# RWAlgorithms/ConjugateGradientOptim.jl

Measured on AMD Instinct MI355X. Metric: CG iterations/sec at n=1e8 (outer iterations of minimizeobjective, PR-CG), higher is better.
Workload: dtype f64

## Files before the change

conjugategradientoptim.jl_amd/_lib.py:

```python
from __future__ import annotations

import ctypes as C
import os
import subprocess

_PKG = os.path.dirname(os.path.abspath(__file__))
LIB_PATH = os.environ.get("CGO_LIB_PATH") or os.path.join(_PKG, "lib", "libcgo_hip.so")
CSRC = os.path.join(_PKG, "csrc")

dp = C.POINTER(C.c_double)
i64p = C.POINTER(C.c_int64)


class BetaConfig(C.Structure):
    _fields_ = [("kind", C.c_int32), ("lbfgs_m", C.c_int32), ("mu", C.c_double)]


class CGConfigC(C.Structure):
    _fields_ = [("eps", C.c_double), ("beta", BetaConfig), ("max_iters", C.c_int64),
                ("verbose", C.c_int32), ("trace_enabled", C.c_int32)]


class LSConfigC(C.Structure):
    _fields_ = [("kind", C.c_int32), ("cond_kind", C.c_int32), ("c1", C.c_double),
# ... 89 lines not shown
    _fields_ = [("kind", C.c_int32), ("k", C.c_int32), ("a", C.c_double * 7), ("a_acc", C.c_double), ("beta", C.c_double),
                ("co_set", C.c_int32), ("co_count", C.c_int32), ("co_gamma", C.c_double), ("co_cy", C.c_double * 10),
                ("co_cs", C.c_double * 10)]


class BatchPassOutC(C.Structure):
    _fields_ = [("ts", (C.c_double * 7) * 7), ("gu", C.c_double), ("uu", C.c_double), ("width", C.c_int64), ("stored", C.c_int64)]


class BatchProbeC(C.Structure):
    _fields_ = [("tier", C.c_int32), ("obj_kind", C.c_int32), ("m", C.c_int32), ("n_params", C.c_int32), ("model", C.c_void_p),
                ("n", C.c_int64), ("batch", C.c_int64), ("x", dp), ("u", dp), ("params", dp * 4), ("scalars", dp),
                ("skip", C.POINTER(C.c_uint8)), ("S", dp), ("Y", dp), ("qn", C.c_void_p), ("npass", C.c_int32),
                ("reserved", C.c_int32), ("pass_", BatchPassC * 32), ("rows", dp), ("out", C.POINTER(BatchPassOutC)),
                ("x_out", dp), ("u_out", dp), ("g_out", dp), ("S_out", dp), ("Y_out", dp), ("qn_out", C.c_void_p),
                ("reason", C.POINTER(C.c_int32)), ("done", i64p), ("passes", i64p), ("points", C.c_int32),
                ("reserved2", C.c_int32), ("ld", C.c_int64), ("symbol", C.c_char * 128)]


ALLGATHER_FN = C.CFUNCTYPE(C.c_int, C.c_void_p, dp, dp, C.c_int32)
FDF_FN = C.CFUNCTYPE(C.c_double, C.c_void_p, dp, dp, C.c_int64)

_vp = C.c_void_p
_pp = C.POINTER(C.c_void_p)
SIGNATURES = {
    "cgo_version": (C.c_int, []),
    "cgo_build_id": (C.c_char_p, []),
    "cgo_last_error": (C.c_char_p, []),
    "cgo_status_name": (C.c_char_p, [C.c_int32]),
    "cgo_device_count": (C.c_int, [C.POINTER(C.c_int32)]),
    "cgo_check_cg_config": (C.c_int, [C.POINTER(CGConfigC)]),
    "cgo_check_ls_config": (C.c_int, [C.POINTER(LSConfigC)]),
    "cgo_ctx_create": (C.c_int, [C.c_int32, _pp]),
    "cgo_solver_policy_init": (None, [C.POINTER(SolverPolicyC)]),
    "cgo_ctx_set_default_policy": (C.c_int, [_vp, C.POINTER(SolverPolicyC)]),
    "cgo_solver_get_policy": (C.c_int, [_vp, C.POINTER(SolverPolicyC)]),
    "cgo_solver_create_ex": (C.c_int, [_vp, _vp, C.POINTER(CGConfigC), C.POINTER(LSConfigC), C.POINTER(SolverPolicyC), _pp]),
    "cgo_solver_create_sys_ex": (C.c_int, [_vp, _vp, C.POINTER(CGConfigC), C.POINTER(LSSConfigC), C.POINTER(SolverPolicyC), _pp]),
    "cgo_ctx_destroy": (C.c_int, [_vp]),
    "cgo_comm_unique_id": (C.c_int, [_vp]),
    "cgo_ctx_set_comm_rccl": (C.c_int, [_vp, C.c_int32, C.c_int32, _vp]),
    "cgo_ctx_set_comm_callback": (C.c_int, [_vp, C.c_int32, C.c_int32, ALLGATHER_FN, _vp]),
    "cgo_ctx_set_comm_shm": (C.c_int, [_vp, C.c_int32, C.c_int32, C.c_char_p, C.c_int32]),
    "cgo_shm_unlink": (C.c_int, [C.c_char_p]),
    "cgo_ctx_comm_info": (C.c_int, [_vp, C.POINTER(C.c_int32), C.POINTER(C.c_int32), C.POINTER(C.c_int32), C.POINTER(C.c_int32)]),
    "cgo_ctx_exchange_stats": (C.c_int, [_vp, i64p, dp, dp, C.c_int32]),
    "cgo_ctx_comm_connect_devices": (C.c_int, [_vp, C.POINTER(C.c_int32)]),
    "cgo_rccl_available": (C.c_int, []),
    "cgo_objective_create": (C.c_int, [_vp, C.c_int32, C.c_int64, C.c_int64, C.c_int64, _pp]),
    "cgo_objective_create_from_source": (C.c_int, [_vp, C.c_char_p, C.c_int32, C.c_int64, C.c_int64, C.c_int64, _pp]),
    "cgo_objective_create_callback": (C.c_int, [_vp, FDF_FN, _vp, C.c_int64, C.c_int64, C.c_int64, _pp]),
    "cgo_objective_destroy": (C.c_int, [_vp]),
    "cgo_objective_create_from_source_ex": (C.c_int, [_vp, C.c_char_p, C.c_int32, C.c_int64, C.c_int64, C.c_int64, _pp]),
    "cgo_objective_num_params": (C.c_int, [_vp, C.POINTER(C.c_int32)]),
    "cgo_objective_set_param_host": (C.c_int, [_vp, C.c_int32, dp]),
    "cgo_objective_set_param_device": (C.c_int, [_vp, C.c_int32, _vp]),
    "cgo_objective_fill_param": (C.c_int, [_vp, C.c_int32, C.c_int32, C.c_uint64, C.c_double, C.c_double]),
    "cgo_objective_set_scalar": (C.c_int, [_vp, C.c_int32, C.c_double]),
    "cgo_objective_set_cost_class": (C.c_int, [_vp, C.c_int32]),
    "cgo_objective_eval_host": (C.c_int, [_vp, dp, dp, dp]),
    "cgo_solver_create": (C.c_int, [_vp, _vp, C.POINTER(CGConfigC), C.POINTER(LSConfigC), _pp]),
    "cgo_solver_destroy": (C.c_int, [_vp]),
    "cgo_solver_set_x0_host": (C.c_int, [_vp, dp]),
    "cgo_solver_set_x0_fill": (C.c_int, [_vp, C.c_int32, C.c_uint64, C.c_double, C.c_double]),
    "cgo_solver_set_x0_device": (C.c_int, [_vp, _vp]),
    "cgo_solver_results_device": (C.c_int, [_vp, _vp, _vp]),
    "cgo_solver_start": (C.c_int, [_vp]),
    "cgo_solver_iterate": (C.c_int, [_vp, C.c_int64, C.POINTER(C.c_int32)]),
    "cgo_solver_results": (C.c_int, [_vp, C.POINTER(ResultsC)]),
    "cgo_solver_trial_log": (C.c_int, [_vp, C.c_int64, dp, dp, dp, i64p]),
    "cgo_solver_profile_enable": (C.c_int, [_vp, C.c_int32]),
    "cgo_solver_profile_reset": (C.c_int, [_vp]),
    "cgo_solver_profile_get": (C.c_int, [_vp, C.c_int32, i64p, dp, dp]),
    "cgo_kernel_kind_name": (C.c_char_p, [C.c_int32]),
    "cgo_solver_kernel_family": (C.c_char_p, [_vp]),
    "cgo_solver_controller_launches": (C.c_int64, [_vp]),
    "cgo_solver_resident_stats": (C.c_int, [_vp, i64p, i64p, i64p]),
    "cgo_solver_lbfgs_stats": (C.c_int, [_vp, i64p, i64p, i64p]),
    "cgo_num_kernel_kinds": (C.c_int, []),
    "cgo_solver_set_lazy_direction": (C.c_int, [_vp, C.c_int32]),
    "cgo_solver_probe_set_beta_prev": (C.c_int, [_vp, C.c_double]),
    "cgo_solver_set_replay_depth": (C.c_int, [_vp, C.c_int32]),
    "cgo_solver_set_lean_sums": (C.c_int, [_vp, C.c_int32]),
    "cgo_solver_probe_set_replay": (C.c_int, [_vp, C.c_int32, dp, dp]),
    "cgo_solver_kernel_symbol": (C.c_int, [_vp, C.c_int32, C.c_char_p, C.c_int32]),
    "cgo_evalwolfeconditions": (C.c_int, [C.POINTER(LSConfigC), C.c_double, C.c_double, C.c_double, C.c_double,
                                          C.c_double, C.c_double, C.POINTER(C.c_int32), C.POINTER(C.c_int32)]),
    "cgo_evalbacktrackcondition": (C.c_int, [C.POINTER(LSConfigC), C.c_double, C.c_double, C.c_double, C.c_double,
                                             C.POINTER(C.c_int32)]),
    "cgo_check_lss_config": (C.c_int, [C.POINTER(LSSConfigC)]),
    "cgo_lss_default_max_iters": (C.c_int64, [C.c_double]),
    "cgo_solver_create_sys": (C.c_int, [_vp, _vp, C.POINTER(CGConfigC), C.POINTER(LSSConfigC), _pp]),
    "cgo_solvesystem": (C.c_int, [_vp, _vp, dp, C.POINTER(CGConfigC), C.POINTER(LSSConfigC), C.POINTER(ResultsC)]),
    "cgo_minimize": (C.c_int, [_vp, _vp, dp, C.POINTER(CGConfigC), C.POINTER(LSConfigC), C.POINTER(ResultsC)]),
    "cgo_minimize_rerun": (C.c_int, [_vp, _vp, dp, C.POINTER(CGConfigC), C.POINTER(LSConfigC),
                                     C.POINTER(CGConfigC), C.POINTER(LSConfigC), C.c_int32,
                                     C.POINTER(ResultsC), C.POINTER(C.c_int32)]),
    "cgo_minimize_batch": (C.c_int, [_vp, C.c_int32, C.c_int64, C.c_int64, dp, dp, C.POINTER(CGConfigC), C.POINTER(LSConfigC),
                                     C.c_int64, C.POINTER(BatchResultsC)]),
    "cgo_batch_max_n": (C.c_int64, [_vp, C.c_int32]),
    "cgo_minimize_batch_obj": (C.c_int, [_vp, _vp, C.c_int64, dp, C.POINTER(dp), C.c_int32, C.POINTER(CGConfigC), C.POINTER(LSConfigC),
                                         C.c_int64, C.POINTER(BatchResultsC)]),
    "cgo_batch_max_n_obj": (C.c_int64, [_vp]),
    "cgo_batch_open": (C.c_int, [_vp, _vp, C.c_int64, C.POINTER(dp), C.c_int32, C.POINTER(_vp)]),
    "cgo_batch_solve": (C.c_int, [_vp, dp, dp, C.POINTER(C.c_uint8), C.POINTER(CGConfigC), C.POINTER(LSConfigC), C.c_int64,
                                  C.POINTER(BatchResultsC)]),
    "cgo_batch_close": (C.c_int, [_vp]),
    "cgo_batch_policy_init": (None, [C.POINTER(BatchPolicyC)]),
    "cgo_minimize_batch_ex": (C.c_int, [_vp, C.c_int32, C.c_int64, C.c_int64, dp, dp, C.POINTER(CGConfigC), C.POINTER(LSConfigC),
                                        C.c_int64, C.POINTER(BatchPolicyC), C.POINTER(BatchResultsC), C.POINTER(C.c_int32)]),
    "cgo_minimize_batch_obj_ex": (C.c_int, [_vp, _vp, C.c_int64, dp, C.POINTER(dp), C.c_int32, C.POINTER(CGConfigC), C.POINTER(LSConfigC),
                                            C.c_int64, C.POINTER(BatchPolicyC), C.POINTER(BatchResultsC), C.POINTER(C.c_int32)]),
    "cgo_batch_open_ex": (C.c_int, [_vp, _vp, C.c_int64, C.POINTER(dp), C.c_int32, C.POINTER(BatchPolicyC), C.POINTER(_vp)]),
    "cgo_batch_rows": (C.c_int, [_vp, C.POINTER(C.c_int32)]),
    "cgo_batch_max_n_ex": (C.c_int64, [_vp, C.c_int32, C.POINTER(BatchPolicyC)]),
    "cgo_batch_max_n_obj_ex": (C.c_int64, [_vp, C.POINTER(BatchPolicyC)]),
    "cgo_batch_rows_shape": (None, [C.POINTER(C.c_int32), C.POINTER(C.c_int32)]),
    "cgo_minimize_batch_lbfgs": (C.c_int, [_vp, C.c_int32, C.c_int64, C.c_int64, dp, dp, C.POINTER(CGConfigC), C.POINTER(LSConfigC),
                                           C.c_int64, C.POINTER(BatchResultsC)]),
    "cgo_batch_lbfgs_max_m": (C.c_int32, []),
    "cgo_batch_lbfgs_max_n": (C.c_int64, [_vp, C.c_int32]),
    "cgo_batch_lbfgs_shape": (None, [C.POINTER(C.c_int32), C.POINTER(C.c_int32)]),
    "cgo_minimize_batch_lbfgs_obj": (C.c_int, [_vp, _vp, C.c_int64, dp, C.POINTER(dp), C.c_int32, dp, C.POINTER(CGConfigC), C.POINTER(LSConfigC),
                                               C.c_int64, C.POINTER(BatchResultsC)]),
    "cgo_batch_lbfgs_max_n_obj": (C.c_int64, [_vp]),
    "cgo_batch_lbfgs_shape_obj": (None, [C.c_int32, C.POINTER(C.c_int32), C.POINTER(C.c_int32)]),
    "cgo_minimize_batch_lbfgs_ex": (C.c_int, [_vp, C.c_int32, C.c_int64, C.c_int64, dp, dp, C.POINTER(CGConfigC), C.POINTER(LSConfigC),
                                              C.c_int64, C.POINTER(BatchPolicyC), C.POINTER(BatchResultsC), C.POINTER(C.c_int32)]),
    "cgo_minimize_batch_lbfgs_obj_ex": (C.c_int, [_vp, _vp, C.c_int64, dp, C.POINTER(dp), C.c_int32, dp, C.POINTER(CGConfigC),
                                                  C.POINTER(LSConfigC), C.c_int64, C.POINTER(BatchPolicyC), C.POINTER(BatchResultsC),
                                                  C.POINTER(C.c_int32)]),
    "cgo_batch_lbfgs_max_n_ex": (C.c_int64, [_vp, C.c_int32, C.c_int32, C.POINTER(BatchPolicyC)]),
    "cgo_batch_lbfgs_max_n_obj_ex": (C.c_int64, [_vp, C.c_int32, C.POINTER(BatchPolicyC)]),
    "cgo_batch_lbfgs_lds_rows": (C.c_int32, [C.c_int32, C.c_int32]),
    "cgo_batch_lbfgs_lds_shape": (None, [C.c_int32, C.POINTER(C.c_int32), C.POINTER(C.c_int32)]),
    "cgo_batch_lbfgs_open": (C.c_int, [_vp, _vp, C.c_int64, C.POINTER(dp), C.c_int32, C.c_int32, C.POINTER(BatchPolicyC), C.POINTER(_vp)]),
    "cgo_batch_lbfgs_solve": (C.c_int, [_vp, dp, dp, C.POINTER(C.c_uint8), C.POINTER(CGConfigC), C.POINTER(LSConfigC), C.c_int64,
                                        C.POINTER(BatchResultsC)]),
    "cgo_batch_lbfgs_m": (C.c_int, [_vp, C.POINTER(C.c_int32)]),
    "cgo_batch_probe": (C.c_int, [_vp, C.POINTER(BatchProbeC)]),
    "cgo_batch_probe_qn_bytes": (C.c_int64, []),
    "cgo_stop_status": (C.c_int32, [C.c_int64, C.c_int64, C.c_double, C.c_double, C.c_double, C.c_double, i64p]),
    "cgo_kernel_dir": (C.c_int, [_vp, dp, dp, C.c_double, C.c_int64, dp]),
    "cgo_kernel_beta_partials": (C.c_int, [_vp, dp, dp, dp, C.c_int64, dp]),
    "cgo_getbeta": (C.c_int, [_vp, C.POINTER(BetaConfig), dp, dp, dp, C.c_int64, dp]),
    "cgo_kernel_trial": (C.c_int, [_vp, dp, dp, C.c_double, dp, dp]),
    "cgo_bench_kernel": (C.c_int, [_vp, _vp, C.c_int32, C.c_int64, C.c_int32, dp, dp]),
    "cgo_bench_stream_mix": (C.c_int, [_vp, C.c_int64, C.c_int32, dp, dp]),
    "cgo_solver_placement_info": (C.c_int, [_vp, dp, dp, C.POINTER(C.c_int32)]),
    "cgo_solver_probe_launch": (C.c_int, [_vp, C.c_int32, C.c_int32, C.c_double, C.c_double, dp, C.c_int32, dp, dp, dp,
                                          dp, C.c_int32, C.POINTER(C.c_int32), dp, dp, dp, C.c_char_p, C.c_int32]),
    "cgo_solver_probe_lbfgs": (C.c_int, [_vp, C.POINTER(LbfgsProbeC)] + [dp] * 13),
    "cgo_solver_probe_resident": (C.c_int, [_vp, C.POINTER(ResidentProbeC), dp, dp, dp, C.c_int64, dp, dp]),
    "cgo_solver_probe_armed": (C.c_int, [_vp, C.POINTER(ArmedProbeC), dp, dp, dp, dp]),
}


class CgoError(RuntimeError):
    def __init__(self, code: int, msg: str):
        super().__init__(f"[cgo error {code}] {msg}")
        self.code = code
        self.msg = msg


def build(force: bool = False) -> str:
    if force:
# ... 34 lines not shown
```

conjugategradientoptim.jl_amd/api.py:

```python
from __future__ import annotations

import ctypes as C
import math
import re
from dataclasses import dataclass, field
from typing import List, Optional, Sequence, Union

import numpy as np

from . import _lib
from ._lib import BetaConfig, CGConfigC, LSConfigC, LSSConfigC, ResultsC, check, dp, i64p



class TraceTrait:
    pass


class EnableTrace(TraceTrait):
    def __repr__(self):
        return "EnableTrace()"


class DisableTrace(TraceTrait):
# ... 561 lines not shown
        c.lse_fixed_reference = tri(self.lse_fixed_reference)
        c.resident_points = self.resident_points or 0
        c.resident_chunk = self.resident_chunk or 0
        c.hbm_stream_bytes = float(self.hbm_stream_bytes or 0.0)
        return c


class Solver:
    def __init__(self, fdf: DeviceObjective, config: CGConfig, linesearch_config: LineSearchConfig,
                 policy: Optional[SolverPolicy] = None):
        if not isinstance(fdf, DeviceObjective):
            raise TypeError(
                "fdf! must be an objective descriptor: a device objective (QuadDiag, RosenbrockPaired, Booth, "
                "ElementwiseObjective, ...) or HostObjective(closure, n) — there is no CPU solver path in this package")
        self.obj, self.config, self.ls = fdf, config, linesearch_config
        self._cfg_c, self._ls_c = config._c(), linesearch_config._c()
        self._h = C.c_void_p()
        create = (_lib.lib().cgo_solver_create_sys_ex if isinstance(linesearch_config, LinesearchSolveSys)
                  else _lib.lib().cgo_solver_create_ex)
        self._pol_c = policy._c() if policy is not None else None
        check(create(fdf.ctx._h, fdf._h, C.byref(self._cfg_c), C.byref(self._ls_c),
                     C.byref(self._pol_c) if self._pol_c is not None else None, C.byref(self._h)))

    def policy(self) -> dict:
        c = _lib.SolverPolicyC()
        check(_lib.lib().cgo_solver_get_policy(self._h, C.byref(c)))
        return {n: getattr(c, n) for n, _ in c._fields_ if n not in ("size", "reserved")}

    def set_x0(self, x_initial_global: np.ndarray):
        loc = self.obj.local(np.asarray(x_initial_global, dtype=np.float64))
        check(_lib.lib().cgo_solver_set_x0_host(self._h, loc.ctypes.data_as(dp)))

    def set_x0_fill(self, fill: str, lo: float, hi: float = 0.0, seed: int = 0):
        check(_lib.lib().cgo_solver_set_x0_fill(self._h, FILL_KINDS[fill], seed, lo, hi))

    def set_x0_device(self, x0):
        check(_lib.lib().cgo_solver_set_x0_device(self._h, _dev_ptr(x0, self.obj.n_local)))

    def results_device(self, minimizer=None, gradient=None):
        check(_lib.lib().cgo_solver_results_device(self._h, _dev_ptr(minimizer, self.obj.n_local), _dev_ptr(gradient, self.obj.n_local)))

    def start(self):
        check(_lib.lib().cgo_solver_start(self._h))

    def iterate(self, iters: int) -> bool:
        fin = C.c_int32(0)
        check(_lib.lib().cgo_solver_iterate(self._h, iters, C.byref(fin)))
        return bool(fin.value)

    def enable_trial_log(self):
        cnt = C.c_int64()
        check(_lib.lib().cgo_solver_trial_log(self._h, -1, None, None, None, C.byref(cnt)))

    def trial_log(self):
        cnt = C.c_int64()
        check(_lib.lib().cgo_solver_trial_log(self._h, 0, None, None, None, C.byref(cnt)))
        k = cnt.value
        a, p, d = np.zeros(max(k, 1)), np.zeros(max(k, 1)), np.zeros(max(k, 1))
        check(_lib.lib().cgo_solver_trial_log(self._h, k, a.ctypes.data_as(dp), p.ctypes.data_as(dp),
                                              d.ctypes.data_as(dp), C.byref(cnt)))
        return a[:k], p[:k], d[:k]

    def kernel_family(self) -> str:
        return _lib.lib().cgo_solver_kernel_family(self._h).decode()

    def kernel_symbol(self, kind_name: str) -> str:
        L = _lib.lib()
        buf = C.create_string_buffer(200)
        for k in range(L.cgo_num_kernel_kinds()):
            if L.cgo_kernel_kind_name(k).decode() == kind_name:
                check(L.cgo_solver_kernel_symbol(self._h, k, buf, 200))
                return buf.value.decode()
        return ""

    def set_lazy_direction(self, on: bool = True):
        check(_lib.lib().cgo_solver_set_lazy_direction(self._h, int(bool(on))))

    def set_replay_depth(self, d: int):
        check(_lib.lib().cgo_solver_set_replay_depth(self._h, int(d)))

    def set_lean_sums(self, on: bool):
        check(_lib.lib().cgo_solver_set_lean_sums(self._h, int(bool(on))))

    def probe_launch(self, kind_name: str, variant: int, a_acc: float, beta: float, a: Sequence[float], x, u=None, aux=None,
                     beta_prev: Optional[float] = None, replay: Optional[Sequence] = None):
        L = _lib.lib()
        kk = [L.cgo_kernel_kind_name(k).decode() for k in range(L.cgo_num_kernel_kinds())].index(kind_name)
        if beta_prev is not None:
            check(L.cgo_solver_probe_set_beta_prev(self._h, float(beta_prev)))
        if replay is not None:
            ra = np.ascontiguousarray([p[0] for p in replay], dtype=np.float64)
            rb = np.ascontiguousarray([p[1] for p in replay], dtype=np.float64)
            check(L.cgo_solver_probe_set_replay(self._h, len(replay), ra.ctypes.data_as(dp), rb.ctypes.data_as(dp)))
        n = self.obj.n_local
        vec = lambda v: None if v is None else np.ascontiguousarray(v, dtype=np.float64)
        x, u, aux = vec(x), vec(u), vec(aux)
        for v in (x, u, aux):
            if v is not None and v.size != n:
                raise ValueError(f"probe vectors hold n_local = {n} elements")
        av = np.ascontiguousarray(a, dtype=np.float64) if len(a) else np.zeros(1)
        sums, ln = np.full(64, np.nan), C.c_int32(0)
        xo, uo, go = np.empty(n), np.empty(n), np.empty(n)
        sym = C.create_string_buffer(200)
        ptr = lambda v: None if v is None else v.ctypes.data_as(dp)
        check(L.cgo_solver_probe_launch(self._h, kk, int(variant), float(a_acc), float(beta), ptr(av), len(a), ptr(x), ptr(u),
                                        ptr(aux), ptr(sums), 64, C.byref(ln), ptr(xo), ptr(uo), ptr(go), sym, 200))
        return dict(sums=sums[:ln.value].copy(), x=xo, u=uo, g=go, symbol=sym.value.decode())

    LBFGS_PASSES = ("push", "push_gram", "direction_gram", "direction_trial", "push_lite", "loop")

    def probe_lbfgs(self, pass_name: str, x=None, u=None, g=None, gt=None, S=None, Y=None, **kw):
        n = self.obj.n_local
        P = self._cfg_c.beta.lbfgs_m + 1
        vec = lambda v: None if v is None else np.ascontiguousarray(v, dtype=np.float64)
        x, u, g, gt = vec(x), vec(u), vec(g), vec(gt)
        for v in (x, u, g, gt):
            if v is not None and v.size != n:
                raise ValueError(f"probe vectors hold n_local = {n} elements")
        S = None if S is None else np.ascontiguousarray(S, dtype=np.float64).reshape(P, n)
        Y = None if Y is None else np.ascontiguousarray(Y, dtype=np.float64).reshape(P, n)
        p = _lib.LbfgsProbeC()
        p.pass_ = self.LBFGS_PASSES.index(pass_name)
        dots = None
        for key, val in kw.items():
            if key in ("list", "spec_list"):
                getattr(p, key)[:len(val)] = [int(v) for v in val]
                setattr(p, "count" if key == "list" else "spec_count", len(val))
            elif key in ("cy", "cs", "alpha"):
                getattr(p, key)[:len(val)] = [float(v) for v in val]
            elif key == "stats":
                p.M, p.S = float(val[0]), float(val[1])
            elif key == "dots":
                dots = np.ascontiguousarray(val, dtype=np.float64).reshape(-1, 10)
                p.dots, p.dot_count = dots.ctypes.data_as(dp), dots.shape[0]
            else:
                if not hasattr(p, key):
                    raise TypeError(f"probe_lbfgs: no field {key}")
                setattr(p, key, val)
        outs = {k: np.full(n, np.nan) for k in ("x", "xo", "u", "g", "gt")}
        So, Yo = np.full((P, n), np.nan), np.full((P, n), np.nan)
        ptr = lambda v: None if v is None else v.ctypes.data_as(dp)
        check(_lib.lib().cgo_solver_probe_lbfgs(self._h, C.byref(p), ptr(x), ptr(u), ptr(g), ptr(gt), ptr(S), ptr(Y),
                                                *[ptr(outs[k]) for k in ("x", "xo", "u", "g", "gt")], ptr(So), ptr(Yo)))
        sym = p.symbol.decode()
        return dict(sums=np.array(p.sums[:p.sums_len]), S=So, Y=Yo, alpha=np.array(p.alpha[:]), symbols=sym.split(" + ") if sym else [],
                    new_in_list=p.new_in_list, spec_ok=bool(p.spec_ok),
                    gram=np.array(p.gram[:5 + 5 * p.spec_count]) if p.spec_ok else None, **outs)

    def probe_resident(self, script, x, u):
        n = self.obj.n_local
        x, u = np.ascontiguousarray(x, dtype=np.float64), np.ascontiguousarray(u, dtype=np.float64)
        if x.size != n or u.size != n:
            raise ValueError(f"probe vectors hold n_local = {n} elements")
        p = _lib.ResidentProbeC()
        if len(script) > 32:
            raise ValueError("probe_resident: at most 32 passes")
        p.npass = len(script)
        for q, item in enumerate(script):
            c = p.pass_[q]
            if item[0] == "trial":
                c.kind, a = 0, item[1]
            elif item[0] == "accept_dir_trial":
                c.kind, c.a_acc, c.beta, a = 1, float(item[1]), float(item[2]), item[3]
            else:
                raise ValueError(f"probe_resident: no pass kind {item[0]!r}")
            if len(a) > 7:
                raise ValueError("probe_resident: at most 7 trial steps")
            c.k = len(a)
            c.a[:len(a)] = [float(v) for v in a]
        rows = np.full((max(p.npass, 1), 256, 56), np.nan)
        xo, uo = np.empty(n), np.empty(n)
        check(_lib.lib().cgo_solver_probe_resident(self._h, C.byref(p), x.ctypes.data_as(dp), u.ctypes.data_as(dp),
                                                   rows.ctypes.data_as(dp), rows.size, xo.ctypes.data_as(dp), uo.ctypes.data_as(dp)))
        g = p.grid
        got = rows.ravel()[:p.npass * g * 56].reshape(p.npass, g, 56)
        outs, rws, tails = [], [], []
# ... 1097 lines not shown
```

conjugategradientoptim.jl_amd/csrc/cgo_backend_cg.hip:

```cpp
#include "cgo_backend_internal.hpp"

#include "cgo_kernels.hip.hpp"
#include "cgo_kernels_cg.hip.hpp"
#include "cgo_kernels_chain.hip.hpp"
#include "cgo_kernels_lse.hip.hpp"
#include "cgo_kernels_resident.hip.hpp"

namespace cgo {

using namespace dev;

double bytes_r(int obj_kind, int mode, int64_t n, int n_params) {
    const int p = std::max(obj_kind == CGO_OBJ_QUAD_DIAG ? 1 : 0, n_params);
    return 8.0 * (double)n * (double)r_vectors(mode, p);
}

template <int N> using Pts = std::integral_constant<int, N>;
template <int MAXPTS, class F>
static inline void with_points(int npts, F f) {
    static_assert(MAXPTS == 1 || MAXPTS == 3 || MAXPTS == 5 || MAXPTS == 7, "a launch evaluates 1, 3, 5 or 7 trial points");
    if constexpr (MAXPTS >= 3) { if (npts == 3) return f(Pts<3>{}); }
    if constexpr (MAXPTS >= 5) { if (npts == 5) return f(Pts<5>{}); }
    if constexpr (MAXPTS >= 7) { if (npts != 1) return f(Pts<7>{}); }
    return f(Pts<1>{});
}

template <class Obj, bool BIG>
static int launch_cg(int mode, int npts, const RParams &P, int grid, hipStream_t st) {
#define ROW(MODE, MAXPTS) if (mode == (MODE) && P.tail.ctl) { with_points<MAXPTS>(npts, [&](auto n) { k_cg_armed<Obj, decltype(n)::value><<<grid, BLOCK, 0, st>>>(P); }); return 0; }
    CGO_CG_ARMED_ROWS(ROW)
#undef ROW
    switch (mode) {
#define ROW(MODE, MAXPTS) case (MODE): with_points<MAXPTS>(npts, [&](auto n) { k_cg<Obj, (MODE), decltype(n)::value, BIG><<<grid, BLOCK, 0, st>>>(P); }); return 0;
    CGO_CG_ROWS(ROW)
#undef ROW
    default: break;
    }
    if constexpr (BIG) {
        switch (mode) {
#define ROW(MODE, MAXPTS) case (MODE): with_points<MAXPTS>(npts, [&](auto n) { k_cg<Obj, (MODE), decltype(n)::value, true><<<grid, BLOCK, 0, st>>>(P); }); return 0;
        CGO_CG_LAG_ROWS(ROW)
        CGO_CG_REPLAY_ROWS(ROW)
        CGO_CG_LEAN_ROWS(ROW)
#undef ROW
        default: break;
        }
    }
    return -1;
}

static inline bool lean_row(int mode) {
#define ROW(MODE, MAXPTS) if (mode == (MODE)) return true;
    CGO_CG_LEAN_ROWS(ROW)
#undef ROW
    return false;
}
int HipBackend::lean_for(int mode) const { return (lean_bits_ && lean_row(mode | lean_bits_)) ? lean_bits_ : 0; }

void unpack_r(const double *s, int k, Scal *out, bool dir, int npts) {
    if (npts == 0) npts = npts_for(k);
    for (int j = 0; j < k; ++j) {
        const double *q = s + RS_PER_POINT * j;
        out[j].f = q[RS_F]; out[j].gtu = q[RS_GTU]; out[j].gtgt = q[RS_GTGT]; out[j].gtg = q[RS_GTG];
        out[j].yy = q[RS_YY]; out[j].uy = q[RS_UY]; out[j].ygt = q[RS_YGT];
    }
    if (dir) { out[0].gu = s[RS_PER_POINT * npts]; out[0].uu = s[RS_PER_POINT * npts + 1]; }
}

static inline int chain_npts(int mode, int npts) { return ((mode & R_TRIAL) && npts >= 3) ? 3 : 1; }

RPlan HipBackend::r_plan(int mode, int npts) const {
    const double bytes = bytes_r(obj_->kind, mode, obj_->n_local, obj_->nparams());
    const bool big = r_big_only(mode) || bytes > big_bytes(r_read_only(mode));
    return {big, big ? GRID_BIG : grid_cg(obj_->n_local, chain() ? 1 : npts), chain() ? chain_npts(mode, npts) : npts, bytes};
}
bool HipBackend::adt_is_big() const { return bytes_r(obj_->kind, R_ADT, obj_->n_local, obj_->nparams()) > big_bytes(false); }

int HipBackend::launch_r(int kk, int mode, double a_acc, double beta, const double *a, int k, bool fetch,
                         double *sums) {
    if (int rc = pipe_drain()) return rc;
    pipe_streak_ = 0;
    if (u_lag_ && !(mode & R_ULAG)) {
        if (r_reads_u(mode)) { if (int rc = materialize_u()) return rc; }
        else if (mode & (R_INIT | R_RESET)) u_lag_ = false;
    }
    if (rep_n_ > 0 && !(mode & R_REPLAY)) { if (int rc = materialize_lag()) return rc; }
    RPlan plan;
    const int npts = npts_for(k);
    if (int rc = launch_r_kernel(kk, mode, a_acc, beta, a, k, npts, nullptr, &plan)) return rc;
    const int grid = plan.grid;
    total_launches_++;
    const bool has_sums = r_has_sums(mode);
    const bool fused = has_sums && tail_fused(grid);
    if (has_sums && chain()) {
        const bool three = plan.npts == 3;
        const int W = three ? NRC3 : NRC, edge = three ? RC3_EDGE : RC_EDGE, nsums = three ? NR : NR1;
        if (!fused) { if (int rc = finalize_rows(ctx_, grid, W, true)) return rc; }
        const int Wd = ctx_->world(), me = ctx_->rank();
        std::vector<double> raw((size_t)W * Wd);
        double all[NRC3];
        if (int rc = fetch_sums(ctx_, all, MERGE_SUM, W, raw.data())) return rc;
        if (sums) std::memcpy(sums, all, sizeof(double) * nsums);
        if (me > 0) {
            const double *e = raw.data() + (size_t)(me - 1) * W + edge + 4;
            halo_xl_[0] = e[0]; halo_xl_[1] = e[1]; halo_ul_[0] = e[2]; halo_ul_[1] = e[3];
        }
        if (me < Wd - 1) {
            const double *e = raw.data() + (size_t)(me + 1) * W + edge;
            halo_xr_[0] = e[0]; halo_xr_[1] = e[1]; halo_ur_[0] = e[2]; halo_ur_[1] = e[3];
        }
        if (probe_) { std::memcpy(probe_row_, all, sizeof(double) * W); probe_len_ = W; }
    } else if (has_sums) {
        if (!fused) { if (int rc = finalize_rows(ctx_, grid, rows_for(npts), true)) return rc; }
        if (fetch) {
            if (int rc = fetch_sums(ctx_, sums, MERGE_SUM, rows_for(npts))) return rc;
        }
        if (probe_ && fetch) { std::memcpy(probe_row_, sums, sizeof(double) * rows_for(npts)); probe_len_ = rows_for(npts); }
    }
    if (prof_on_) prof_commit(kk, plan.bytes);
    return CGO_OK;
}

bool HipBackend::lazy_eligible() const {
    if (!lazy_on_ || !rmode_ || chain() || sys_on_ || probe_ || pingpong_ == 1) return false;
    bool aot = false;
#define ROW(KIND, T) aot = aot || obj_->kind == KIND;
    CGO_OBJ_ROWS(ROW)
#undef ROW
    if (!aot) return false;
    if (const char *e = getenv("CGO_PINGPONG")) { if (e[0] == '1') return false; }
    if (ctl_depth() > 0) return false;
    return adt_is_big() && r_plan(R_TRIAL, 1).big;
}

int HipBackend::materialize_u() {
    if (!u_lag_) return CGO_OK;
    const int64_t asked = total_launches_;
    const int rc = launch_rk(KK_MATERIALIZE_U, 0.0, 0.0, nullptr, 0, false, nullptr);
    total_launches_ = asked;
    if (rc) return rc;
    u_lag_ = false;
    return CGO_OK;
}

int HipBackend::materialize_lag() {
    if (int rc = materialize_u()) return rc;
    if (rep_n_ == 0) return CGO_OK;
    const int64_t asked = total_launches_;
    const int rc = launch_rk(KK_MATERIALIZE_XU, 0.0, 0.0, nullptr, 0, false, nullptr);
    total_launches_ = asked;
    if (rc) return rc;
    rep_n_ = 0;
    return CGO_OK;
}

int HipBackend::set_replay_depth_now(int d) {
    if (d < 1 || d > RMAX + 1) { set_error("replay depth: 1 … 8"); return CGO_EINVAL; }
    if (d != replay_depth_) { if (int rc = materialize_lag()) return rc; }
    replay_depth_ = d;
    return CGO_OK;
}

void HipBackend::set_probe_replay(int nrep, const double *a, const double *beta) {
    probe_rep_n_ = std::max(0, std::min(nrep, (int)RMAX));
    for (int j = 0; j < probe_rep_n_; ++j) { probe_rep_a_[j] = a[j]; probe_rep_b_[j] = beta[j]; }
}

int HipBackend::accept_dir_trial_r(double a_acc, double beta, const double *a, int k, double *s) {
    if (!lazy_eligible()) return launch_rk(KK_ACCEPT_DIR_TRIAL, a_acc, beta, a, k, true, s);
    if (replay_depth_ >= 2) {
        if (int rc = materialize_u()) return rc;
        if (rep_n_ < replay_depth_ - 1 && rep_n_ < RMAX) {
            const int mode_n = r_mode_of(KK_ACCEPT_TRIAL_NOSTORE);
            if (int rc = launch_r(KK_ACCEPT_TRIAL_NOSTORE, mode_n | lean_for(mode_n), a_acc, beta, a, k, true, s)) return rc;
            rep_a_[rep_n_] = a_acc; rep_b_[rep_n_] = beta; rep_n_++;
            return CGO_OK;
        }
        const int mode_s = R_REPLAY | R_ADT;
        if (int rc = launch_r(KK_ACCEPT_DIR_TRIAL, mode_s | lean_for(mode_s), a_acc, beta, a, k, true, s)) return rc;
        rep_n_ = 0;
        return CGO_OK;
    }
    if (!u_lag_) {
        if (int rc = launch_rk(KK_ACCEPT_TRIAL_LAZY, a_acc, beta, a, k, true, s)) return rc;
        u_lag_ = true; beta_lag_ = beta;
        return CGO_OK;
    }
    if (int rc = launch_r(KK_ACCEPT_DIR_TRIAL, R_ULAG | R_ADT, a_acc, beta, a, k, true, s)) return rc;
    u_lag_ = false;
    return CGO_OK;
}
int HipBackend::trial_r(const double *a, int k, double *s) {
    if (rep_n_ > 0 && lazy_eligible()) return launch_r(KK_TRIAL, R_REPLAY | R_TRIAL, 0, 0, a, k, true, s);
    if (u_lag_ && lazy_eligible()) return launch_r(KK_TRIAL, R_ULAG | R_TRIAL, 0, 0, a, k, true, s);
    return launch_rk(KK_TRIAL, 0, 0, a, k, true, s);
}

bool HipBackend::pipe_fused(int grid) const {
    return tail_fused(grid) && obj_->kind != CGO_OBJ_USER && !chain() && ctl_fused_;
}
bool HipBackend::tail_fused(int grid) const {
    static const int cap = [] { const char *e = getenv("CGO_FUSED_TAIL_MAX_GRID"); int v = e ? atoi(e) : 0; return v > 0 ? v : 1024; }();
    return ctx_->fused_tail && grid <= cap && grid <= TAIL_GROUP * TAIL_GROUP;
}
Tail HipBackend::make_tail(bool on) {
    Tail t{};
    if (!on) return t;
    ctx_->seq++;
    t.partials2 = ctx_->partials2_f; t.tickets = ctx_->tickets; t.out = ctx_->out_dev;
    t.strict = ctx_->tail_strict ? 1 : 0;
    ctx_->pub_target(&t.host_out, &t.host_seq);
    ctx_->pub_checked = (t.host_out != nullptr) && !ctx_->tail_strict;
    t.seq = ctx_->seq;
    return t;
}

int HipBackend::launch_r_kernel(int kk, int mode, double a_acc, double beta, const double *a, int k, int npts,
                                const CtlArgs *ctl, RPlan *plan_out) {
    HIPCHK(hipSetDevice(ctx_->device));
    if (obj_->unset_slot() >= 0) return param_unset_error(obj_->unset_slot());
    const int64_t n = obj_->n_local;
    if (mode & (R_GRAD | R_GRADT)) { if (int rc = ensure_ga()) return rc; }
    const bool has_sums = r_has_sums(mode);
    const RPlan plan = *plan_out = r_plan(mode, npts);
    const bool big = plan.big; const int grid = plan.grid;
    last_mode_ = mode; last_npts_ = plan.npts; last_big_ = big;
    if (chain()) {
        if (int rc = prof_begin(kk)) return rc;
        if (int rc = launch_chain_kernel(mode, a_acc, beta, a, k, plan.npts, big, grid, make_tail(has_sums && !ctl && tail_fused(grid)))) return rc;
        return prof_end();
    }
    RParams P;
    P.x = xc_; P.u = uc_; P.gout = ga_.p; obj_->param_args(P); P.n = n;
    P.xo = xc_; P.uo = uc_;
    P.a_acc = a_acc; P.beta = beta; P.s0 = obj_->s0; P.partials = ctx_->partials;
    P.beta_prev = beta_lag_;
    P.nrep = (mode & R_REPLAY) ? rep_n_ : 0;
    for (int j = 0; j < RMAX; ++j) { P.ra[j] = j < P.nrep ? rep_a_[j] : 0.0; P.rb[j] = j < P.nrep ? rep_b_[j] : 0.0; }
    P.ctl = ctl;
    P.x2 = xn_;
    for (int j = 0; j < MAXP; ++j) P.a[j] = (a && j < k) ? a[j] : ((a && k > 0) ? a[k - 1] : 0.0);
    P.tail = make_tail(has_sums && !ctl && tail_fused(grid));
    if (ctl && pipe_fused(grid)) {
        P.tail.partials2 = ctx_->partials2_f; P.tail.tickets = ctx_->tickets; P.tail.out = ctx_->out_dev;
        P.tail.strict = ctx_->tail_strict ? 1 : 0;
        P.tail.ctl = ctl_dev_; P.tail.ctl_rec = ctl_rec_; P.tail.ctl_seq = ctl_seq_;
        if (!ctx_->single()) {
            P.tail.xw = ctx_->world(); P.tail.xme = ctx_->rank(); P.tail.xseq0 = epoch_ << 40;
            for (int r = 0; r < P.tail.xw && r < 8; ++r) P.tail.xmail[r] = ctx_->comm->dev_mailbox(r);
        }
    }
    if (P.tail.tickets) P.partials = ctx_->partials_f;
    const bool wr_x = r_writes_x(mode), wr_u = r_writes_u(mode);
    const bool pp = big && !ctl && (wr_x || wr_u) && !(mode & R_PROJ) && pingpong_ready();
    if (pp && wr_x) P.xo = xalt_;
    if (pp && wr_u) P.uo = ualt_;
    if (mode == R_PROJ && !xn_) { set_error("internal: no second iterate buffer"); return CGO_ESTATE; }
    hipStream_t st = ctx_->stream;
    if (int rc = prof_begin(kk)) return rc;
    int r = -2;
    switch (obj_->kind) {
#define ROW(KIND, T) case KIND: r = big ? launch_cg<T, true>(mode, npts, P, grid, st) : launch_cg<T, false>(mode, npts, P, grid, st); break;
    CGO_OBJ_ROWS(ROW)
#undef ROW
    case CGO_OBJ_USER:
        if (!obj_->rtc) { set_error("user objective has no compiled module"); return CGO_EINVAL; }
        if (r_big_only(mode)) break;
        if (int rc = launch_module(obj_->rtc->cg(mode, npts, big), &P, grid, st)) return rc;
        r = 0;
        break;
    default: break;
    }
    if (r) { set_error("internal: CG kernel mode not instantiated"); return CGO_EINVAL; }
    HIPCHK(hipGetLastError());
    if (pp && wr_x) std::swap(xc_, xalt_);
    if (pp && wr_u) std::swap(uc_, ualt_);
    return prof_end();
}

template <bool BIG>
static int launch_chain(int mode, int npts, const ChainParams &P, int grid, hipStream_t st) {
    switch (mode) {
#define ROW(MODE, MAXPTS) case (MODE): with_points<MAXPTS>(npts, [&](auto n) { k_chain<(MODE), decltype(n)::value, BIG><<<grid, BLOCK, 0, st>>>(P); }); return 0;
    CGO_CHAIN_ROWS(ROW)
#undef ROW
    default: return -1;
    }
}

int HipBackend::launch_chain_kernel(int mode, double a_acc, double beta, const double *a, int k, int npts, bool big, int grid, const Tail &tail) {
    ChainParams P;
    P.tail = tail;
    for (int j = 0; j < 3; ++j) P.a[j] = (a && j < k) ? a[j] : ((a && k > 0) ? a[k - 1] : 0.0);
    P.x = xc_; P.u = uc_; P.xo = xc_; P.uo = uc_; P.gout = ga_.p;
    P.odd = (int)(obj_->n_local & 1);
    P.n = obj_->n_local + P.odd; P.a_acc = a_acc; P.beta = beta; P.partials = tail.tickets ? ctx_->partials_f : ctx_->partials;
    for (int j = 0; j < 2; ++j) { P.hxl[j] = halo_xl_[j]; P.hul[j] = halo_ul_[j]; P.hxr[j] = halo_xr_[j]; P.hur[j] = halo_ur_[j]; }
    P.has_left = obj_->offset > 0 ? 1 : 0;
    P.has_right = obj_->offset + obj_->n_local < obj_->n_global ? 1 : 0;
    const bool wr_x = r_writes_x(mode), wr_u = r_writes_u(mode);
    if (wr_x) P.xo = xalt_;
    if (wr_u) P.uo = ualt_;
    const int r = big ? launch_chain<true>(mode, npts, P, grid, ctx_->stream) : launch_chain<false>(mode, npts, P, grid, ctx_->stream);
    if (r) { set_error("internal: chain kernel mode not instantiated"); return CGO_EINVAL; }
    HIPCHK(hipGetLastError());
    if (wr_x) std::swap(xc_, xalt_);
    if (wr_u) std::swap(uc_, ualt_);
    return CGO_OK;
}

std::string HipBackend::r_symbol(int mode, int npts, bool big) const {
    char buf[160];
    if (chain()) snprintf(buf, sizeof buf, "k_chain<%d, %d, %s>", mode, npts, big ? "true" : "false");
    else snprintf(buf, sizeof buf, "k_cg<%s, %d, %d, %s>", obj_tname(), mode, npts, big ? "true" : "false");
    return buf;
}

std::string HipBackend::kernel_symbol(int kk) const {
    if (!rmode_) {
        if (obj_->two_phase() || kk == KK_LBFGS_PUSH || kk == KK_LBFGS_LOOP || kk == KK_LBFGS_FINAL) return lbfgs_symbol(kk);
        const int mode = fused_mode(kk);
        return mode < 0 ? "" : fused_symbol(obj_tname(), mode, is_big(obj_->kind, mode, obj_->n_local, obj_->nparams(), pol_.hbm_stream_bytes));
    }
    const RKind *rk = r_kind(kk);
    if (!rk) return "";
    int mode = rk->mode;
    const bool lazy = lazy_eligible();
    switch (kk) {
    case KK_ACCEPT_DIR_TRIAL: if (lazy) mode |= replay_depth_ >= 2 ? R_REPLAY : R_ULAG; break;
    case KK_ACCEPT_TRIAL_LAZY: case KK_MATERIALIZE_U: if (!lazy || replay_depth_ >= 2) return ""; break;
    case KK_ACCEPT_TRIAL_NOSTORE: case KK_MATERIALIZE_XU: if (!lazy || replay_depth_ < 2) return ""; break;
    default: break;
    }
    const RPlan plan = r_plan(mode, rk->pts == PTS_ONE ? 1 : npts_for(rk->pts == PTS_MAX ? max_points() : std::min(max_points(), 3)));
    if ((mode & R_REPLAY) && (mode & R_ACCEPT)) mode |= lean_for(mode);
    return r_symbol(mode, plan.npts, plan.big);
}


__global__ void k_ctl_init(CtlDev *d, const CtlConfig cfg, const CtlState st, unsigned long long round) {
    d->cfg = cfg;
    d->st = st;
    d->round = round;
    d->args = ctl_args_of(st);
}



template <int N, int THREADS>
__global__ __launch_bounds__(THREADS) void k_finalize_ctl(const double *partials, int rows, double *out, CtlDev *d,
                                                          CtlRecord *rec_ring, unsigned long long *seq_ring) {
    constexpr int G = BLOCK / N;
    constexpr int WD = sizeof(CtlDev) / 8, WR = sizeof(CtlRecord) / 8;
    __shared__ double sm[G][N];
    __shared__ double fin[CTL_NSUMS];
    __shared__ CtlDev sd;
    __shared__ CtlRecord sr;
    const int tid = threadIdx.x;
    if (tid < WD) ((unsigned long long *)&sd)[tid] = ((const unsigned long long *)d)[tid];
    if (tid < CTL_NSUMS) fin[tid] = 0.0;
    __syncthreads();
    const bool go = sd.st.go != 0;
    const unsigned long long round = sd.round, seq = round + 1;
    CtlRecord *rec_host = rec_ring + (round % PIPE_RING);
    unsigned long long *seq_host = seq_ring + (round % PIPE_RING);
    if (go) {
        if (tid < G * N) {
            double t = 0.0;
            const long long total = (long long)rows * N;
            for (long long i = tid; i < total; i += G * N) t += partials[i];
            sm[tid / N][tid % N] = t;
        }
        __syncthreads();
        if (tid < N) {
            double v = 0.0;
#pragma unroll
            for (int g = 0; g < G; ++g) v += sm[g][tid];
            out[tid] = v;
            fin[tid] = v;
        }
        __syncthreads();
    }
    if (tid == 0) {
        if (go) {
            ctl_step(sd.cfg, sd.st, fin, sr);
            sd.args = ctl_args_of(sd.st);
        } else ctl_idle_record(sr);
        sd.round = round + 1;
    }
    __syncthreads();
    if (go && tid < WD) ((unsigned long long *)d)[tid] = ((const unsigned long long *)&sd)[tid];
    if (!go && tid == 0) d->round = round + 1;
    if (tid < WR) {
        ((unsigned long long *)rec_host)[tid] = ((const unsigned long long *)&sr)[tid];
        __threadfence_system();
    }
    __syncthreads();
    if (tid == 0) __hip_atomic_store(seq_host, seq, __ATOMIC_RELEASE, __HIP_MEMORY_SCOPE_SYSTEM);
}

int HipBackend::ctl_depth() const {
    if (!(rmode_ && ctx_->host_publish && !obj_->two_phase())) return 0;
    if (ctx_->single()) return ctl_depth_;
    if (!ctx_->dev_exchange() || ctx_->force_gather) return 0;
    return (!adt_is_big() && pipe_fused(grid_cg(obj_->n_local, policy_points()))) ? ctl_depth_ : 0;
}

int HipBackend::pipe_alloc() {
    if (ctl_dev_) return CGO_OK;
    HIPCHK(hipMalloc(&ctl_dev_, sizeof(CtlDev)));
    HIPCHK(hipHostMalloc((void **)&ctl_rec_, sizeof(CtlRecord) * PIPE_RING, hipHostMallocDefault));
    HIPCHK(hipHostMalloc((void **)&ctl_seq_, sizeof(unsigned long long) * PIPE_RING, hipHostMallocDefault));
    std::memset(ctl_rec_, 0, sizeof(CtlRecord) * PIPE_RING);
    std::memset(ctl_seq_, 0, sizeof(unsigned long long) * PIPE_RING);
    pipe_prof_.assign(PIPE_RING, {-1, 0u});
    return CGO_OK;
}

// ... 176 lines not shown
        if (pp.first >= 0 && pp.second == prof_gen_ && pp.first < ring_used_) {
            ring_[pp.first].kk = KK_ACCEPT_DIR_TRIAL;
            ring_[pp.first].bytes = prof_bytes_[KK_ACCEPT_DIR_TRIAL];
        }
    }
    if (!rec.accepted) pipe_stopped_ = true;
    if (!pipe_stopped_) {
        const int64_t want = std::min<int64_t>(std::min<int64_t>(ctl_depth_, pipe_streak_), rounds - 1);
        const int64_t have = (int64_t)(pipe_enq_ - pipe_done_);
        if (have < want && (want - have >= (want + 1) / 2 || have == 0))
            if (int rc = pipe_enqueue(want - have)) return rc;
    }
    return CGO_OK;
}

int HipBackend::accept_dir_trial_keep_streak(const CtlState &s0, Scal *out) {
    const int64_t keep = pipe_streak_;
    const int rc = accept_dir_trial(s0.a_acc, s0.beta, s0.a, s0.npts, out);
    pipe_streak_ = keep;
    return rc;
}



int HipBackend::probe_prepare() {
    if (probe_) return CGO_OK;
    if (int rc = pipe_drain()) return rc;
    u_lag_ = false; rep_n_ = 0;
    HIPCHK(hipSetDevice(ctx_->device));
    HIPCHK(hipStreamSynchronize(ctx_->stream));
    (void)pingpong_ready();
    const size_t n = (size_t)obj_->n_local, na = n + (chain() ? (n & 1) : 0), np = probe_padded(na);
    DevBuf *bufs[] = {&x_, &u_, &x2_, &u2_, &ga_, &gb_};
    for (DevBuf *b : bufs) {
        if (b == &x2_ || b == &u2_) { if (pingpong_ != 1) continue; }
        if (int rc = b->alloc(np)) return rc;
        HIPCHK(hipMemsetAsync(b->p, 0, na * sizeof(double), ctx_->stream));
        HIPCHK(hipMemsetD32Async((hipDeviceptr_t)(b->p + na), (int)PROBE_NAN32, (np - na) * 2, ctx_->stream));
    }
    for (int j = 0; j < obj_->nparams(); ++j) {
        if (!obj_->p_set[j]) continue;
        DevBuf p;
        if (int rc = p.alloc(np)) return rc;
        HIPCHK(hipMemcpyAsync(p.p, obj_->p[j].p, n * sizeof(double), hipMemcpyDeviceToDevice, ctx_->stream));
        HIPCHK(hipMemsetD32Async((hipDeviceptr_t)(p.p + n), (int)PROBE_NAN32, (np - n) * 2, ctx_->stream));
        HIPCHK(hipStreamSynchronize(ctx_->stream));
        std::swap(p.p, obj_->p[j].p); std::swap(p.n, obj_->p[j].n);
    }
    HIPCHK(hipStreamSynchronize(ctx_->stream));
    xc_ = x_.p; uc_ = u_.p; xalt_ = x2_.p; ualt_ = u2_.p;
    g_ = ga_.p; gt_ = gb_.p; xn_ = gb_.p;
    lse_have_ = false;
    probe_ = true;
    return CGO_OK;
}

int HipBackend::probe_slack_intact() {
    const size_t n = (size_t)obj_->n_local, na = n + (chain() ? (n & 1) : 0);
    struct { const DevBuf *b; const char *name; size_t used; int slot; } v[] = {
        {&x_, "x", na, -1}, {&u_, "u", na, -1}, {&x2_, "x (ping-pong)", na, -1}, {&u2_, "u (ping-pong)", na, -1},
        {&ga_, "gradient A", na, -1}, {&gb_, "gradient B / x2", na, -1}, {&obj_->p[0], "parameter vector", n, 0},
        {&obj_->p[1], "parameter vector 1", n, 1}, {&obj_->p[2], "parameter vector 2", n, 2}, {&obj_->p[3], "parameter vector 3", n, 3}};
    std::vector<unsigned> h;
    for (const auto &e : v) {
        if (!e.b->p || (e.slot >= 0 && !(e.slot < obj_->nparams() && obj_->p_set[e.slot]))) continue;
        const size_t words = (e.b->n - e.used) * 2;
        h.assign(words, 0u);
        HIPCHK(hipMemcpyAsync(h.data(), e.b->p + e.used, words * 4, hipMemcpyDeviceToHost, ctx_->stream));
        HIPCHK(hipStreamSynchronize(ctx_->stream));
        for (size_t w = 0; w < words; ++w)
            if (h[w] != PROBE_NAN32) {
                set_error(std::string("probe: the launch wrote past the ") + std::to_string(e.used) + " elements of " + e.name +
                          " (element " + std::to_string(e.used + w / 2) + ")");
                return CGO_ESTATE;
            }
    }
    return CGO_OK;
}

int HipBackend::probe_launch(int kk, int variant, double a_acc, double beta, const double *a, int k, const double *x,
                             const double *u, const double *aux, double *sums, int sums_cap, int *sums_len, double *x_out,
                             double *u_out, double *g_out, std::string &symbol) {
    *sums_len = 0;
    const bool lse = obj_->two_phase();
    if (k < 0 || k > MAXP || (k > 0 && !a)) { set_error("probe: 0 ≤ k ≤ 7 trial steps"); return CGO_EINVAL; }
    if (!rmode_ && !lse) return probe_launch_stored(kk, variant, a_acc, beta, a, k, x, u, aux, sums, sums_cap, sums_len, x_out, u_out, g_out, symbol);
    int mode = -1;
    if (lse) {
        if (kk == KK_LSE_STATS && (variant == 0 || variant == LM_NOU || variant == (LM_ACCEPT | LM_DIR))) mode = variant;
        if (kk == KK_LSE_GRAD && variant >= 0 && variant <= 2) mode = variant;
        if (kk == KK_LSE_STATS && mode != LM_NOU && k < 1) mode = -1;
        if (kk == KK_LSE_GRAD && mode != 2 && k < 1) mode = -1;
    } else {
        static constexpr RKind norm_passes{KK_SCALED_NORM, R_GRAD, PTS_ONE, {R_GRADT, 0}};
        const RKind *rk = kk == KK_SCALED_NORM ? &norm_passes : r_kind(kk);
        if (rk && (variant & R_LEAN)) {
            const int full = kk == KK_ACCEPT_DIR_TRIAL ? (R_REPLAY | R_ADT) : (kk == KK_ACCEPT_TRIAL_NOSTORE ? rk->mode : -1);
            if (lean_row(variant) && (variant & ~R_LEAN) == full) mode = variant;
        } else if (rk) {
            const int m = variant ? variant : rk->mode;
            if (r_kind_allows(*rk, m) || (kk == KK_INIT && chain() && m == R_EDGES)) mode = m;
        }
        if (mode > 0 && (mode & (R_TRIAL | R_GRADT | R_PROJ)) && k < 1) mode = -1;
        if (mode > 0 && chain() && k > 3) mode = -1;
        if (mode > 0 && r_big_only(mode) && (chain() || obj_->kind == CGO_OBJ_USER)) mode = -1;
    }
    if (mode < 0) { set_error("probe: kernel kind / variant / trial steps not a launch this solver's engine issues"); return CGO_EINVAL; }
    if (int rc = probe_prepare()) return rc;
    HIPCHK(hipSetDevice(ctx_->device));
    hipStream_t st = ctx_->stream;
    const size_t n = (size_t)obj_->n_local, nb = n * sizeof(double);
    double *ub = lse ? u_.p : uc_;
    double *gb = lse ? gt_ : ga_.p;
    double *auxb = lse ? g_ : xn_;
    auto put = [&](double *dst, const double *src) -> int {
        if (src) HIPCHK(hipMemcpyAsync(dst, src, nb, hipMemcpyHostToDevice, st));
        else HIPCHK(hipMemsetD32Async((hipDeviceptr_t)dst, (int)PROBE_NAN32, n * 2, st));
        return CGO_OK;
    };
    if (int rc = put(xc_, x)) return rc;
    if (int rc = put(ub, u)) return rc;
    if (int rc = put(auxb, aux)) return rc;
    if (gb != auxb) { if (int rc = put(gb, nullptr)) return rc; }
    if (!lse && pingpong_ == 1) {
        if (int rc = put(xalt_, nullptr)) return rc;
        if (int rc = put(ualt_, nullptr)) return rc;
    }
    HIPCHK(hipStreamSynchronize(st));
    probe_len_ = 0;
    last_mode_ = -1;
    beta_lag_ = probe_beta_prev_;
    rep_n_ = (!lse && (mode & R_REPLAY)) ? probe_rep_n_ : 0;
    for (int j = 0; j < rep_n_; ++j) { rep_a_[j] = probe_rep_a_[j]; rep_b_[j] = probe_rep_b_[j]; }
    int rc = CGO_OK;
    char buf[160];
    if (lse) {
        Scal o;
        if (kk == KK_LSE_STATS) {
            lse_have_ = false;
            rc = lse_stats(mode, a_acc, beta, k ? a[0] : 0.0, o, mode == (LM_ACCEPT | LM_DIR));
            snprintf(buf, sizeof buf, "k_lse_stats<%d, %s, %s>", last_mode_, last_big_ ? "true" : "false", last_npts_ ? "true" : "false");
        } else {
            const bool nb0 = need_beta_;
            need_beta_ = mode == 1;
            rc = lse_grad(mode == 2, k ? a[0] : 0.0, o);
            need_beta_ = nb0;
            snprintf(buf, sizeof buf, "k_lse_grad<%s, %s, %s>", last_mode_ == 1 ? "true" : "false", last_mode_ == 2 ? "true" : "false",
                     last_big_ ? "true" : "false");
        }
        if (rc) return rc;
        symbol = buf;
    } else {
        double s[64];
        rc = launch_r(kk, mode, a_acc, beta, a, k, true, s);
        rep_n_ = 0;
        if (rc) return rc;
        symbol = r_symbol(last_mode_, last_npts_, last_big_);
    }
    HIPCHK(hipStreamSynchronize(st));
    if (x_out) HIPCHK(hipMemcpyAsync(x_out, xc_, nb, hipMemcpyDeviceToHost, st));
    if (u_out) HIPCHK(hipMemcpyAsync(u_out, lse ? u_.p : uc_, nb, hipMemcpyDeviceToHost, st));
    if (g_out) HIPCHK(hipMemcpyAsync(g_out, mode == R_PROJ && !lse ? xn_ : gb, nb, hipMemcpyDeviceToHost, st));
    HIPCHK(hipStreamSynchronize(st));
    if (int rc2 = probe_slack_intact()) return rc2;
    *sums_len = probe_len_;
    if (probe_len_ > sums_cap) { set_error("probe: sums_cap smaller than the launch's row"); return CGO_EINVAL; }
    if (probe_len_) std::memcpy(sums, probe_row_, sizeof(double) * probe_len_);
    return CGO_OK;
}

void HipBackend::probe_append(const double *row, int len) {
    if (probe_len_ + len > (int)(sizeof probe_row_ / sizeof probe_row_[0])) return;
    std::memcpy(probe_row_ + probe_len_, row, sizeof(double) * len);
    probe_len_ += len;
}

int HipBackend::probe_launch_stored(int kk, int variant, double a_acc, double beta, const double *a, int k, const double *x,
                                    const double *u, const double *aux, double *sums, int sums_cap, int *sums_len, double *x_out,
                                    double *u_out, double *g_out, std::string &symbol) {
    if (ctx_->world() != 1) { set_error("probe: a single-rank solver"); return CGO_EINVAL; }
    const bool host = obj_->host_closure();
    int mode = -1;
    if (const MKind *mk = m_kind(kk)) {
        const int m = variant ? variant : (host ? mk->host : fused_mode(kk));
        if (host ? m == mk->host : (m == mk->mode || (mk->alt && m == mk->alt))) mode = m;
    } else if (kk == KK_SCALED_NORM) {
        mode = (variant == 0 || variant == 1 || variant == 3 || variant == 4) ? variant : -1;
    }
    const bool trial_step = kk == KK_TRIAL || kk == KK_ACCEPT_DIR_TRIAL;
    if (mode >= 0 && trial_step && k != 1) mode = -1;
    if (mode < 0) { set_error("probe: kernel kind / variant / trial steps not a launch this solver's engine issues"); return CGO_EINVAL; }
    if (int rc = probe_prepare()) return rc;
    HIPCHK(hipSetDevice(ctx_->device));
    hipStream_t st = ctx_->stream;
    const size_t n = (size_t)obj_->n_local, nb = n * sizeof(double);
    auto put = [&](double *dst, const double *src) -> int {
        if (src) HIPCHK(hipMemcpyAsync(dst, src, nb, hipMemcpyHostToDevice, st));
        else HIPCHK(hipMemsetD32Async((hipDeviceptr_t)dst, (int)PROBE_NAN32, n * 2, st));
        return CGO_OK;
    };
    const bool norm = kk == KK_SCALED_NORM;
    const bool gt_in_x = norm && (mode == 1 || mode == 4);
    const bool swaps = kk == KK_ACCEPT_DIR_TRIAL || kk == KK_ACCEPT_DIR || kk == KK_ACCEPT_ONLY;
    if (int rc = put(xc_, gt_in_x ? nullptr : x)) return rc;
    if (int rc = put(u_.p, u)) return rc;
    if (int rc = put(swaps ? gt_ : g_, aux)) return rc;
    if (int rc = put(swaps ? g_ : gt_, gt_in_x ? x : nullptr)) return rc;
    HIPCHK(hipStreamSynchronize(st));
    probe_len_ = 0;
    probe_syms_.clear();
    probe_stored_ = true;
    int rc = CGO_OK;
    Scal o[MAXP];
    switch (kk) {
    case KK_INIT: {
        double s[NS];
        rc = host ? host_trial(0.0, true, o[0]) : launch_k(KK_INIT, 0, 0, 0, true, s);
        break;
    }
    case KK_TRIAL: {
        const bool nb0 = need_beta_;
        need_beta_ = mode == m_mode_of(KK_TRIAL);
        rc = trial(a, 1, o);
        need_beta_ = nb0;
        break;
    }
    case KK_ACCEPT_DIR_TRIAL: rc = accept_dir_trial(a_acc, beta, a, 1, o); break;
    case KK_ACCEPT_DIR: rc = accept_dir(a_acc, beta, o[0]); break;
    case KK_ACCEPT_ONLY: rc = accept_only(a_acc); break;
    case KK_RESET_DIR: rc = reset_dir(o[0]); break;
    case KK_UPG_NORM: { double uu; rc = upg_sumsq(uu); break; }
    default: { double mx, ss; bool nan; rc = scaled_norm_parts(mode, 0.0, mx, ss, nan); break; }
    }
    probe_stored_ = false;
    if (rc) return rc;
    symbol = probe_syms_;
    HIPCHK(hipStreamSynchronize(st));
    if (x_out) HIPCHK(hipMemcpyAsync(x_out, xc_, nb, hipMemcpyDeviceToHost, st));
    if (u_out) HIPCHK(hipMemcpyAsync(u_out, u_.p, nb, hipMemcpyDeviceToHost, st));
    if (g_out) HIPCHK(hipMemcpyAsync(g_out, gt_, nb, hipMemcpyDeviceToHost, st));
// ... 429 lines not shown
```

conjugategradientoptim.jl_amd/csrc/cgo_capi.hip:

```cpp
#include <sys/mman.h>

#include <cmath>
#include <cstdio>
#include <cstdlib>
#include <cstring>
#include <functional>
#include <new>
#include <vector>

#include "cgo_hip_backend.hpp"
#include "cgo_qn.hpp"
#include "cgo_build_id.inc"

using namespace cgo;

struct cgo_ctx { HipCtx c; int refs = 1; cgo_solver_policy defpol; bool has_defpol = false; };
struct cgo_objective { HipObjective o; cgo_ctx *owner = nullptr; int refs = 1; };
static void ctx_unref(cgo_ctx *c) { if (c && --c->refs == 0) delete c; }
static void obj_unref(cgo_objective *o) {
    if (o && --o->refs == 0) {
        cgo_ctx *c = o->owner;
        if (c) (void)hipSetDevice(c->c.device);
        delete o;
        ctx_unref(c);
// ... 264 lines not shown
    REQUIRE(obj && dev_local, "null argument");
    REQUIRE(slot >= 0 && slot < obj->o.nparams(), "objective has no such parameter vector");
    HipCtx *c = obj->o.ctx;
    HIPCHK2(hipSetDevice(c->device));
    HIPCHK2(hipMemcpyAsync(obj->o.p[slot].p, dev_local, sizeof(double) * (size_t)obj->o.n_local, hipMemcpyDeviceToDevice, c->stream));
    HIPCHK2(hipStreamSynchronize(c->stream));
    obj->o.p_set[slot] = true;
    return CGO_OK;
    API_GUARD_END
}

int cgo_objective_num_params(cgo_objective *obj, int32_t *n_params) {
    API_GUARD_BEGIN
    REQUIRE(obj && n_params, "null argument");
    *n_params = obj->o.nparams();
    return CGO_OK;
    API_GUARD_END
}

int cgo_objective_fill_param(cgo_objective *obj, int32_t slot, int32_t fill_kind, uint64_t seed,
                             double lo, double hi) {
    API_GUARD_BEGIN
    REQUIRE(obj, "null argument");
    REQUIRE(slot >= 0 && slot < obj->o.nparams(), "objective has no such parameter vector");
    REQUIRE(fill_kind >= 0 && fill_kind <= 2, "unknown fill kind");
    HipCtx *c = obj->o.ctx;
    HIPCHK2(hipSetDevice(c->device));
    if (int rc = fill_device(c, obj->o.p[slot].p, obj->o.n_local, obj->o.offset, fill_kind, seed, lo, hi)) return rc;
    HIPCHK2(hipStreamSynchronize(c->stream));
    obj->o.p_set[slot] = true;
    return CGO_OK;
    API_GUARD_END
}

int cgo_objective_set_scalar(cgo_objective *obj, int32_t slot, double value) {
    API_GUARD_BEGIN
    REQUIRE(obj && slot == 0, "bad argument");
    obj->o.s0 = value;
    return CGO_OK;
    API_GUARD_END
}

int cgo_objective_set_cost_class(cgo_objective *obj, int32_t cost_class) {
    API_GUARD_BEGIN
    REQUIRE(obj && (cost_class == 0 || cost_class == 1), "bad argument");
    REQUIRE(obj->o.kind == CGO_OBJ_USER, "built-in objectives carry their own cost class");
    obj->o.user_cheap = cost_class == 1;
    return CGO_OK;
    API_GUARD_END
}

int cgo_objective_eval_host(cgo_objective *obj, const double *x, double *g, double *f) {
    API_GUARD_BEGIN
    REQUIRE(obj && x && f, "null argument");
    if (obj->o.host_closure()) {
        std::vector<double> tmp;
        if (!g) { tmp.resize((size_t)obj->o.n_local); g = tmp.data(); }
        *f = obj->o.host_fn(obj->o.host_user, g, x, obj->o.n_local);
        return CGO_OK;
    }
    return HipBackend::run_eval(&obj->o, x, g, f);
    API_GUARD_END
}

void cgo_solver_policy_init(cgo_solver_policy *p) {
    if (!p) return;
    std::memset(p, 0, sizeof(*p));
    p->size = (int32_t)sizeof(*p);
    p->resident = p->controller_depth = p->controller_graph = p->controller_fused = -1;
    p->fused_tail = p->strict_tail = p->placement_search = -1;
    p->lbfgs_fuse_grad = p->lbfgs_fuse_trial = p->lse_fixed_reference = -1;
}

int cgo_ctx_set_default_policy(cgo_ctx *ctx, const cgo_solver_policy *policy) {
    API_GUARD_BEGIN
    REQUIRE(ctx, "null argument");
    if (!policy) { ctx->has_defpol = false; return CGO_OK; }
    REQUIRE(policy->size == (int32_t)sizeof(cgo_solver_policy), "cgo_solver_policy.size does not match this library (call cgo_solver_policy_init first)");
    ctx->defpol = *policy; ctx->has_defpol = true;
    return CGO_OK;
    API_GUARD_END
}

static const int kReplayDepth = 6;
static const bool kLeanSums = true;
static int env_tri(const char *name) { const char *e = getenv(name); return e ? (e[0] != '0' ? 1 : 0) : -1; }
static int resolve_policy(cgo_ctx *ctx, const cgo_solver_policy *arg, cgo_solver_policy &r, std::string &why) {
    cgo_solver_policy lib; cgo_solver_policy_init(&lib);
    const cgo_solver_policy *defp = ctx->has_defpol ? &ctx->defpol : nullptr;
    for (const cgo_solver_policy *p : {arg, defp})
        if (p && p->size != (int32_t)sizeof(cgo_solver_policy)) { why = "cgo_solver_policy.size does not match this library (call cgo_solver_policy_init first)"; return CGO_EINVAL; }
    r = lib;
    const cgo_solver_policy *layers[2] = {defp, arg};
    for (const cgo_solver_policy *p : layers) {
        if (!p) continue;
        if (p->points) r.points = p->points;
        if (p->resident >= 0) r.resident = p->resident;
        if (p->controller_depth >= 0) r.controller_depth = p->controller_depth;
        if (p->controller_graph >= 0) r.controller_graph = p->controller_graph;
        if (p->controller_fused >= 0) r.controller_fused = p->controller_fused;
        if (p->stored_gradient) r.stored_gradient = p->stored_gradient;
        if (p->fused_tail >= 0) r.fused_tail = p->fused_tail;
        if (p->strict_tail >= 0) r.strict_tail = p->strict_tail;
        if (p->placement_search >= 0) r.placement_search = p->placement_search;
        if (p->placement_stages) r.placement_stages = p->placement_stages;
        if (p->placement_max_bytes) r.placement_max_bytes = p->placement_max_bytes;
        if (p->lbfgs_form) r.lbfgs_form = p->lbfgs_form;
        if (p->lbfgs_fuse_grad >= 0) r.lbfgs_fuse_grad = p->lbfgs_fuse_grad;
        if (p->lbfgs_fuse_trial >= 0) r.lbfgs_fuse_trial = p->lbfgs_fuse_trial;
        if (p->lse_fixed_reference >= 0) r.lse_fixed_reference = p->lse_fixed_reference;
        if (p->resident_points) r.resident_points = p->resident_points;
        if (p->resident_chunk) r.resident_chunk = p->resident_chunk;
        if (p->hbm_stream_bytes > 0.0) r.hbm_stream_bytes = p->hbm_stream_bytes;
    }
    if (!(r.points == 0 || r.points == 1 || r.points == 3 || r.points == 5 || r.points == 7)) { why = "cgo_solver_policy.points must be 0, 1, 3, 5 or 7"; return CGO_EINVAL; }
    if (r.lbfgs_form < 0 || r.lbfgs_form > 4) { why = "cgo_solver_policy.lbfgs_form must be 0 … 4"; return CGO_EINVAL; }
    if (!(r.resident_points == 0 || r.resident_points == 1 || r.resident_points == 3 || r.resident_points == 7)) { why = "cgo_solver_policy.resident_points must be 0, 1, 3 or 7"; return CGO_EINVAL; }
    if (r.placement_stages < 0 || r.placement_stages > 3 || r.placement_max_bytes < 0) { why = "cgo_solver_policy.placement_* out of range"; return CGO_EINVAL; }
    if (r.resident < 0) r.resident = env_tri("CGO_RESIDENT");
    if (r.controller_depth < 0) { if (const char *e = getenv("CGO_CTL_DEPTH")) r.controller_depth = std::max(0, atoi(e)); }
    if (r.controller_graph < 0) r.controller_graph = env_tri("CGO_CTL_GRAPH");
    if (r.controller_fused < 0) r.controller_fused = env_tri("CGO_CTL_FUSED");
    if (!r.stored_gradient) { const char *e = getenv("CGO_STORED_G"); r.stored_gradient = (e && e[0] == '1') ? 1 : 0; }
    if (r.placement_search < 0) r.placement_search = env_tri("CGO_PLACE_TUNE");
    if (!r.placement_stages) { if (const char *e = getenv("CGO_PLACE_STAGES")) { const int v = atoi(e); if (v >= 1 && v <= 3) r.placement_stages = v; } }
    if (!r.lbfgs_form) {
        const char *tl = getenv("CGO_LBFGS_TWO_LOOP"), *sp = getenv("CGO_LBFGS_SPEC");
        if (tl && tl[0] == '1') r.lbfgs_form = 4;
        else if (sp && sp[0] == '0') r.lbfgs_form = 3;
        else if (sp && sp[0] == '1') r.lbfgs_form = 2;
    }
    if (r.lbfgs_fuse_grad < 0) r.lbfgs_fuse_grad = env_tri("CGO_LBFGS_FUSE_GRAD");
    if (r.lbfgs_fuse_trial < 0) r.lbfgs_fuse_trial = env_tri("CGO_LBFGS_FUSE_TRIAL");
    if (r.lse_fixed_reference < 0) r.lse_fixed_reference = env_tri("CGO_LSE_REF");
    if (!r.resident_points) { if (const char *e = getenv("CGO_RES_POINTS")) { const int v = atoi(e); if (v == 1 || v == 3 || v == 7) r.resident_points = v; } }
    if (!r.resident_chunk) { if (const char *e = getenv("CGO_RES_CHUNK")) { const long long v = atoll(e); if (v >= 2 && v < (1LL << 30)) r.resident_chunk = (int32_t)(v & ~1LL); } }
    if (!(r.hbm_stream_bytes > 0.0)) { if (const char *e = getenv("CGO_BIG_BYTES")) { const double v = atof(e); if (v > 0.0) r.hbm_stream_bytes = v; } }
    if (r.controller_graph < 0) r.controller_graph = 0;
    if (r.controller_fused < 0) r.controller_fused = 1;
    if (r.lbfgs_fuse_grad < 0) r.lbfgs_fuse_grad = 1;
    if (r.lbfgs_fuse_trial < 0) r.lbfgs_fuse_trial = 1;
    if (r.lse_fixed_reference < 0) r.lse_fixed_reference = 1;
    if (r.placement_search < 0) r.placement_search = 0;
    return CGO_OK;
}

int cgo_solver_get_policy(cgo_solver *s, cgo_solver_policy *out) {
    API_GUARD_BEGIN
    REQUIRE(s && out, "null argument");
    *out = s->pol;
    out->points = s->be->policy_points();
    out->resident = s->be->resident_enabled() ? 1 : 0;
    out->controller_depth = s->be->ctl_depth_setting();
    out->fused_tail = s->ctx->c.fused_tail ? 1 : 0;
    out->strict_tail = s->ctx->c.tail_strict ? 1 : 0;
    return CGO_OK;
    API_GUARD_END
}

static int make_solver(cgo_ctx *ctx, cgo_objective *obj, const cgo_cg_config *cfg, const cgo_ls_config *ls,
                       const cgo_lss_config *lss, const cgo_solver_policy *policy, cgo_solver **out) {
    *out = nullptr;
    REQUIRE(obj->o.ctx == &ctx->c, "objective belongs to another ctx");
    std::string why;
    if (int rc = check_cg_config(cfg, why)) { set_error(why); return rc; }
    if (ls) { if (int rc = check_ls_config(ls, why)) { set_error(why); return rc; } }
    else {
        if (int rc = check_lss_config(lss, why)) { set_error(why); return rc; }
        REQUIRE(cfg->beta.kind < CGO_BETA_LBFGS, "solvesystem takes a CGβConfig (solve_system.jl:69), not a QNβConfig");
        REQUIRE(!obj->o.two_phase() && !obj->o.host_closure() && obj->o.kind != CGO_OBJ_ROSENBROCK_CHAINED,
                "solvesystem needs an element-wise device objective (k_cg kernel family)");
    }
    const bool chain = obj->o.kind == CGO_OBJ_ROSENBROCK_CHAINED;
    if (chain) REQUIRE(cfg->beta.kind != CGO_BETA_LBFGS, "the chained (stencil) Rosenbrock objective runs on the gradient-free CG kernels: CG β kinds only");
    cgo_solver_policy pol;
    { std::string pw; if (int rc = resolve_policy(ctx, policy, pol, pw)) { set_error(pw); return rc; } }
    cgo_solver *s = new cgo_solver();
    s->ctx = ctx; s->obj = obj; s->pol = pol;
    obj->refs++;
    obj->o.users++;
    s->be = new HipBackend(&ctx->c, &obj->o);
    s->sv = nullptr;
    s->be->set_policy(pol);
    s->be->set_need_beta(cfg->beta.kind != CGO_BETA_LBFGS);
    s->be->set_rmode(chain || (!obj->o.two_phase() && !obj->o.host_closure() && cfg->beta.kind != CGO_BETA_LBFGS && (!ls || !pol.stored_gradient)));
    int rc = s->be->alloc();
    if (rc) { delete s; obj_unref(obj); return rc; }
    const bool cheap = obj->o.kind == CGO_OBJ_QUAD_DIAG || obj->o.kind == CGO_OBJ_BOOTH ||
                       (obj->o.kind == CGO_OBJ_USER && obj->o.user_cheap);
    s->be->set_multi_min_n(0);
    s->be->set_multi5_min_n(cheap ? 0 : INT64_MAX);
    s->be->set_multi7_min_n(cheap ? 0 : INT64_MAX);
    s->be->set_three_point_band(0, 0);
    const char *mm = getenv("CGO_MULTI_MIN_N"), *m5 = getenv("CGO_MULTI5_MIN_N"), *m7 = getenv("CGO_MULTI7_MIN_N");
    if (chain) m5 = m7 = nullptr;
    if (mm || m5 || m7) s->be->set_three_point_band(0, 0);
    if (mm) s->be->set_multi_min_n(atoll(mm));
    if (m5) s->be->set_multi5_min_n(atoll(m5));
    if (m7) s->be->set_multi7_min_n(atoll(m7));
    if (pol.points) {
        const int pts = chain ? std::min(pol.points, 3) : pol.points;
        s->be->set_three_point_band(0, 0);
        s->be->set_multi_min_n(pts >= 3 ? 0 : INT64_MAX);
        s->be->set_multi5_min_n(pts >= 5 ? 0 : INT64_MAX);
        s->be->set_multi7_min_n(pts >= 7 ? 0 : INT64_MAX);
    }
    s->be->set_ctl_depth((ls && !cheap && !chain && s->be->policy_points() <= 3 && (ctx->c.world() == 1 || ctx->c.dev_exchange()) && obj->o.n_local <= 100000) ? 4 : 0);
    if (pol.controller_depth >= 0) s->be->set_ctl_depth(chain ? 0 : pol.controller_depth);
    s->be->set_ctl_graph(pol.controller_graph != 0);
    {
        bool lazy = obj->o.kind == CGO_OBJ_QUAD_DIAG;
        const int forced = env_tri("CGO_LAZY_DIR");
        if (forced >= 0) lazy = forced != 0;
        s->be->set_lazy_direction(lazy);
    }
    {
        int depth = 1;
        if (obj->o.kind == CGO_OBJ_QUAD_DIAG && 8.0 * (double)obj->o.n_local * 5.0 > 1.4e9) depth = kReplayDepth;
        if (const char *e = getenv("CGO_REPLAY_DEPTH")) { const int v = atoi(e); if (v >= 1 && v <= 8) depth = v; }
        s->be->set_replay_depth(depth);
    }
    {
        bool lean = kLeanSums && obj->o.kind == CGO_OBJ_QUAD_DIAG && 8.0 * (double)obj->o.n_local * 5.0 > 1.4e9;
        const int forced = env_tri("CGO_LEAN_SUMS");
        if (forced >= 0) lean = forced != 0;
        s->be->set_beta_unread(beta_unread_sums(cfg->beta.kind));
        s->be->set_lean_sums(lean);
    }
    if (int prc = s->be->place()) { delete s; obj_unref(obj); return prc; }
    if (pol.resident >= 0) s->be->set_resident(pol.resident != 0);
    if (int prc = s->be->prepare_controller()) { delete s; obj_unref(obj); return prc; }
    s->sv = ls ? new Solver(s->be, *cfg, *ls) : new Solver(s->be, *cfg, *lss);
    *out = s;
    return CGO_OK;
}

int cgo_solver_create(cgo_ctx *ctx, cgo_objective *obj, const cgo_cg_config *cfg,
                      const cgo_ls_config *ls, cgo_solver **out) {
    API_GUARD_BEGIN
    REQUIRE(ctx && obj && cfg && ls && out, "null argument");
    return make_solver(ctx, obj, cfg, ls, nullptr, nullptr, out);
    API_GUARD_END
}

int cgo_solver_create_ex(cgo_ctx *ctx, cgo_objective *obj, const cgo_cg_config *cfg, const cgo_ls_config *ls,
                         const cgo_solver_policy *policy, cgo_solver **out) {
    API_GUARD_BEGIN
    REQUIRE(ctx && obj && cfg && ls && out, "null argument");
    return make_solver(ctx, obj, cfg, ls, nullptr, policy, out);
    API_GUARD_END
}

int cgo_solver_create_sys(cgo_ctx *ctx, cgo_objective *obj, const cgo_cg_config *cfg,
                          const cgo_lss_config *ls, cgo_solver **out) {
    API_GUARD_BEGIN
    REQUIRE(ctx && obj && cfg && ls && out, "null argument");
    return make_solver(ctx, obj, cfg, nullptr, ls, nullptr, out);
    API_GUARD_END
}

int cgo_solver_create_sys_ex(cgo_ctx *ctx, cgo_objective *obj, const cgo_cg_config *cfg, const cgo_lss_config *ls,
                             const cgo_solver_policy *policy, cgo_solver **out) {
    API_GUARD_BEGIN
    REQUIRE(ctx && obj && cfg && ls && out, "null argument");
    return make_solver(ctx, obj, cfg, nullptr, ls, policy, out);
    API_GUARD_END
}

int cgo_check_lss_config(const cgo_lss_config *ls) {
    API_GUARD_BEGIN
    std::string why;
    if (int rc = check_lss_config(ls, why)) { set_error(why); return rc; }
    return CGO_OK;
    API_GUARD_END
}

int64_t cgo_lss_default_max_iters(double rho) { return lss_default_max_iters(rho); }

int cgo_solver_destroy(cgo_solver *s) {
    API_GUARD_BEGIN
    if (s) {
        (void)hipSetDevice(s->ctx->c.device);
        cgo_objective *o = s->obj;
        delete s;
        obj_unref(o);
    }
    return CGO_OK;
    API_GUARD_END
}

int cgo_solver_set_x0_host(cgo_solver *s, const double *x0) {
    API_GUARD_BEGIN
    REQUIRE(s && x0, "null argument");
    return s->be->set_x0_host(x0);
    API_GUARD_END
}

int cgo_solver_set_x0_device(cgo_solver *s, const double *x0_dev) {
    API_GUARD_BEGIN
    REQUIRE(s && x0_dev, "null argument");
    hipPointerAttribute_t at;
    if (hipPointerGetAttributes(&at, x0_dev) != hipSuccess || at.type != hipMemoryTypeDevice || at.device != s->ctx->c.device) {
        (void)hipGetLastError();
        set_error("cgo_solver_set_x0_device: not a device pointer of this context's GPU");
        return CGO_EINVAL;
    }
    return s->be->set_x0_device(x0_dev);
    API_GUARD_END
}

int cgo_solver_results_device(cgo_solver *s, double *minimizer_dev, double *gradient_dev) {
// ... 59 lines not shown
    if (int rc = s->be->tail_errors()) return rc;
    if (out->minimizer || out->gradient) return s->be->download(out->minimizer, out->gradient);
    return CGO_OK;
    API_GUARD_END
}

int cgo_solver_trial_log(cgo_solver *s, int64_t cap, double *a, double *phi, double *dphi, int64_t *count) {
    API_GUARD_BEGIN
    REQUIRE(s && count, "null argument");
    if (cap < 0) { s->sv->set_log_enabled(true); *count = 0; return CGO_OK; }
    const auto &L = s->sv->trial_log();
    *count = (int64_t)L.size();
    const int64_t m = std::min<int64_t>(cap, (int64_t)L.size());
    for (int64_t i = 0; i < m; ++i) {
        if (a) a[i] = L[i].a;
        if (phi) phi[i] = L[i].phi;
        if (dphi) dphi[i] = L[i].dphi;
    }
    return CGO_OK;
    API_GUARD_END
}

const char *cgo_solver_kernel_family(cgo_solver *s) {
    if (!s) return "";
    const bool qn = s->sv->config().beta.kind == CGO_BETA_LBFGS;
    if (s->obj->o.two_phase()) return qn ? "k_lse (two-phase) + k_lbfgs" : "k_lse (two-phase)";
    if (s->be->rmode()) {
        const int mp = s->be->max_points();
        return mp >= 7 ? "k_cg (gradient-free, 7-point)" : mp >= 5 ? "k_cg (gradient-free, 5-point)" : (mp >= 3 ? "k_cg (gradient-free, 3-point)" : "k_cg (gradient-free, 1-point)");
    }
    return qn ? "k_fused (stored gradient) + k_lbfgs" : "k_fused (stored gradient)";
}

int64_t cgo_solver_controller_launches(cgo_solver *s) { return s ? s->be->ctl_served() : 0; }

int cgo_solver_resident_stats(cgo_solver *s, int64_t *slices, int64_t *iterations, int64_t *gave_up) {
    API_GUARD_BEGIN
    REQUIRE(s, "null argument");
    if (slices) *slices = s->be->resident_slices();
    if (iterations) *iterations = s->be->resident_iters();
    if (gave_up) *gave_up = s->be->resident_gave_up();
    return CGO_OK;
    API_GUARD_END
}

int cgo_solver_lbfgs_stats(cgo_solver *s, int64_t *speculated, int64_t *fused, int64_t *plain) {
    API_GUARD_BEGIN
    REQUIRE(s, "null argument");
    if (speculated) *speculated = s->be->push_count(0);
    if (fused) *fused = s->be->push_count(1);
    if (plain) *plain = s->be->push_count(2);
    return CGO_OK;
    API_GUARD_END
}

int cgo_solver_kernel_symbol(cgo_solver *s, int32_t kernel_kind, char *buf, int32_t cap) {
    API_GUARD_BEGIN
    REQUIRE(s && buf && cap > 0, "bad argument");
    const std::string sym = s->be->kernel_symbol(kernel_kind);
    std::snprintf(buf, (size_t)cap, "%s", sym.c_str());
    return CGO_OK;
    API_GUARD_END
}

int cgo_solver_set_lazy_direction(cgo_solver *s, int32_t on) {
    API_GUARD_BEGIN
    REQUIRE(s, "null argument");
    return s->be->set_lazy_direction_now(on != 0);
    API_GUARD_END
}

int cgo_solver_set_replay_depth(cgo_solver *s, int32_t d) {
    API_GUARD_BEGIN
    REQUIRE(s, "null argument");
    REQUIRE(d >= 1 && d <= 8, "replay depth: 1 … 8");
    return s->be->set_replay_depth_now(d);
    API_GUARD_END
}

int cgo_solver_set_lean_sums(cgo_solver *s, int32_t on) {
    API_GUARD_BEGIN
    REQUIRE(s, "null argument");
    s->be->set_lean_sums(on != 0);
    return CGO_OK;
    API_GUARD_END
}

int cgo_solver_probe_set_replay(cgo_solver *s, int32_t nrep, const double *a, const double *beta) {
    API_GUARD_BEGIN
    REQUIRE(s, "null argument");
    REQUIRE(nrep >= 0 && nrep <= 7 && (nrep == 0 || (a && beta)), "probe replay list: 0 … 7 (a*, β) pairs");
    s->be->set_probe_replay(nrep, a, beta);
    return CGO_OK;
    API_GUARD_END
}

int cgo_solver_probe_set_beta_prev(cgo_solver *s, double beta_prev) {
    API_GUARD_BEGIN
    REQUIRE(s, "null argument");
    s->be->set_probe_beta_prev(beta_prev);
    return CGO_OK;
    API_GUARD_END
}

int cgo_solver_profile_enable(cgo_solver *s, int32_t on) {
    API_GUARD_BEGIN
    REQUIRE(s, "null argument");
    s->be->profile_enable(on != 0);
    return CGO_OK;
    API_GUARD_END
}
int cgo_solver_profile_reset(cgo_solver *s) {
    API_GUARD_BEGIN
    REQUIRE(s, "null argument");
    s->be->profile_reset();
    return CGO_OK;
    API_GUARD_END
}
int cgo_solver_profile_get(cgo_solver *s, int32_t kind, int64_t *launches, double *ms, double *bytes) {
    API_GUARD_BEGIN
    REQUIRE(s && launches && ms && bytes, "null argument");
    s->be->profile_get(kind, launches, ms, bytes);
    return CGO_OK;
    API_GUARD_END
}

int cgo_minimize(cgo_ctx *ctx, cgo_objective *obj, const double *x0, const cgo_cg_config *cfg,
                 const cgo_ls_config *ls, cgo_results *out) {
    API_GUARD_BEGIN
    REQUIRE(x0 && out, "null argument");
    cgo_solver *s = nullptr;
    int rc = cgo_solver_create(ctx, obj, cfg, ls, &s);
    if (rc) return rc;
    rc = s->be->set_x0_host(x0);
    if (!rc) rc = s->sv->start();
    bool fin = false;
    while (!rc && !fin) rc = s->sv->iterate(INT64_MAX / 2, fin);
    if (!rc) rc = cgo_solver_results(s, out);
    std::string keep = get_error();
    cgo_solver_destroy(s);
    if (rc) set_error(keep);
    return rc;
    API_GUARD_END
}

int cgo_evalwolfeconditions(const cgo_ls_config *ls, double phi_a, double dphi_a, double a, double uu,
                            double phi_0, double dphi_0, int32_t *valid_large, int32_t *valid_small) {
    API_GUARD_BEGIN
    REQUIRE(ls && valid_large && valid_small, "null argument");
    REQUIRE(ls->cond_kind == CGO_COND_WOLFE || ls->cond_kind == CGO_COND_YUAN_WEI_LU, "not a Wolfe-type condition");
    if (ls->cond_kind == CGO_COND_WOLFE) {
        if (!(0.0 < ls->c1 && ls->c1 < ls->c2 && ls->c2 < 1.0)) { set_error("AssertionError: zero(T) < c1 < c2 < one(T)  (wolfe.jl:278)"); return CGO_EINVAL; }
    } else if (!(0.0 < ls->delta1 && ls->delta1 < ls->c1 && ls->c1 < ls->c2 && ls->c2 < 1.0)) {
        set_error("AssertionError: zero(T) < δ1 < c1 < c2 < one(T)  (wolfe.jl:233)"); return CGO_EINVAL;
    }
    bool okl = false, oks = false;
    wolfe_tests(*ls, phi_0, dphi_0, uu, phi_a, dphi_a, a, okl, oks);
    *valid_large = okl; *valid_small = oks;
    return CGO_OK;
    API_GUARD_END
}

int cgo_evalbacktrackcondition(const cgo_ls_config *ls, double phi_a, double a, double phi_0, double dphi_0,
                               int32_t *valid) {
    API_GUARD_BEGIN
    REQUIRE(ls && valid, "null argument");
// ... 924 lines not shown
```

conjugategradientoptim.jl_amd/csrc/cgo_engine.cpp:

```cpp
#include "cgo_engine.hpp"

#include <algorithm>
#include <cstring>

namespace cgo {

static const char *kStatusNames[CGO_NUM_STATUS] = {
    "incomplete",
    "success",
    "increasing_objective",
    "non_finite_objective_or_gradient_proposed",
    "max_iters_reached",
    "non_descent_search_direction",
    "linesearch_a_max_overflow",
    "linesearch_max_iters_reached",
    "zoom_max_iters_reached",
    "accepted_non_finite_iterate",
    "cannot_find_initial_feasible_step",
    "max_step_length_reached",
    "cannot_find_feasible_step",
    "step_bracket_precision_issue",
    "bisection_lower_bound_larger_than_proposed_step",
    "feasible",
    "infeasible",
// ... 52 lines not shown
            if (!(0.0 < l->delta1 && l->delta1 < l->c1 && l->c1 < l->c2 && l->c2 < 1.0)) {
                why = "AssertionError: zero(T) < δ1 < c1 < c2 < one(T)  (wolfe.jl:233)"; return CGO_EINVAL;
            }
        } else { why = "unknown Wolfe condition kind"; return CGO_EINVAL; }
        return CGO_OK;
    }
    if (l->kind == CGO_LS_BACKTRACKING) {
        if (l->cond_kind != CGO_COND_ARMIJO) { why = "Backtracking needs the Armijo condition"; return CGO_EINVAL; }
        if (!(0.0 < l->c1 && l->c1 < 1.0)) {
            why = "AssertionError: zero(T) < c1 < one(T)  (geometric.jl:169)"; return CGO_EINVAL;
        }
        if (!(l->discount_factor > 0.0 && std::isfinite(l->discount_factor))) { why = "discount_factor must be positive"; return CGO_EINVAL; }
        return CGO_OK;
    }
    why = "unknown LineSearchConfig kind";
    return CGO_EINVAL;
}

static inline TrialSums trial_sums(const Scal &t) { return TrialSums{t.f, t.gtu, t.gtgt, t.gtg, t.yy, t.uy, t.ygt}; }

int check_lss_config(const cgo_lss_config *l, std::string &why) {
    if (!l) { why = "null LinesearchSolveSys"; return CGO_EINVAL; }
    if (!(0.0 < l->rho && l->rho < 1.0)) { why = "AssertionError: zero(T) < ρ < one(T)  (solve_system.jl:21)"; return CGO_EINVAL; }
    if (!(l->s > 0.0)) { why = "AssertionError: s > zero(T)  (solve_system.jl:23)"; return CGO_EINVAL; }
    if (l->max_iters < 0) { why = "max_iters must be ≥ 0"; return CGO_EINVAL; }
    return CGO_OK;
}

int64_t lss_default_max_iters(double rho) { return (int64_t)std::nearbyint(std::log(1e-6) / std::log(rho)); }

double beta_from_scalars(const cgo_beta_config &b, const Scal &t, double gu_old, double gg_old,
                         double uu_old) {
    const TrialSums ts = trial_sums(t);
    return beta_from_sums(b.kind, b.mu, ts, gu_old, gg_old, uu_old, beta_norms_fast(ts, uu_old));
}

int Solver::robust_norm(double sumsq, int which, double &out) {
    if (sumsq >= 1e-280 && sumsq <= 1e300) { out = std::sqrt(sumsq); return CGO_OK; }
    double m = 0, ss = 0;
    bool has_nan = false;
    if (int rc = be_->scaled_norm_parts(which, last_eval_a_, m, ss, has_nan)) return rc;
    if (has_nan) out = NAN;
    else if (m == 0.0 || std::isinf(m)) out = m;
    else out = m * std::sqrt(ss);
    return CGO_OK;
}

Solver::Solver(VecBackend *be, const cgo_cg_config &cfg, const cgo_ls_config &ls)
    : be_(be), cfg_(cfg), ls_(ls) {}

Solver::Solver(VecBackend *be, const cgo_cg_config &cfg, const cgo_lss_config &lss)
    : be_(be), cfg_(cfg), ls_{}, sys_(true), lss_(lss) {}

int Solver::start() {
    Scal s;
    if (cfg_.beta.kind == CGO_BETA_LBFGS) {
        const int P = cfg_.beta.lbfgs_m + 1;
        int rc = be_->lbfgs_alloc(P);
        if (rc) return rc;
        qn_rho_.assign(P, 0.0);
        qn_list_.clear(); qn_free_ = 0; qn_gamma_ = 1.0;
        qn_gram_ = be_->lbfgs_gram_max_pairs() >= cfg_.beta.lbfgs_m;
        qn_SY_.assign((size_t)P * P, 0.0); qn_YY_.assign((size_t)P * P, 0.0);
        qn_sg_.assign(P, 0.0); qn_yg_.assign(P, 0.0);
    }
    if (sys_ && (cfg_.beta.kind >= CGO_BETA_LBFGS || !be_->sys_supported())) return CGO_EINVAL;
    int rc = be_->init_eval(s);
    if (rc) return rc;
    if (sys_ && (rc = be_->sys_begin())) return rc;
    total_evals_ = 1;
    f_x_ = s.f;
    f_x0_ = f_x_;
    gg_ = s.gtgt;
    if ((rc = robust_norm(gg_, 0, norm_df_x_))) return rc;
    dphi0_ = -gg_;
    uu_ = gg_;
    dir_is_neg_grad_ = true;
    a_initial_ = NAN;
    it_ = 0; iters_ran_ = 0; status_ = CGO_INCOMPLETE;
    ncache_ = 0; finished_ = false; started_ = true;
    qn_trial_done_ = false;
    res_fail_streak_ = 0; res_backoff_ = 0;
    tr_f_.clear(); tr_g_.clear(); tr_a_.clear(); tr_e_.clear(); log_.clear();
    return CGO_OK;
}

void Solver::finish(int64_t iters, int status) {
    iters_ran_ = iters;
    status_ = status;
    finished_ = true;
    ncache_ = 0;
    qn_trial_done_ = false;
    be_->discard_pending();
    if (cfg_.trace_enabled) {
        tr_f_.resize((size_t)iters); tr_g_.resize((size_t)iters);
        tr_a_.resize((size_t)iters); tr_e_.resize((size_t)iters);
    }
}

double Solver::first_step(double a_initial) const { return ls_first_step(ls_, a_initial); }

void Solver::first_hints(double a0, double (&h)[2]) const { ls_first_hints(ls_, a0, h[0], h[1]); }

int Solver::eval(double a, double &phi, double &dphi, double h1, double h2, double h3, double h4) {
    const double hs[4] = {h1, h2, h3, h4};
    return evaln(a, phi, dphi, hs, 4);
}

int Solver::evaln(double a, double &phi, double &dphi, const double *hs, int nh) {
    int hit = -1;
    for (int j = 0; j < ncache_; ++j)
        if (std::memcmp(&a, &cache_[j].a, sizeof(double)) == 0) { hit = j; break; }
    if (hit >= 0) {
        last_ = cache_[hit].s;
    } else {
        double pts[7] = {a, 0, 0, 0, 0, 0, 0};
        int k = 1;
        const int mp = sys_ ? be_->max_points() : std::min(be_->max_points(), 3);
        for (int q = 0; q < nh && k < mp; ++q) {
            const double h = hs[q];
            bool ok = std::isfinite(h) && h > 0.0;
            for (int j = 0; ok && j < k; ++j) ok = (h != pts[j]);
            if (ok) pts[k++] = h;
        }
        Scal out[7];
        if (int rc = be_->trial(pts, k, out)) return rc;
        ncache_ = k;
        for (int j = 0; j < k; ++j) cache_[j] = {pts[j], out[j]};
        last_ = out[0];
    }
    last_eval_a_ = a;
    total_evals_++;
    phi = last_.f;
    dphi = last_.gtu;
    if (log_on_) log_.push_back({a, phi, dphi});
    return CGO_OK;
}

int Solver::ls_strong_wolfe(double a_initial, LSOut &o) {
    auto ev = [this](double a, double &phi, double &dphi, double h1, double h2, double h3, double h4) {
        return eval(a, phi, dphi, h1, h2, h3, h4);
    };
    return ls_strong_wolfe_t(ls_, f_x_, dphi0_, a_initial, ev, o);
}

int Solver::find_feasible(double &a, double lb, int64_t &evals, double &phi, double &dphi,
                          int &flag, double h1, double h2, double h3, double h4) {
    auto ev = [this](double a_, double &phi_, double &dphi_, double g1, double g2, double g3, double g4) {
        return eval(a_, phi_, dphi_, g1, g2, g3, g4);
    };
    return ls_find_feasible_t(ls_, a, lb, evals, phi, dphi, flag, ev, h1, h2, h3, h4);
}

int Solver::ls_wolfe_bisection(double a_initial, LSOut &o) {
    auto ev = [this](double a, double &phi, double &dphi, double h1, double h2, double h3, double h4) {
        return eval(a, phi, dphi, h1, h2, h3, h4);
    };
    struct Bk {
        Solver *s;
        int is_neg_grad(bool &yes) {
            yes = s->dir_is_neg_grad_;
            if (!yes) {
                double ss = 0;
                if (int rc = s->be_->upg_sumsq(ss)) return rc;
                yes = (std::sqrt(ss) == 0.0);
            }
            return 0;
        }
        int reset_dir(double &uu) {
            Scal sc;
            if (int rc = s->be_->reset_dir(sc)) return rc;
            s->ncache_ = 0;
            uu = sc.uu;
            s->dphi0_ = sc.gu;
            s->dir_is_neg_grad_ = true;
            return 0;
        }
    } bk{this};
    return ls_wolfe_bisection_t(ls_, f_x_, dphi0_, uu_, a_initial, ev, bk, o);
}

int Solver::ls_backtracking(double a_initial, LSOut &o) {
    const double phi0 = f_x_, d0 = dphi0_, c1 = ls_.c1, rho = ls_.discount_factor;
    auto armijo = [&](double phi_a, double a) { return armijo_test(c1, phi_a, a, phi0, d0); };
    if (!std::isfinite(phi0)) { o = {phi0, 0.0, 0, CGO_ACCEPTED_NON_FINITE_ITERATE}; return CGO_OK; }
    if (d0 > 0.0) { o = {phi0, 0.0, 0, CGO_NON_DESCENT_SEARCH_DIRECTION}; return CGO_OK; }
    double a = a_initial;
    if (!std::isfinite(a)) a = std::fabs(phi0) / uu_;
    if (!std::isfinite(a)) a = 1.0;
    int64_t evals = 0;
    double phi = 0, dphi = 0;
    int flag = 0;
    if (int rc = find_feasible(a, 0.0, evals, phi, dphi, flag, a / rho, a * rho, a / rho / rho, a * rho * rho)) return rc;
    if (flag != CGO_FEASIBLE) { o = {phi0, 0.0, 0, CGO_CANNOT_FIND_INITIAL_FEASIBLE_STEP}; return CGO_OK; }
    ++evals;
    total_evals_++;
    if (log_on_) log_.push_back({a, phi, dphi});
    const bool divide = armijo(phi, a);
    double a_prev = a, phi_prev = phi;
    for (int64_t k = 0; k < ls_.max_iters; ++k) {
        a = divide ? a / rho : a * rho;
        if (!std::isfinite(a)) { o = {phi_prev, a_prev, evals, CGO_NON_FINITE_STEP_PROPOSED}; return CGO_OK; }
        if (a == a_prev) { o = {phi_prev, a_prev, evals, CGO_PROPOSED_STEP_SAME_AS_CURRENT_STEP}; return CGO_OK; }
        const double n1 = divide ? a / rho : a * rho, n2 = divide ? n1 / rho : n1 * rho, n3 = divide ? n2 / rho : n2 * rho;
        if (int rc = eval(a, phi, dphi, n1, n2, n3, divide ? n3 / rho : n3 * rho)) return rc;
        ++evals;
        if (!armijo(phi, a)) { o = {phi_prev, a_prev, evals, CGO_SUCCESS}; return CGO_OK; }
        a_prev = a;
        phi_prev = phi;
    }
    o = {phi, a, evals, CGO_LINESEARCH_MAX_ITERS_REACHED};
    return CGO_OK;
}

void Solver::qn_commit(int slot) {
    const int m = cfg_.beta.lbfgs_m;
    qn_list_.insert(qn_list_.begin(), slot);
    if ((int)qn_list_.size() > m) {
        qn_free_ = qn_list_.back();
        qn_list_.pop_back();
    } else {
        std::vector<char> used(m + 1, 0);
        for (int p : qn_list_) used[p] = 1;
        for (int p = 0; p <= m; ++p) if (!used[p]) { qn_free_ = p; break; }
    }
}

int Solver::qn_direction(Scal &s, double a_trial, Scal *trial) {
    const int c = (int)qn_list_.size(), P = cfg_.beta.lbfgs_m + 1;
    qn_trial_done_ = false;
    if (c == 0) return be_->reset_dir(s);
    const double gamma = qn_gamma_;
    if (!qn_gram_) return be_->lbfgs_direction(qn_list_.data(), qn_rho_.data(), c, gamma, s);
    const int *L = qn_list_.data();
    std::vector<double> a(c, 0.0), cc(c, 0.0), cy(c), cs(c);
    for (int k = 0; k < c; ++k) {
        double sq = qn_sg_[L[k]];
        for (int j = 0; j < k; ++j) sq -= a[j] * qn_SY_[(size_t)L[k] * P + L[j]];
        a[k] = qn_rho_[L[k]] * sq;
    }
    for (int k = c - 1; k >= 0; --k) {
        double yq = qn_yg_[L[k]];
        for (int j = 0; j < c; ++j) yq -= a[j] * qn_YY_[(size_t)L[k] * P + L[j]];
        double yr = gamma * yq;
        for (int j = c - 1; j > k; --j) yr += cc[j] * qn_SY_[(size_t)L[j] * P + L[k]];
        cc[k] = a[k] - qn_rho_[L[k]] * yr;
    }
    for (int k = 0; k < c; ++k) { cy[k] = gamma * a[k]; cs[k] = -cc[k]; }
    if (trial && std::isfinite(a_trial) && be_->lbfgs_direction_gram_can_fuse_trial()) {
        qn_trial_done_ = true;
        return be_->lbfgs_direction_gram_trial(L, cy.data(), cs.data(), c, -gamma, a_trial, s, *trial);
    }
    return be_->lbfgs_direction_gram(L, cy.data(), cs.data(), c, -gamma, s);
}

int Solver::run_resident(int64_t cap, int64_t &done, int &reason) {
    ResConfig c{};
    c.ls = ls_; c.eps = cfg_.eps; c.mu = cfg_.beta.mu; c.beta_kind = cfg_.beta.kind;
    c.npts = be_->max_points() >= 7 ? 7 : (be_->max_points() >= 3 ? 3 : 1);
    c.max_iters = cfg_.max_iters; c.log_on = log_on_ ? 1 : 0;
    ResState s{};
    s.f_x = f_x_; s.gg = gg_; s.norm = norm_df_x_; s.dphi0 = dphi0_; s.uu = uu_; s.a_initial = a_initial_;
    s.it = it_; s.dir_neg = dir_is_neg_grad_ ? 1 : 0;
    s.ncache = ncache_ <= RES_MAXP ? ncache_ : 0;
    for (int j = 0; j < s.ncache; ++j) { s.ca[j] = cache_[j].a; s.cs[j] = trial_sums(cache_[j].s); }
    if (int rc = be_->resident_run(c, s, cap, res_recs_, res_log_)) return rc;
    done = s.done; reason = s.reason;
    if (s.done > 0) adopt(s, res_recs_.data(), res_log_.data());
    return CGO_OK;
}

void Solver::adopt(const ResState &s, const ResRecord *recs, const ResLog *log) {
    {
        f_x_ = s.f_x; gg_ = s.gg; norm_df_x_ = s.norm; dphi0_ = s.dphi0; uu_ = s.uu; a_initial_ = s.a_initial;
        it_ = s.it; dir_is_neg_grad_ = s.dir_neg != 0;
        last_eval_a_ = s.last_a;
        total_evals_ += s.evals;
        if (cfg_.trace_enabled)
            for (int64_t i = 0; i < s.done; ++i) {
                const ResRecord &r = recs[(size_t)i];
                tr_f_.push_back(r.f); tr_g_.push_back(r.norm); tr_a_.push_back(r.a); tr_e_.push_back(r.evals);
            }
        if (log_on_) for (int64_t i = 0; i < s.log_len; ++i) log_.push_back({log[(size_t)i].a, log[(size_t)i].phi, log[(size_t)i].dphi});
        ncache_ = s.ncache;
        for (int j = 0; j < s.ncache; ++j) {
            Scal q; const TrialSums &t = s.cs[j];
            q.f = t.f; q.gtu = t.gtu; q.gtgt = t.gtgt; q.gtg = t.gtg; q.yy = t.yy; q.uy = t.uy; q.ygt = t.ygt;
            q.gu = s.dphi0; q.uu = s.uu;
            cache_[j] = {s.ca[j], q};
        }
    }
}

void Solver::resume(double f_x0, int64_t evals, const ResState &s, const ResRecord *recs) {
    total_evals_ = 1;
    f_x0_ = f_x0;
    iters_ran_ = 0; status_ = CGO_INCOMPLETE;
    ncache_ = 0; finished_ = false; started_ = true;
    qn_trial_done_ = false;
    res_fail_streak_ = 0; res_backoff_ = 0;
    tr_f_.clear(); tr_g_.clear(); tr_a_.clear(); tr_e_.clear(); log_.clear();
    ResState t = s;
    t.done = s.it; t.evals = evals; t.log_len = 0;
    adopt(t, recs, nullptr);
}

int Solver::iterate(int64_t iters, bool &finished) {
    if (!started_) return CGO_ESTATE;
    if (sys_) return iterate_sys(iters, finished);
    const bool qn = cfg_.beta.kind == CGO_BETA_LBFGS;
    const bool resident = !qn && be_->resident_ready(cfg_, ls_);
    bool host_next = false;
    for (int64_t budget = iters; budget > 0 && !finished_; --budget) {
        const int64_t n = it_ + 1;
        {
            int64_t ran = 0;
            const int st = stop_status(it_, cfg_.max_iters, f_x_, norm_df_x_, cfg_.eps, f_x0_, ran);
            if (st != CGO_INCOMPLETE) { finish(ran, st); break; }
        }
        if (resident && !host_next && res_backoff_ == 0 && be_->resident_ready(cfg_, ls_)) {
            int64_t done = 0;
            int reason = RES_HOST;
            if (int rc = run_resident(std::min(budget, cfg_.max_iters - it_), done, reason)) return rc;
            if (reason == RES_ERROR) return CGO_ECOMM;
            host_next = (reason == RES_HOST);
            if (done > 0) { res_fail_streak_ = 0; budget -= done - 1; continue; }
            res_fail_streak_ = std::min(res_fail_streak_ + 1, 6);
            res_backoff_ = (int64_t(1) << res_fail_streak_) - 2;
        } else if (res_backoff_ > 0) {
            --res_backoff_;
        }
        host_next = false;
        LSOut o{};
        int rc = (ls_.kind == CGO_LS_STRONG_WOLFE_BISECTION) ? ls_strong_wolfe(a_initial_, o)
                 : (ls_.kind == CGO_LS_WOLFE_BISECTION)      ? ls_wolfe_bisection(a_initial_, o)
                                                             : ls_backtracking(a_initial_, o);
        if (rc) return rc;
        ncache_ = 0;
        a_initial_ = o.a;
        if (o.status != CGO_SUCCESS) { finish(n - 1, o.status); break; }
        VecBackend::GramOut G;
        bool push_first = false;
        if (qn && qn_gram_) {
            if (be_->lbfgs_push_spec(last_eval_a_, o.a, qn_free_, qn_list_.data(), (int)qn_list_.size(), G)) {
                push_first = true;
            } else if (be_->two_phase() && be_->lbfgs_push_materializes(last_eval_a_)) {
                if ((rc = be_->lbfgs_push_gram(last_eval_a_, o.a, qn_free_, qn_list_.data(), (int)qn_list_.size(), G))) return rc;
                if (!G.materialized) return CGO_ESTATE;
                push_first = true;
            }
        }
        if (push_first) {
            last_.gtgt = G.gtgt;
        } else if (be_->two_phase() || qn_trial_done_) {
            if ((rc = be_->materialize(last_))) return rc;
        }
        double norm_df_xp = NAN;
        if ((rc = robust_norm(last_.gtgt, 1, norm_df_xp))) return rc;
        if (!std::isfinite(o.phi) || !std::isfinite(norm_df_xp)) {
            finish(n - 1, CGO_NON_FINITE_OBJECTIVE_OR_GRADIENT_PROPOSED);
            break;
        }
        double beta = 0.0;
        if (!qn) {
            const TrialSums ts = trial_sums(last_);
            BetaNorms bn = beta_norms_fast(ts, uu_);
            bn.gt = norm_df_xp;
            if (!beta_norms_fast_ok(cfg_.beta.kind, ts, uu_) && cfg_.beta.kind == CGO_BETA_YUAN_WANG_SHENG) {
                if ((rc = robust_norm(uu_, 3, bn.u))) return rc;
                if ((rc = robust_norm(ts.yy, 4, bn.y))) return rc;
            }
            beta = beta_from_sums(cfg_.beta.kind, cfg_.beta.mu, ts, dphi0_, gg_, uu_, bn);
        }
        f_x_ = o.phi;
        norm_df_x_ = norm_df_xp;
        gg_ = last_.gtgt;
        it_ = n;
        if (cfg_.trace_enabled) {
            tr_f_.push_back(f_x_); tr_g_.push_back(norm_df_x_);
            tr_a_.push_back(o.a); tr_e_.push_back(o.evals);
        }
        const bool will_stop = (n == cfg_.max_iters) ||
            (std::isfinite(f_x_) && std::isfinite(norm_df_x_) && norm_df_x_ < cfg_.eps);
        const double a_xp = last_eval_a_;
        Scal s;
        if (qn) {
            const int slot = qn_free_, c = (int)qn_list_.size(), P = cfg_.beta.lbfgs_m + 1;
            double sy = 0, yy = 0;
            if (qn_gram_) {
                if (push_first) rc = be_->lbfgs_push_commit(!will_stop);
                else rc = be_->lbfgs_push_gram(a_xp, o.a, slot, qn_list_.data(), c, G);
                if (rc) return rc;
                sy = G.sy; yy = G.yy;
                for (int j = 0; j < c; ++j) {
                    const int pj = qn_list_[j];
                    if (G.y_based) { qn_sg_[pj] += G.sjyn[j]; qn_yg_[pj] += G.yjyn[j]; }
                    else { qn_sg_[pj] = G.sjg[j]; qn_yg_[pj] = G.yjg[j]; }
                    if (sy > 0.0) {
                        qn_SY_[(size_t)pj * P + slot] = G.sjyn[j];
                        qn_SY_[(size_t)slot * P + pj] = G.yjsn[j];
                        qn_YY_[(size_t)pj * P + slot] = qn_YY_[(size_t)slot * P + pj] = G.yjyn[j];
                    }
                }
                if (sy > 0.0) {
                    qn_SY_[(size_t)slot * P + slot] = sy; qn_YY_[(size_t)slot * P + slot] = yy;
                    qn_sg_[slot] = G.sgn; qn_yg_[slot] = G.ygn;
                }
            } else {
                if ((rc = be_->lbfgs_push(a_xp, o.a, slot, sy, yy))) return rc;
            }
            if (sy > 0.0) {
                qn_rho_[slot] = 1.0 / sy;
                qn_gamma_ = sy / yy;
                qn_commit(slot);
            }
            if (!will_stop) {
                const double a0 = first_step(a_initial_);
                Scal t0;
                if ((rc = qn_direction(s, ls_.kind == CGO_LS_BACKTRACKING ? NAN : a0, &t0))) return rc;
                dphi0_ = s.gu; uu_ = s.uu;
                dir_is_neg_grad_ = qn_list_.empty();
                if (qn_trial_done_) { ncache_ = 1; cache_[0] = {a0, t0}; }
            }
        } else if (will_stop) {
            if ((rc = be_->accept_only(a_xp))) return rc;
        } else if (!std::isfinite(first_step(a_initial_))) {
            if ((rc = be_->accept_dir(a_xp, beta, s))) return rc;
            dphi0_ = s.gu; uu_ = s.uu;
            dir_is_neg_grad_ = (beta == 0.0);
        } else {
            double pts[7] = {0, 0, 0, 0, 0, 0, 0};
            int k;
            if (be_->max_points() >= 5) {
                k = ls_trial_points_n(ls_, first_step(a_initial_), be_->max_points() >= 7 ? 7 : 5, pts);
            } else {
                double p3[3];
                k = ls_trial_points(ls_, first_step(a_initial_), be_->max_points() >= 3, p3);
                for (int j = 0; j < 3; ++j) pts[j] = p3[j];
            }
            Scal out[7];
            if (be_->ctl_depth() > 0 && !be_->two_phase() && ls_.kind != CGO_LS_BACKTRACKING) {
                CtlConfig cc;
                cc.ls = ls_; cc.eps = cfg_.eps; cc.mu = cfg_.beta.mu;
                cc.beta_kind = cfg_.beta.kind; cc.maxp = be_->max_points();
                cc.max_iters = cfg_.max_iters;
                CtlState cs;
                cs.f_x = f_x_; cs.gg = gg_; cs.a_acc = a_xp; cs.beta = beta;
                for (int j = 0; j < CTL_MAXP; ++j) cs.a[j] = pts[j < k ? j : k - 1];
                cs.npts = k; cs.go = 1; cs.it = it_;
                rc = be_->accept_dir_trial_ctl(cc, cs, budget, out);
            } else {
                rc = be_->accept_dir_trial(a_xp, beta, pts, k, out);
            }
            if (rc) return rc;
            dphi0_ = out[0].gu; uu_ = out[0].uu;
            dir_is_neg_grad_ = (beta == 0.0);
            ncache_ = k;
            for (int j = 0; j < k; ++j) cache_[j] = {pts[j], out[j]};
        }
    }
    finished = finished_;
    return CGO_OK;
}

int check_batch_config(const cgo_cg_config &cfg, const cgo_ls_config &ls, std::string &why) {
    if (cfg.beta.kind == CGO_BETA_LBFGS) { why = "batched solves: β = L-BFGS is not supported (CG flavours only)"; return CGO_EINVAL; }
    if (cfg.beta.kind == CGO_BETA_BROYDEN_FAMILY) { why = "batched solves: β = Broyden family is not supported (CG flavours only)"; return CGO_EINVAL; }
    if (ls.kind == CGO_LS_BACKTRACKING) { why = "batched solves: the Backtracking line search is not supported (StrongWolfeBisection or WolfeBisection)"; return CGO_EINVAL; }
    return CGO_OK;
}

int run_batch(VecBackend *be, const cgo_cg_config &cfg, const cgo_ls_config &ls, int64_t batch, int64_t slice_iters, BatchRun &out) {
    ResConfig c{};
    c.ls = ls; c.eps = cfg.eps; c.mu = cfg.beta.mu; c.beta_kind = cfg.beta.kind;
    c.npts = 3; c.max_iters = cfg.max_iters; c.log_on = 0;
    const int64_t budget = slice_iters > 0 ? slice_iters : 64;
    out.evals.assign((size_t)batch, 0);
    out.launches = 0;
    std::vector<char> live((size_t)batch, 1);
    for (;;) {
        if (int rc = be->batch_launch(c, budget, out.st, out.f_x0)) return rc;
        out.launches++;
        if ((int64_t)out.st.size() != batch || (int64_t)out.f_x0.size() != batch) return CGO_ESTATE;
        bool any = false;
        for (int64_t b = 0; b < batch; ++b) {
            if (!live[(size_t)b]) continue;
            const ResState &s = out.st[(size_t)b];
            out.evals[(size_t)b] += s.evals;
            if (s.reason == RES_STOP || s.reason == RES_HOST) live[(size_t)b] = 0;
            else if (s.reason == RES_BUDGET && s.done > 0) any = true;
            else return CGO_ESTATE;
        }
        if (!any) break;
    }
    return CGO_OK;
}

int Solver::iterate_sys(int64_t iters, bool &finished) {
    for (int64_t budget = iters; budget > 0 && !finished_; --budget) {
        const int64_t n = it_ + 1;
        if (n > cfg_.max_iters) { finish(cfg_.max_iters, CGO_MAX_ITERS_REACHED); break; }
        if (norm_df_x_ < cfg_.eps) { finish(n - 1, CGO_SUCCESS); break; }
        const double s0 = lss_.s, rho = lss_.rho;
        double a = NAN, phi = NAN, dphi = NAN, nrm = NAN;
        int64_t hit = -1;
        int rc;
        for (int64_t i = 0; i < lss_.max_iters; ++i) {
            a = s0 * std::pow(rho, (double)i);
            double nxt[6];
            for (int q = 0; q < 6; ++q) nxt[q] = (i + 1 + q < lss_.max_iters) ? s0 * std::pow(rho, (double)(i + 1 + q)) : NAN;
            if ((rc = evaln(a, phi, dphi, nxt, 6))) return rc;
            if ((rc = robust_norm(last_.gtgt, 1, nrm))) return rc;
            if (!(-dphi < lss_.sigma * a * nrm * uu_)) { hit = i; break; }
        }
        ncache_ = 0;
        if (hit < 0) { finish(n - 1, CGO_LINESEARCH_FAILED); break; }
        if (nrm < cfg_.eps) {
            f_x_ = phi; norm_df_x_ = nrm; it_ = n;
            if (cfg_.trace_enabled) { tr_f_.push_back(phi); tr_g_.push_back(nrm); tr_a_.push_back(a); tr_e_.push_back(hit); }
            if ((rc = be_->accept_only(a))) return rc;
            finish(n, CGO_SUCCESS);
            break;
        }
        const double m = a * last_.gtu / (nrm * nrm);
        Scal p;
        if ((rc = be_->sys_project(a, m, p))) return rc;
        total_evals_++;
        double nrm_next = NAN;
        if ((rc = robust_norm(p.gtgt, 2, nrm_next))) return rc;
        if (!std::isfinite(p.f) || !std::isfinite(nrm_next)) {
            finish(n - 1, CGO_NON_FINITE_OBJECTIVE_OR_GRADIENT_PROPOSED);
            break;
        }
        if ((rc = be_->sys_commit())) return rc;
        f_x_ = p.f;
        double beta;
        {
            const TrialSums ts = trial_sums(p);
            BetaNorms bn = beta_norms_fast(ts, uu_);
            bn.gt = nrm_next;
            beta = beta_from_sums(cfg_.beta.kind, cfg_.beta.mu, ts, dphi0_, gg_, uu_, bn);
        }
        gg_ = p.gtgt;
        norm_df_x_ = nrm_next;
        it_ = n;
// ... 25 lines not shown
```

conjugategradientoptim.jl_amd/csrc/cgo_engine.hpp:

```cpp
#pragma once

#include <cmath>
#include <cstdint>
#include <memory>
#include <string>
#include <vector>

#include "../../include/cgo.h"
#include "cgo_ctl.hpp"
#include "cgo_resident.hpp"

namespace cgo {

struct Scal {
    double f = 0;
    double gtu = 0;
    double gtgt = 0;
    double gtg = 0;
    double yy = 0;
    double uy = 0;
    double ygt = 0;
    double gu = 0;
    double uu = 0;
};

enum KernelKind : int {
    KK_INIT = 0,
    KK_TRIAL,
    KK_ACCEPT_DIR_TRIAL,
    KK_ACCEPT_DIR,
    KK_ACCEPT_ONLY,
    KK_RESET_DIR,
    KK_UPG_NORM,
    KK_LBFGS_PUSH,
    KK_LBFGS_LOOP,
    KK_LBFGS_FINAL,
    KK_LSE_STATS,
    KK_LSE_GRAD,
    KK_SCALED_NORM,
    KK_DIR_TRIAL,
    KK_SYS_PROJECT,
    KK_RESIDENT,
    KK_ACCEPT_TRIAL_NOSTORE,
    KK_MATERIALIZE_XU,
    KK_ACCEPT_TRIAL_LAZY,
    KK_MATERIALIZE_U,
    KK_COUNT
};

struct Comm {
    int rank = 0, world = 1;
    virtual ~Comm() {}
    virtual int allgather_host(const double *send, double *recv, int count) = 0;
    virtual int allgather_device(const double *, double *, int, void * ) { return -1; }
    virtual int kind() const { return 3; }
    virtual int ranks_seen() { return world; }
    virtual double *shm_slot_host(int , int ) { return nullptr; }
    virtual double *shm_slot_dev(int , int ) { return nullptr; }
    virtual int connect_devices() { return 0; }
    virtual double *dev_mailbox(int ) { return nullptr; }
};

struct VecBackend {
    virtual ~VecBackend() {}
    virtual int64_t n_local() const = 0;
    virtual int set_x0_host(const double *x0) = 0;
    virtual int set_x0_fill(int kind, uint64_t seed, double lo, double hi) = 0;
    virtual int init_eval(Scal &out) = 0;
    virtual int max_points() const { return 1; }
    virtual int trial(const double *a, int k, Scal *out) = 0;
    virtual int accept_dir_trial(double a_acc, double beta, const double *a, int k, Scal *out) = 0;
    virtual int ctl_depth() const { return 0; }
    virtual int accept_dir_trial_ctl(const CtlConfig &, const CtlState &s, int64_t , Scal *out) {
        return accept_dir_trial(s.a_acc, s.beta, s.a, s.npts, out);
    }
    virtual bool resident_ready(const cgo_cg_config &, const cgo_ls_config &) const { return false; }
    virtual int resident_run(const ResConfig &, ResState &, int64_t , std::vector<ResRecord> &, std::vector<ResLog> &) { return CGO_EINVAL; }
    virtual int batch_launch(const ResConfig &, int64_t , std::vector<ResState> & , std::vector<double> & ) { return CGO_EINVAL; }
    virtual bool sys_supported() const { return false; }
    virtual int sys_begin() { return CGO_EINVAL; }
    virtual int sys_project(double , double , Scal &) { return CGO_EINVAL; }
    virtual int sys_commit() { return CGO_EINVAL; }
    virtual int dir_trial(double , const double * , int , Scal *) { return CGO_EINVAL; }
    virtual int accept_dir(double a_acc, double beta, Scal &out) = 0;
    virtual int accept_only(double a_acc) = 0;
    virtual int reset_dir(Scal &out) = 0;
    virtual int upg_sumsq(double &out) = 0;
    virtual int lbfgs_push(double a_x, double a_s, int slot, double &sy, double &yy) = 0;
    virtual int lbfgs_direction(const int *slots, const double *rho, int count, double gamma,
                                Scal &out) = 0;
    virtual int lbfgs_alloc(int slots) = 0;
    virtual int lbfgs_gram_max_pairs() const { return 0; }
    struct GramOut {
        double sy, yy, sgn, ygn;
        double sjg[16], yjg[16], sjyn[16], yjsn[16], yjyn[16];
        bool materialized = false;
        bool y_based = false;
        double gtgt = 0.0;
    };
    virtual int lbfgs_push_gram(double, double, int, const int *, int, GramOut &) { return CGO_EINVAL; }
    virtual bool lbfgs_push_materializes(double ) { return false; }
    virtual int lbfgs_push_commit(bool ) { return CGO_OK; }
    virtual bool lbfgs_push_spec(double , double , int , const int * , int , GramOut &) { return false; }
    virtual int lbfgs_direction_gram(const int *, const double *, const double *, int, double, Scal &) { return CGO_EINVAL; }
    virtual bool lbfgs_direction_gram_can_fuse_trial() const { return false; }
    virtual int lbfgs_direction_gram_trial(const int *, const double *, const double *, int, double, double , Scal & , Scal & ) { return CGO_EINVAL; }
    virtual bool two_phase() const { return false; }
    virtual void discard_pending() {}
    virtual int materialize(Scal &) { return 0; }
    virtual int download(double *x, double *g) = 0;
    virtual int scaled_norm_parts(int which, double a_trial, double &maxabs, double &scaled_ss, bool &has_nan) = 0;
    virtual void profile_enable(bool) {}
    virtual void profile_reset() {}
    virtual void profile_get(int, int64_t *launches, double *ms, double *bytes) {
        *launches = 0; *ms = 0; *bytes = 0;
    }
    virtual int64_t launches() const { return 0; }
};

const char *status_name(int s);
const char *kernel_kind_name(int k);
int check_cg_config(const cgo_cg_config *c, std::string &why);
int check_ls_config(const cgo_ls_config *l, std::string &why);
int check_lss_config(const cgo_lss_config *l, std::string &why);
int64_t lss_default_max_iters(double rho);

double beta_from_scalars(const cgo_beta_config &b, const Scal &t, double gu_old, double gg_old,
                         double uu_old);

struct TrialRecord { double a, phi, dphi; };

class Solver {
  public:
    Solver(VecBackend *be, const cgo_cg_config &cfg, const cgo_ls_config &ls);
    Solver(VecBackend *be, const cgo_cg_config &cfg, const cgo_lss_config &lss);
    int start();
    int iterate(int64_t iters, bool &finished);
    double objective() const { return f_x_; }
    int64_t iters_ran() const { return iters_ran_; }
    int status() const { return status_; }
    bool finished() const { return finished_; }
    int64_t total_evals() const { return total_evals_; }
    const std::vector<double> &trace_objective() const { return tr_f_; }
    const std::vector<double> &trace_grad_norm() const { return tr_g_; }
    const std::vector<double> &trace_step_size() const { return tr_a_; }
    const std::vector<int64_t> &trace_evals() const { return tr_e_; }
    const std::vector<TrialRecord> &trial_log() const { return log_; }
    void set_log_enabled(bool on) { log_on_ = on; }
    VecBackend *backend() { return be_; }
    const cgo_cg_config &config() const { return cfg_; }
    const cgo_ls_config &linesearch() const { return ls_; }
    bool is_sys() const { return sys_; }
    void resume(double f_x0, int64_t evals, const ResState &s, const ResRecord *recs);

  private:
    void adopt(const ResState &s, const ResRecord *recs, const ResLog *log);
    int eval(double a, double &phi, double &dphi, double h1 = NAN, double h2 = NAN, double h3 = NAN, double h4 = NAN);
    int evaln(double a, double &phi, double &dphi, const double *hints, int nh);
    void first_hints(double a0, double (&h)[2]) const;
    int ls_strong_wolfe(double a_initial, LSOut &o);
    int ls_wolfe_bisection(double a_initial, LSOut &o);
    int ls_backtracking(double a_initial, LSOut &o);
    int find_feasible(double &a, double lb, int64_t &evals, double &phi, double &dphi,
                      int &flag, double h1 = NAN, double h2 = NAN, double h3 = NAN, double h4 = NAN);
    double first_step(double a_initial) const;
    int robust_norm(double sumsq, int which, double &out);
    void finish(int64_t iters, int status);
    int iterate_sys(int64_t iters, bool &finished);
    int run_resident(int64_t cap, int64_t &done, int &reason);
    std::vector<ResRecord> res_recs_;
    int res_fail_streak_ = 0;
    int64_t res_backoff_ = 0;
    std::vector<ResLog> res_log_;

    VecBackend *be_;
    cgo_cg_config cfg_;
    cgo_ls_config ls_;
    bool sys_ = false;
    cgo_lss_config lss_{};
    bool started_ = false, finished_ = false;
    double f_x_ = NAN, f_x0_ = NAN, norm_df_x_ = NAN, gg_ = NAN;
    double a_initial_ = NAN;
    int64_t it_ = 0;
    int64_t iters_ran_ = 0;
    int status_ = CGO_INCOMPLETE;
    double dphi0_ = NAN, uu_ = NAN;
    bool dir_is_neg_grad_ = true;
    struct Cached { double a; Scal s; };
    Cached cache_[7];
    int ncache_ = 0;
    Scal last_;
    double last_eval_a_ = NAN;
    int64_t total_evals_ = 0;
    std::vector<int> qn_list_;
    int qn_free_ = 0;
    std::vector<double> qn_rho_;
    double qn_gamma_ = 1.0;
    bool qn_gram_ = false;
    std::vector<double> qn_SY_, qn_YY_, qn_sg_, qn_yg_;
    int qn_direction(Scal &s, double a_trial = NAN, Scal *trial = nullptr);
    bool qn_trial_done_ = false;
    void qn_commit(int slot);
    std::vector<double> tr_f_, tr_g_, tr_a_;
    std::vector<int64_t> tr_e_;
    std::vector<TrialRecord> log_;
    bool log_on_ = false;
};

struct BatchRun {
    std::vector<ResState> st;
    std::vector<double> f_x0;
    std::vector<int64_t> evals;
    int64_t launches = 0;
};
int check_batch_config(const cgo_cg_config &cfg, const cgo_ls_config &ls, std::string &why);
int run_batch(VecBackend *be, const cgo_cg_config &cfg, const cgo_ls_config &ls, int64_t batch, int64_t slice_iters, BatchRun &out);

}
```

conjugategradientoptim.jl_amd/csrc/cgo_hip_backend.hip:

```cpp
#include "cgo_backend_internal.hpp"

#include "cgo_kernels.hip.hpp"
#include "cgo_kernels_lse.hip.hpp"
#include "cgo_kernels_cg.hip.hpp"
#include "cgo_kernels_chain.hip.hpp"

namespace cgo {

using namespace dev;

static double wait_timeout_ns() {
    static const double t = [] { const char *e = getenv("CGO_WAIT_TIMEOUT_S"); double v = e ? atof(e) : 0.0; return (v > 0.0 ? v : 120.0) * 1e9; }();
    return t;
}

static thread_local std::string g_err;
void set_error(const std::string &msg) { g_err = msg; }
const char *get_error() { return g_err.c_str(); }


int DevBuf::alloc(size_t count) {
    release();
    if (count == 0) count = 1;
    HIPCHK(hipMalloc((void **)&p, count * sizeof(double)));
// ... 687 lines not shown
    if (probe_stored_) {
        probe_note(nullptr, 0, "%s", fused_symbol(obj_tname(), mode, is_big(obj_->kind, mode, obj_->n_local, obj_->nparams(), pol_.hbm_stream_bytes)).c_str());
        if (fetch) probe_append(sums, NS);
    }
    if (prof_on_) prof_commit(kk, bytes_for(obj_->kind, mode, obj_->n_local, obj_->nparams()));
    return CGO_OK;
}

static void unpack(const double *s, Scal &o, bool trial, bool dir) {
    if (trial) {
        o.f = s[S_F]; o.gtu = s[S_GTU]; o.gtgt = s[S_GTGT]; o.gtg = s[S_GTG];
        o.yy = s[S_YY]; o.uy = s[S_UY]; o.ygt = s[S_YGT];
    }
    if (dir) { o.gu = s[S_GU]; o.uu = s[S_UU]; }
}

int HipBackend::init_eval(Scal &out) {
    if (int rc = flush_lite()) return rc;
    if (rmode_) {
        double s[NR7];
        if (chain() && !ctx_->single()) {
            if (int rc = launch_r(KK_INIT, R_EDGES, 0, 0, nullptr, 0, true, s)) return rc;
        }
        if (int rc = launch_rk(KK_INIT, 0, 0, nullptr, 0, true, s)) return rc;
        out = Scal();
        out.f = s[RS_F]; out.gtgt = s[RS_GTGT];
        return CGO_OK;
    }
    if (obj_->host_closure()) return host_trial(0.0, true, out);
    if (obj_->two_phase()) {
        out = Scal();
        if (int rc = lse_stats(LM_NOU, 0, 0, 0, out, false)) return rc;
        const double f = out.f;
        if (int rc = lse_grad(true, 0.0, out)) return rc;
        out.f = f;
        std::swap(g_, gt_);
        return CGO_OK;
    }
    double s[NS];
    if (int rc = launch_k(KK_INIT, 0, 0, 0, true, s)) return rc;
    std::swap(g_, gt_);
    out = Scal();
    out.f = s[S_F];
    out.gtgt = s[S_GTGT];
    return CGO_OK;
}

int HipBackend::trial(const double *a, int k, Scal *out) {
    if (rmode_) {
        double s[NR7];
        if (int rc = trial_r(a, k, s)) return rc;
        unpack_r(s, k, out, false);
        return CGO_OK;
    }
    if (obj_->host_closure()) return host_trial(a[0], false, out[0]);
    if (obj_->two_phase()) return lse_stats(0, 0, 0, a[0], out[0], false);
    if (int rc = flush_lite()) return rc;
    spec_valid_ = false; spec_unmat_ = false;
    double s[NS];
    if (int rc = launch_k(KK_TRIAL, 0, 0, a[0], true, s)) return rc;
    unpack(s, out[0], true, false);
    return CGO_OK;
}

int HipBackend::accept_dir_trial(double a_acc, double beta, const double *a, int k, Scal *out) {
    if (rmode_) {
        double s[NR7];
        if (int rc = accept_dir_trial_r(a_acc, beta, a, k, s)) return rc;
        unpack_r(s, k, out, true);
        return CGO_OK;
    }
    double s[NS];
    if (obj_->host_closure()) {
        Scal d;
        if (int rc = accept_dir(a_acc, beta, d)) return rc;
        if (int rc = host_trial(a[0], false, out[0])) return rc;
        out[0].gu = d.gu; out[0].uu = d.uu;
        return CGO_OK;
    }
    std::swap(g_, gt_);
    if (obj_->two_phase()) return lse_stats(LM_ACCEPT | LM_DIR, a_acc, beta, a[0], out[0], true);
    if (int rc = launch_k(KK_ACCEPT_DIR_TRIAL, a_acc, beta, a[0], true, s)) return rc;
    unpack(s, out[0], true, true);
    return CGO_OK;
}

int HipBackend::accept_dir(double a_acc, double beta, Scal &out) {
    if (rmode_) {
        double s[NR7];
        if (int rc = launch_rk(KK_ACCEPT_DIR, a_acc, beta, nullptr, 0, true, s)) return rc;
        out.gu = s[RS_PER_POINT]; out.uu = s[RS_PER_POINT + 1];
        return CGO_OK;
    }
    double s[NS];
    std::swap(g_, gt_);
    if (int rc = launch_k(KK_ACCEPT_DIR, a_acc, beta, 0, true, s)) return rc;
    unpack(s, out, false, true);
    return CGO_OK;
}

int HipBackend::accept_only(double a_acc) {
    if (rmode_) return launch_rk(KK_ACCEPT_ONLY, a_acc, 0, nullptr, 0, false, nullptr);
    std::swap(g_, gt_);
    return launch_k(KK_ACCEPT_ONLY, a_acc, 0, 0, false, nullptr);
}

int HipBackend::reset_dir(Scal &out) {
    if (int rc = flush_lite()) return rc;
    if (rmode_) {
        double s[NR7];
        if (int rc = launch_rk(KK_RESET_DIR, 0, 0, nullptr, 0, true, s)) return rc;
        out.gu = s[RS_PER_POINT]; out.uu = s[RS_PER_POINT + 1];
        return CGO_OK;
    }
    double s[NS];
    if (int rc = launch_k(KK_RESET_DIR, 0, 0, 0, true, s)) return rc;
    unpack(s, out, false, true);
    return CGO_OK;
}

int HipBackend::upg_sumsq(double &out) {
    if (rmode_) {
        double s[NR7];
        if (int rc = launch_rk(KK_UPG_NORM, 0, 0, nullptr, 0, true, s)) return rc;
        out = s[RS_PER_POINT + 1];
        return CGO_OK;
    }
    double s[NS];
    if (int rc = launch_k(KK_UPG_NORM, 0, 0, 0, true, s)) return rc;
    out = s[S_UU];
    return CGO_OK;
}

int HipBackend::sys_begin() {
    if (!rmode_) { set_error("solvesystem needs an element-wise objective (k_cg kernel family)"); return CGO_EINVAL; }
    if (int rc = pipe_drain()) return rc;
    if (int rc = materialize_lag()) return rc;
    sys_on_ = true;
    HIPCHK(hipSetDevice(ctx_->device));
    if (int rc = ensure_gb()) return rc;
    HIPCHK(hipMemcpyAsync(xn_, xc_, sizeof(double) * (size_t)obj_->n_local, hipMemcpyDeviceToDevice, ctx_->stream));
    return CGO_OK;
}

int HipBackend::sys_project(double a, double m, Scal &out) {
    double s[NR7];
    const double a1[1] = {a};
    if (int rc = launch_rk(KK_SYS_PROJECT, 0.0, m, a1, 1, true, s)) return rc;
    unpack_r(s, 1, &out, false);
    return CGO_OK;
}

int HipBackend::sys_commit() { std::swap(xc_, xn_); return CGO_OK; }

int HipBackend::dir_trial(double beta, const double *a, int k, Scal *out) {
    double s[NR7];
    if (k <= 0) {
        if (int rc = launch_r(KK_DIR_TRIAL, R_DIR, 0.0, beta, nullptr, 0, true, s)) return rc;
        out[0].gu = s[RS_PER_POINT]; out[0].uu = s[RS_PER_POINT + 1];
        return CGO_OK;
    }
    if (int rc = launch_rk(KK_DIR_TRIAL, 0.0, beta, a, k, true, s)) return rc;
    unpack_r(s, k, out, true);
    return CGO_OK;
}

// ... 314 lines not shown
```

conjugategradientoptim.jl_amd/csrc/cgo_hip_backend.hpp:

```cpp
#pragma once

#include <hip/hip_runtime.h>

#include <memory>
#include <string>
#include <vector>

#include "cgo_engine.hpp"
#include "cgo_launch_kinds.hpp"
#include "cgo_rtc.hpp"

namespace cgo {

namespace dev { struct CtlArgs; struct Tail; struct LoopParams; struct ResParams; struct BatchParams; struct BatchLbfgsParams; }

void set_error(const std::string &msg);
const char *get_error();

struct DevBuf {
    double *p = nullptr;
    size_t n = 0;
    DevBuf() {}
    DevBuf(const DevBuf &) = delete;
    DevBuf &operator=(const DevBuf &) = delete;
// ... 117 lines not shown
    int64_t resident_iters() const { return res_iters_; }
    int64_t resident_slices() const { return res_slices_; }
    int64_t resident_gave_up() const { return res_gave_up_; }
    static int64_t batch_max_n(HipCtx *ctx, int obj_kind, const RtcModule *rtc = nullptr);
    int batch_begin(int64_t batch, int64_t n, const double *x0, const double *const *params, int64_t max_iters, bool trace);
    int batch_alloc(int64_t batch, int64_t n, const double *const *params, bool device_rows = false);
    static int64_t batch_rows_max_n();
    static int batch_rows_unroll();
    static int batch_rows_block();
    static double batch_rows_bytes(int64_t batch, int64_t n, int nparams);
    bool batch_device_rows() const { return bat_rows_; }
    int batch_reset(const double *x0, const double *scalars, const unsigned char *active, int64_t max_iters, bool trace);
    int batch_launch(const ResConfig &c, int64_t budget, std::vector<ResState> &st, std::vector<double> &f_x0) override;
    int batch_records(int64_t b, int64_t count, std::vector<ResRecord> &out);
    int64_t batch_rec_stride() const { return bat_rec_stride_; }
    int batch_export_row(int64_t b, HipBackend &dst, bool with_u);
    int batch_export_slots(int64_t b, HipBackend &dst);
    int batch_results(double *x , double *g , const unsigned char *active = nullptr);
    int batch_lbfgs_alloc(int m, bool lds = false);
    int batch_lbfgs_reset(int m = 0);
    int batch_lbfgs_m() const { return bat_m_; }
    static int64_t batch_lbfgs_max_n();
    static int batch_lbfgs_unroll();
    static int batch_lbfgs_unroll_for(int nparams);
    static int batch_lbfgs_block();
    static double batch_lbfgs_bytes(int64_t batch, int64_t n, int nparams, int m);
    static int batch_lbfgs_lds_rows(int nparams, int m);
    static int batch_lbfgs_lds_unroll_for(int nparams);
    static int64_t batch_lbfgs_lds_ld_of(int64_t max_lds, int64_t static_lds, int rows);
    static int64_t batch_lbfgs_lds_max_ld(HipCtx *ctx, int obj_kind, int m, const RtcModule *rtc = nullptr);
    bool batch_lbfgs_in_lds() const { return bat_qn_lds_; }
    int batch_probe(cgo_batch_probe_args &p);
    int64_t push_count(int kind) const { return push_counts_[kind]; }
    bool sys_supported() const override { return rmode_; }
    int sys_begin() override;
    int sys_project(double a, double m, Scal &out) override;
    int sys_commit() override;
    int dir_trial(double beta, const double *a, int k, Scal *out) override;
    int accept_dir(double a_acc, double beta, Scal &out) override;
    int accept_only(double a_acc) override;
    int reset_dir(Scal &out) override;
    int upg_sumsq(double &out) override;
    int lbfgs_alloc(int slots) override;
    int lbfgs_gram_max_pairs() const override { return gram_on_ ? 12 : 0; }
    int lbfgs_push_gram(double a_x, double a_s, int slot, const int *prev, int count, GramOut &out) override;
    bool lbfgs_push_materializes(double a_x) override;
    bool lbfgs_push_spec(double a_x, double a_s, int slot, const int *prev, int count, GramOut &out) override;
    int lbfgs_push_commit(bool direction_follows) override;
    int lbfgs_direction_gram(const int *slots, const double *cy, const double *cs, int count, double cg,
                             Scal &out) override;
    bool lbfgs_direction_gram_can_fuse_trial() const override;
    int lbfgs_direction_gram_trial(const int *slots, const double *cy, const double *cs, int count, double cg, double a_trial,
                                   Scal &dir, Scal &trial) override;
    int lbfgs_push(double a_x, double a_s, int slot, double &sy, double &yy) override;
    int lbfgs_direction(const int *slots, const double *rho, int count, double gamma,
                        Scal &out) override;
    bool two_phase() const override { return obj_->two_phase(); }
    int materialize(Scal &out) override;
    void discard_pending() override { push_pending_ = false; push_lite_pending_ = false; lite_deferred_ = false; spec_valid_ = false; spec_unmat_ = false; }
    int download(double *x, double *g) override;
    int scaled_norm_parts(int which, double a_trial, double &maxabs, double &scaled_ss, bool &has_nan) override;
    void profile_enable(bool on) override;
    void profile_reset() override;
    void profile_get(int kind, int64_t *launches, double *ms, double *bytes) override;
    int64_t launches() const override { return total_launches_; }
    void set_need_beta(bool b) { need_beta_ = b; }
    void set_rmode(bool on) { rmode_ = on; }
    void set_multi_min_n(int64_t n) { multi_min_n_ = n; }
    void set_multi5_min_n(int64_t n) { multi5_min_n_ = n; }
    void set_multi7_min_n(int64_t n) { multi7_min_n_ = n; }
    void set_three_point_band(int64_t lo, int64_t hi) { band3_lo_ = lo; band3_hi_ = hi; }
    bool rmode() const { return rmode_; }
    void set_lazy_direction(bool on) { lazy_on_ = on; }
    bool lazy_direction() const { return lazy_on_; }
    int set_lazy_direction_now(bool on) { if (!on) { if (int rc = materialize_lag()) return rc; } lazy_on_ = on; return 0; }
    void set_probe_beta_prev(double b) { probe_beta_prev_ = b; }
    void set_replay_depth(int d) { replay_depth_ = d < 1 ? 1 : (d > 8 ? 8 : d); }
    int replay_depth() const { return replay_depth_; }
    int set_replay_depth_now(int d);
    void set_probe_replay(int nrep, const double *a, const double *beta);
    void set_beta_unread(int bits) { lean_mask_ = bits; if (lean_bits_) lean_bits_ = bits; }
    void set_lean_sums(bool on) { lean_bits_ = on ? lean_mask_ : 0; }
    bool lean_sums() const { return lean_bits_ != 0; }
    std::string kernel_symbol(int kernel_kind) const;
    int probe_launch(int kernel_kind, int variant, double a_acc, double beta, const double *a, int k, const double *x,
                     const double *u, const double *aux, double *sums, int sums_cap, int *sums_len, double *x_out,
                     double *u_out, double *g_out, std::string &symbol);
    bool probed() const { return probe_; }
    int probe_launch_stored(int kernel_kind, int variant, double a_acc, double beta, const double *a, int k, const double *x,
                            const double *u, const double *aux, double *sums, int sums_cap, int *sums_len, double *x_out,
                            double *u_out, double *g_out, std::string &symbol);
    int probe_lbfgs(int m, cgo_lbfgs_probe &p, const double *x, const double *u, const double *g, const double *gt, const double *S,
                    const double *Y, double *x_out, double *xo_out, double *u_out, double *g_out, double *gt_out, double *S_out,
                    double *Y_out);

    int probe_resident(const cgo_cg_config &cfg, const cgo_ls_config &ls, cgo_resident_probe &p, const double *x, const double *u,
                       double *rows, int64_t rows_cap, double *x_out, double *u_out);

    int probe_armed(const cgo_cg_config &cfg, const cgo_ls_config &ls, cgo_armed_probe &p, const double *x, const double *u,
                    double *x_out, double *u_out);

    static int run_dir(HipCtx *ctx, double *u_host, const double *g_host, double beta, int64_t n,
                       double *out2);
    static int run_beta_partials(HipCtx *ctx, const double *gn, const double *g, const double *u,
                                 int64_t n, double *out9);
    static int run_trial(HipObjective *obj, const double *x, const double *u, double a,
                         double *gn_out, double *out2);
    static int run_eval(HipObjective *obj, const double *x, double *g_out, double *f);
    static int bench_kernel(HipCtx *ctx, HipObjective *obj, int kernel_kind, int64_t n, int reps,
                            double *ms, double *bytes);
    static int bench_stream_mix(HipCtx *ctx, int64_t n, int reps, double *median_us, double *best_us);

  private:
    int launch(int kk, int mode, double a_acc, double beta, double a_trial, bool fetch,
               double *sums );
    int launch_k(int kk, double a_acc, double beta, double a_trial, bool fetch, double *sums) { return launch(kk, fused_mode(kk), a_acc, beta, a_trial, fetch, sums); }
    HipCtx *ctx_;
    HipObjective *obj_;
    DevBuf x_, u_, ga_, gb_;
    DevBuf x2_, u2_;
    double *uc_ = nullptr;
    double *xalt_ = nullptr, *ualt_ = nullptr;
    int pingpong_ = -1;
    bool sys_on_ = false;
    bool chain() const { return obj_->kind == CGO_OBJ_ROSENBROCK_CHAINED; }
    bool probe_ = false;
    double probe_row_[64] = {};
    int probe_len_ = 0;
    int last_mode_ = -1, last_npts_ = 0;
    bool last_big_ = false;
    int probe_prepare();
    int probe_slack_intact();
    std::string r_symbol(int mode, int npts, bool big) const;
    std::string probe_syms_;
    void probe_note(const double *row, int len, const char *fmt, ...);
    int probe_ring_slack_intact();
    bool probe_stored_ = false;
    void probe_append(const double *row, int len);
    const char *obj_tname() const;
    int launch_loop(const dev::LoopParams &P, int kk, double nvec, bool big, int grid);
    double halo_xl_[2] = {0, 0}, halo_ul_[2] = {0, 0}, halo_xr_[2] = {0, 0}, halo_ur_[2] = {0, 0};
    int launch_chain_kernel(int mode, double a_acc, double beta, const double *a, int k, int npts, bool big, int grid, const dev::Tail &tail);
    bool tail_fused(int grid) const;
    bool pipe_fused(int grid) const;
    dev::Tail make_tail(bool on);
    bool pingpong_ready();
    int tune_placement();
    double place_first_us_ = 0.0, place_best_us_ = 0.0;
    int place_candidates_ = 0;
    double place_cap_bytes_ = 0.0;
    bool placed_ = false;
    int ensure_ga();
    int ensure_gb();
    double *xc_ = nullptr, *xn_ = nullptr;
    double *g_ = nullptr, *gt_ = nullptr;
    bool need_beta_ = true;
    bool rmode_ = false;
    int64_t multi_min_n_ = 3000000;
    int64_t multi5_min_n_ = INT64_MAX;
    int64_t multi7_min_n_ = INT64_MAX;
    int64_t band3_lo_ = 0, band3_hi_ = 0;
    int launch_r(int kk, int mode, double a_acc, double beta, const double *a, int k, bool fetch, double *sums);
    int launch_rk(int kk, double a_acc, double beta, const double *a, int k, bool fetch, double *sums) { return launch_r(kk, r_mode_of(kk), a_acc, beta, a, k, fetch, sums); }
    RPlan r_plan(int mode, int npts) const;
    bool adt_is_big() const;
    int fused_mode(int kk) const { const MKind *mk = m_kind(kk); return !mk ? -1 : ((kk == KK_TRIAL && !need_beta_) ? mk->alt : mk->mode); }
    std::string lbfgs_symbol(int kk) const;
    bool lazy_on_ = false, u_lag_ = false;
    double beta_lag_ = 0.0, probe_beta_prev_ = 0.0;
    bool lazy_eligible() const;
    int materialize_u();
    int replay_depth_ = 1, rep_n_ = 0, probe_rep_n_ = 0;
    double rep_a_[7] = {}, rep_b_[7] = {}, probe_rep_a_[7] = {}, probe_rep_b_[7] = {};
    int materialize_lag();
    int lean_mask_ = 0, lean_bits_ = 0;
    int lean_for(int mode) const;
    int accept_dir_trial_r(double a_acc, double beta, const double *a, int k, double *s);
    int trial_r(const double *a, int k, double *s);
    int launch_r_kernel(int kk, int mode, double a_acc, double beta, const double *a, int k, int npts,
                        const struct dev::CtlArgs *ctl, RPlan *plan_out);
    int ctl_depth_ = 0;
    unsigned long long epoch_ = 0;
    void *ctl_dev_ = nullptr;
    void *ctl_rec_ = nullptr;
    unsigned long long *ctl_seq_ = nullptr;
    unsigned long long pipe_enq_ = 0, pipe_done_ = 0;
    bool pipe_stopped_ = false;
    bool pipe_checked_ = false;
    bool ctl_fused_ = true;
    cgo_solver_policy pol_;
    int pipe_npts_ = 1;
    int64_t pipe_streak_ = 0;
    int64_t pipe_served_ = 0;
    std::vector<std::pair<int, unsigned>> pipe_prof_;
    unsigned prof_gen_ = 0;
    int pipe_alloc();
    int pipe_round_kernels();
    int pipe_finalize_ctl(const double *src, int nrows, int ns);
    int pipe_enqueue_round();
    int pipe_launch_graph(int rounds);
    int pipe_enqueue(int64_t count);
    struct PipeGraph { void *exec; int rounds, npts; double *x, *u; const double *p0; int64_t n; std::string syms; };
    std::vector<PipeGraph> graphs_;
    bool graph_on_ = false;
    bool capturing_ = false;
    unsigned long long pipe_batches_ = 0;
    int64_t graph_rounds_ = 0;
    int pipe_wait(unsigned long long id, CtlRecord &rec);
    int pipe_drain();
    int accept_dir_trial_keep_streak(const CtlState &s0, Scal *out);
    bool res_on_ = true;
    int res_grid_ = 0, res_npts_ = 3;
    int64_t res_chunk_ = 0;
    size_t res_lds_ = 0;
    int res_plan();
    int res_alloc();
    void res_out_buffers(double *&xo, double *&uo) const;
    void res_fill_params(dev::ResParams &P, double *xo, double *uo);
    void res_swap_in(double *xo, double *uo);
    int res_error_reset();
    ResState *res_state_ = nullptr;
    ResRecord *res_recs_ = nullptr;
    ResLog *res_log_ = nullptr;
    ResRecord *res_recs_dev_ = nullptr;
    ResLog *res_log_dev_ = nullptr;
    double *res_xbuf_ = nullptr;
    unsigned int *res_err_ = nullptr;
    DevBuf res_xo_, res_uo_;
    double *res_xin_ = nullptr, *res_uin_ = nullptr;
    unsigned long long *res_done_ = nullptr;
    unsigned long long res_seq_ = 0, res_round_ = 0;
    void *res_pr_script_ = nullptr, *res_pr_out_ = nullptr;
    double *res_pr_rows_ = nullptr;
    bool res_pr_ready_ = false;
    int64_t res_iters_ = 0, res_slices_ = 0, res_gave_up_ = 0;
    int64_t bat_count_ = 0, bat_n_ = 0, bat_ld_ = 0, bat_rec_stride_ = 0;
    bool bat_trace_ = false;
    size_t bat_lds_ = 0;
    bool bat_rows_ = false;
    ResState *bat_st_ = nullptr;
    ResRecord *bat_recs_ = nullptr;
    double *bat_fx0_ = nullptr;
    double *bat_s0v_ = nullptr;
    bool bat_s0v_on_ = false;
    size_t bat_recs_cap_ = 0;
    void batch_fill_rows(std::vector<double> &rows, const double *src) const;
    int batch_recs_reserve(int64_t stride);
    int batch_grad_rows();
    void batch_fill_params(dev::BatchParams &B, const ResConfig &c, int64_t budget) const;
    void batch_lbfgs_fill_params(dev::BatchLbfgsParams &L, const ResConfig &c, int64_t budget) const;
    int bat_m_ = 0;
    double *bat_S_ = nullptr, *bat_Y_ = nullptr;
    QnState *bat_qn_ = nullptr;
    int batch_lbfgs_launch(const ResConfig &c, int64_t budget, std::vector<ResState> &st, std::vector<double> &f_x0);
    bool bat_qn_lds_ = false;
    int batch_lbfgs_lds_on();
    int batch_lbfgs_lds_launch(const dev::BatchLbfgsParams &L);
    bool prof_on_ = false;
    struct ProfSlot { hipEvent_t e0 = nullptr, e1 = nullptr; int kk = -1; double bytes = 0; };
// ... 64 lines not shown
```

include/cgo.h:

```cpp
#ifndef CGO_H
#define CGO_H

#include <stdint.h>

#ifdef __cplusplus
extern "C" {
#endif

#define CGO_VERSION 100

enum {
    CGO_OK = 0,
    CGO_EINVAL = 1,
    CGO_EHIP = 2,
    CGO_ECOMM = 3,
    CGO_ENODEV = 4,
    CGO_ESTATE = 5,
    CGO_ENOMEM = 6
};

enum {
    CGO_INCOMPLETE = 0,
    CGO_SUCCESS = 1,
    CGO_INCREASING_OBJECTIVE = 2,
// ... 264 lines not shown
    int32_t size;
    int32_t rows;
    int32_t reserved[6];
} cgo_batch_policy;
void cgo_batch_policy_init(cgo_batch_policy *p);
int cgo_minimize_batch_ex(cgo_ctx *ctx, int32_t obj_kind, int64_t n, int64_t batch, const double *x0, const double *param0,
                          const cgo_cg_config *cfg, const cgo_ls_config *ls, int64_t slice_iters,
                          const cgo_batch_policy *policy, cgo_batch_results *out, int32_t *rows_used);
int cgo_minimize_batch_obj_ex(cgo_ctx *ctx, cgo_objective *model, int64_t batch, const double *x0,
                              const double *const *params, int32_t n_params,
                              const cgo_cg_config *cfg, const cgo_ls_config *ls, int64_t slice_iters,
                              const cgo_batch_policy *policy, cgo_batch_results *out, int32_t *rows_used);
int cgo_batch_open_ex(cgo_ctx *ctx, cgo_objective *model, int64_t batch, const double *const *params, int32_t n_params,
                      const cgo_batch_policy *policy, cgo_batch **handle);
int cgo_batch_rows(const cgo_batch *handle, int32_t *rows_used);
int64_t cgo_batch_max_n_ex(cgo_ctx *ctx, int32_t obj_kind, const cgo_batch_policy *policy);
int64_t cgo_batch_max_n_obj_ex(cgo_objective *model, const cgo_batch_policy *policy);
void cgo_batch_rows_shape(int32_t *block, int32_t *pairs_per_trip);
int cgo_minimize_batch_lbfgs(cgo_ctx *ctx, int32_t obj_kind, int64_t n, int64_t batch, const double *x0, const double *param0,
                             const cgo_cg_config *cfg, const cgo_ls_config *ls, int64_t slice_iters, cgo_batch_results *out);
int32_t cgo_batch_lbfgs_max_m(void);
int64_t cgo_batch_lbfgs_max_n(cgo_ctx *ctx, int32_t obj_kind);
void cgo_batch_lbfgs_shape(int32_t *block, int32_t *pairs_per_trip);
int cgo_minimize_batch_lbfgs_obj(cgo_ctx *ctx, cgo_objective *model, int64_t batch, const double *x0 ,
                                 const double *const *params , int32_t n_params,
                                 const double *scalars ,
                                 const cgo_cg_config *cfg, const cgo_ls_config *ls, int64_t slice_iters, cgo_batch_results *out);
int64_t cgo_batch_lbfgs_max_n_obj(cgo_objective *model);
void cgo_batch_lbfgs_shape_obj(int32_t n_params, int32_t *block, int32_t *pairs_per_trip);
int cgo_minimize_batch_lbfgs_ex(cgo_ctx *ctx, int32_t obj_kind, int64_t n, int64_t batch, const double *x0, const double *param0,
                                const cgo_cg_config *cfg, const cgo_ls_config *ls, int64_t slice_iters,
                                const cgo_batch_policy *policy, cgo_batch_results *out, int32_t *rows_used);
int cgo_minimize_batch_lbfgs_obj_ex(cgo_ctx *ctx, cgo_objective *model, int64_t batch, const double *x0,
                                    const double *const *params, int32_t n_params, const double *scalars,
                                    const cgo_cg_config *cfg, const cgo_ls_config *ls, int64_t slice_iters,
                                    const cgo_batch_policy *policy, cgo_batch_results *out, int32_t *rows_used);
int64_t cgo_batch_lbfgs_max_n_ex(cgo_ctx *ctx, int32_t obj_kind, int32_t m, const cgo_batch_policy *policy);
int64_t cgo_batch_lbfgs_max_n_obj_ex(cgo_objective *model, int32_t m, const cgo_batch_policy *policy);
int32_t cgo_batch_lbfgs_lds_rows(int32_t n_params, int32_t m);
void cgo_batch_lbfgs_lds_shape(int32_t n_params, int32_t *block, int32_t *pairs_per_trip);
int cgo_batch_lbfgs_open(cgo_ctx *ctx, cgo_objective *model, int64_t batch, const double *const *params, int32_t n_params,
                         int32_t m_max, const cgo_batch_policy *policy , cgo_batch **handle);
int cgo_batch_lbfgs_solve(cgo_batch *handle, const double *x0 , const double *scalars ,
                          const unsigned char *active , const cgo_cg_config *cfg, const cgo_ls_config *ls,
                          int64_t slice_iters , cgo_batch_results *out);
int cgo_batch_lbfgs_m(const cgo_batch *handle, int32_t *m_max);
#define CGO_BATCH_PROBE_MAX_PASSES 32
typedef struct cgo_batch_pass {
    int32_t kind, k;
    double a[7];
    double a_acc, beta;
    int32_t co_set, co_count;
    double co_gamma, co_cy[10], co_cs[10];
} cgo_batch_pass;
typedef struct cgo_batch_pass_out {
    double ts[7][7];
    double gu, uu;
    int64_t width, stored;
} cgo_batch_pass_out;
typedef struct cgo_batch_probe_args {
    int32_t tier, obj_kind, m, n_params;
    cgo_objective *model;
    int64_t n, batch;
    const double *x, *u;
    const double *params[4];
    const double *scalars;
    const unsigned char *skip;
    const double *S, *Y;
    const void *qn;
    int32_t npass, reserved;
    cgo_batch_pass pass[CGO_BATCH_PROBE_MAX_PASSES];
    double *rows;
    cgo_batch_pass_out *out;
    double *x_out, *u_out, *g_out, *S_out, *Y_out;
    void *qn_out;
    int32_t *reason;
    int64_t *done, *passes;
    int32_t points, reserved2;
    int64_t ld;
    char symbol[128];
} cgo_batch_probe_args;
int cgo_batch_probe(cgo_ctx *ctx, cgo_batch_probe_args *p);
int64_t cgo_batch_probe_qn_bytes(void);
int32_t cgo_stop_status(int64_t it, int64_t max_iters, double f_x, double grad_norm, double eps, double f_x0, int64_t *iters_ran);

int cgo_kernel_dir(cgo_ctx *ctx, double *u, const double *g, double beta, int64_t n,
                   double *out2);
int cgo_kernel_beta_partials(cgo_ctx *ctx, const double *g_next, const double *g,
                             const double *u, int64_t n, double *out9);
int cgo_getbeta(cgo_ctx *ctx, const cgo_beta_config *b, const double *g_next, const double *g,
                const double *u, int64_t n, double *beta);
int cgo_kernel_trial(cgo_objective *obj, const double *x, const double *u, double a,
                     double *g_next_out, double *out2);
int cgo_solver_probe_set_beta_prev(cgo_solver *s, double beta_prev);
int cgo_solver_probe_set_replay(cgo_solver *s, int32_t nrep, const double *a, const double *beta);
int cgo_solver_probe_launch(cgo_solver *s, int32_t kernel_kind, int32_t variant, double a_acc, double beta,
                            const double *a, int32_t k,
                            const double *x, const double *u, const double *aux,
                            double *sums, int32_t sums_cap, int32_t *sums_len,
                            double *x_out, double *u_out, double *g_out,
                            char *symbol, int32_t symbol_cap);
typedef struct cgo_lbfgs_probe {
    int32_t pass, slot, count, list[16];
    double a, a_s, a_trial, cg, M, S;
    double cy[16], cs[16];
    int32_t deferred_push, lite_slot;
    double a_lite, a_s_lite, M_lite, S_lite;
    int32_t loop_mode, final_step, apply_scale, k, q_from_g, v_ring, v_slot, w_ring, w_slot, dot_count;
    double rho, scale, dot_host;
    const double *dots;
    double alpha[64];
    int32_t spec_check, spec_slot, spec_count, spec_list[16];
    double spec_a_x, spec_a_s;
    int32_t spec_ok, new_in_list, sums_len, reserved;
    double gram[85];
    double sums[64];
    char symbol[256];
} cgo_lbfgs_probe;
int cgo_solver_probe_lbfgs(cgo_solver *s, cgo_lbfgs_probe *p,
                           const double *x, const double *u, const double *g, const double *gt, const double *S, const double *Y,
                           double *x_out, double *xo_out, double *u_out, double *g_out, double *gt_out, double *S_out, double *Y_out);
#define CGO_RESIDENT_PROBE_MAX_PASSES 32
typedef struct cgo_resident_pass {
    int32_t kind, k;
    double a[7];
    double a_acc, beta;
} cgo_resident_pass;
typedef struct cgo_resident_pass_out {
    double ts[7][7];
    double gu, uu;
    int64_t width;
} cgo_resident_pass_out;
typedef struct cgo_resident_probe {
    int32_t npass, reserved;
    cgo_resident_pass pass[CGO_RESIDENT_PROBE_MAX_PASSES];
    int32_t grid, points;
    int64_t chunk, round0;
    uint32_t err_word;
    int32_t wrote_back;
    cgo_resident_pass_out out[CGO_RESIDENT_PROBE_MAX_PASSES];
    char symbol[128];
} cgo_resident_probe;
int cgo_solver_probe_resident(cgo_solver *s, cgo_resident_probe *p, const double *x, const double *u,
                              double *rows, int64_t rows_cap, double *x_out, double *u_out);
#define CGO_ARMED_PROBE_MAX_ROUNDS 32
typedef struct cgo_ctl_state {
    double f_x, gg, a_acc, beta, a[7];
    int32_t npts, go;
    int64_t it;
} cgo_ctl_state;
typedef struct cgo_ctl_args {
    double a_acc, beta, a[7];
    int64_t go;
} cgo_ctl_args;
typedef struct cgo_ctl_record {
    double sums[56], a_acc, beta, a[7];
    int32_t npts, accepted;
    int64_t xwait;
} cgo_ctl_record;
typedef struct cgo_armed_probe {
    int32_t rounds, form, use_eps, reserved;
    int64_t max_iters;
    double eps;
    cgo_ctl_state st;
    double row[56];
    int32_t width, maxp;
// ... 19 lines not shown
```

Baseline: 2165.

## Predict line-search trial path for quadratic objectives and evaluate only needed points

For diagonal-quadratic objectives with PR-CG and Wolfe bisection line searches, the host runs the line search against a quadratic model built from the previous iteration's curvature to predict which trial steps will actually be visited. The fused accept/direction/trial kernel then evaluates only that predicted number of points through a new templated k_cg_path kernel, instead of the full seven-point tree. If the real search asks for a step that is not in the prediction, the full tree is evaluated again. The replay depth default is also raised from 6 to 8, which changes how many accepted steps are deferred before x and u are materialized.

```diff
diff --git a/conjugategradientoptim.jl_amd/_lib.py b/conjugategradientoptim.jl_amd/_lib.py
--- a/conjugategradientoptim.jl_amd/_lib.py
+++ b/conjugategradientoptim.jl_amd/_lib.py
@@ -195,6 +195,10 @@
     "cgo_solver_probe_set_beta_prev": (C.c_int, [_vp, C.c_double]),
     "cgo_solver_set_replay_depth": (C.c_int, [_vp, C.c_int32]),
     "cgo_solver_set_lean_sums": (C.c_int, [_vp, C.c_int32]),
+    "cgo_solver_set_path_prediction": (C.c_int, [_vp, C.c_int32]),
+    "cgo_solver_path_stats": (C.c_int, [_vp, i64p, i64p, i64p, i64p]),
+    "cgo_solver_probe_set_path": (C.c_int, [_vp, C.c_int32]),
+    "cgo_solver_debug_set_path_skew": (C.c_int, [_vp, C.c_double]),
     "cgo_solver_probe_set_replay": (C.c_int, [_vp, C.c_int32, dp, dp]),
     "cgo_solver_kernel_symbol": (C.c_int, [_vp, C.c_int32, C.c_char_p, C.c_int32]),
     "cgo_evalwolfeconditions": (C.c_int, [C.POINTER(LSConfigC), C.c_double, C.c_double, C.c_double, C.c_double,
diff --git a/conjugategradientoptim.jl_amd/api.py b/conjugategradientoptim.jl_amd/api.py
--- a/conjugategradientoptim.jl_amd/api.py
+++ b/conjugategradientoptim.jl_amd/api.py
@@ -667,8 +667,20 @@
     def set_lean_sums(self, on: bool):
         check(_lib.lib().cgo_solver_set_lean_sums(self._h, int(bool(on))))
 
+    def set_path_prediction(self, on: bool):
+        check(_lib.lib().cgo_solver_set_path_prediction(self._h, int(bool(on))))
+
+    def path_stats(self):
+        by = (C.c_int64 * 8)()
+        p, t, m = C.c_int64(0), C.c_int64(0), C.c_int64(0)
+        check(_lib.lib().cgo_solver_path_stats(self._h, by, C.byref(p), C.byref(t), C.byref(m)))
+        return dict(by_nact={j: int(by[j]) for j in (1, 2, 3, 4, 5, 7)}, predicted=p.value, tree=t.value, misses=m.value)
+
+    def debug_set_path_skew(self, factor: float):
+        check(_lib.lib().cgo_solver_debug_set_path_skew(self._h, float(factor)))
+
     def probe_launch(self, kind_name: str, variant: int, a_acc: float, beta: float, a: Sequence[float], x, u=None, aux=None,
-                     beta_prev: Optional[float] = None, replay: Optional[Sequence] = None):
+                     beta_prev: Optional[float] = None, replay: Optional[Sequence] = None, path_nact: Optional[int] = None):
         L = _lib.lib()
         kk = [L.cgo_kernel_kind_name(k).decode() for k in range(L.cgo_num_kernel_kinds())].index(kind_name)
         if beta_prev is not None:
@@ -677,6 +689,8 @@
             ra = np.ascontiguousarray([p[0] for p in replay], dtype=np.float64)
             rb = np.ascontiguousarray([p[1] for p in replay], dtype=np.float64)
             check(L.cgo_solver_probe_set_replay(self._h, len(replay), ra.ctypes.data_as(dp), rb.ctypes.data_as(dp)))
+        if path_nact is not None:
+            check(L.cgo_solver_probe_set_path(self._h, int(path_nact)))
         n = self.obj.n_local
         vec = lambda v: None if v is None else np.ascontiguousarray(v, dtype=np.float64)
         x, u, aux = vec(x), vec(u), vec(aux)
diff --git a/conjugategradientoptim.jl_amd/csrc/cgo_backend_cg.hip b/conjugategradientoptim.jl_amd/csrc/cgo_backend_cg.hip
--- a/conjugategradientoptim.jl_amd/csrc/cgo_backend_cg.hip
+++ b/conjugategradientoptim.jl_amd/csrc/cgo_backend_cg.hip
@@ -2,6 +2,7 @@
 
 #include "cgo_kernels.hip.hpp"
 #include "cgo_kernels_cg.hip.hpp"
+#include "cgo_kernels_cg_path.hip.hpp"
 #include "cgo_kernels_chain.hip.hpp"
 #include "cgo_kernels_lse.hip.hpp"
 #include "cgo_kernels_resident.hip.hpp"
@@ -49,6 +50,31 @@
     return -1;
 }
 
+template <class Obj>
+static int launch_cg_path(int mode, int nact, const RParams &P, int grid, hipStream_t st) {
+#define ROW(MODE, NACT) if (mode == (MODE) && nact == (NACT)) { k_cg_path<Obj, (MODE), (NACT), true><<<grid, BLOCK, 0, st>>>(P); return 0; }
+    CGO_CG_PATH_ROWS(ROW)
+#undef ROW
+    return -1;
+}
+static inline bool path_row(int mode, int nact) {
+#define ROW(MODE, NACT) if (mode == (MODE) && nact == (NACT)) return true;
+    CGO_CG_PATH_ROWS(ROW)
+#undef ROW
+    return false;
+}
+static inline bool path_objective(int kind) {
+#define ROW(KIND, T) if (kind == KIND) return true;
+    CGO_OBJ_CURV_ROWS(ROW)
+#undef ROW
+    return false;
+}
+bool HipBackend::path_rows() const {
+    if (!path_on_ || !path_objective(obj_->kind) || replay_depth_ < 2 || !lazy_eligible()) return false;
+    const int mode_n = r_mode_of(KK_ACCEPT_TRIAL_NOSTORE), mode_s = R_REPLAY | R_ADT;
+    return path_row(mode_n | lean_for(mode_n), MAXP) && path_row(mode_s | lean_for(mode_s), MAXP);
+}
+
 static inline bool lean_row(int mode) {
 #define ROW(MODE, MAXPTS) if (mode == (MODE)) return true;
     CGO_CG_LEAN_ROWS(ROW)
@@ -86,7 +112,7 @@
     }
     if (rep_n_ > 0 && !(mode & R_REPLAY)) { if (int rc = materialize_lag()) return rc; }
     RPlan plan;
-    const int npts = npts_for(k);
+    const int npts = path_nact_ ? MAXP : npts_for(k);
     if (int rc = launch_r_kernel(kk, mode, a_acc, beta, a, k, npts, nullptr, &plan)) return rc;
     const int grid = plan.grid;
     total_launches_++;
@@ -136,7 +162,10 @@
 int HipBackend::materialize_u() {
     if (!u_lag_) return CGO_OK;
     const int64_t asked = total_launches_;
+    const int nact = path_nact_;
+    path_nact_ = 0;
     const int rc = launch_rk(KK_MATERIALIZE_U, 0.0, 0.0, nullptr, 0, false, nullptr);
+    path_nact_ = nact;
     total_launches_ = asked;
     if (rc) return rc;
     u_lag_ = false;
@@ -147,7 +176,10 @@
     if (int rc = materialize_u()) return rc;
     if (rep_n_ == 0) return CGO_OK;
     const int64_t asked = total_launches_;
+    const int nact = path_nact_;
+    path_nact_ = 0;
     const int rc = launch_rk(KK_MATERIALIZE_XU, 0.0, 0.0, nullptr, 0, false, nullptr);
+    path_nact_ = nact;
     total_launches_ = asked;
     if (rc) return rc;
     rep_n_ = 0;
@@ -173,11 +205,13 @@
         if (rep_n_ < replay_depth_ - 1 && rep_n_ < RMAX) {
             const int mode_n = r_mode_of(KK_ACCEPT_TRIAL_NOSTORE);
             if (int rc = launch_r(KK_ACCEPT_TRIAL_NOSTORE, mode_n | lean_for(mode_n), a_acc, beta, a, k, true, s)) return rc;
+            if (path_nact_) { path_last_n_ = path_nact_; path_count_[path_nact_]++; }
             rep_a_[rep_n_] = a_acc; rep_b_[rep_n_] = beta; rep_n_++;
             return CGO_OK;
         }
         const int mode_s = R_REPLAY | R_ADT;
         if (int rc = launch_r(KK_ACCEPT_DIR_TRIAL, mode_s | lean_for(mode_s), a_acc, beta, a, k, true, s)) return rc;
+        if (path_nact_) { path_last_s_ = path_nact_; path_count_[path_nact_]++; }
         rep_n_ = 0;
         return CGO_OK;
     }
@@ -224,7 +258,8 @@
     const bool has_sums = r_has_sums(mode);
     const RPlan plan = *plan_out = r_plan(mode, npts);
     const bool big = plan.big; const int grid = plan.grid;
-    last_mode_ = mode; last_npts_ = plan.npts; last_big_ = big;
+    last_mode_ = mode; last_npts_ = plan.npts; last_big_ = big; last_nact_ = path_nact_;
+    if (path_nact_ && (chain() || !big || ctl || !path_row(mode, path_nact_) || !path_objective(obj_->kind))) { set_error("internal: not a path row"); return CGO_EINVAL; }
     if (chain()) {
         if (int rc = prof_begin(kk)) return rc;
         if (int rc = launch_chain_kernel(mode, a_acc, beta, a, k, plan.npts, big, grid, make_tail(has_sums && !ctl && tail_fused(grid)))) return rc;
@@ -259,7 +294,14 @@
     hipStream_t st = ctx_->stream;
     if (int rc = prof_begin(kk)) return rc;
     int r = -2;
-    switch (obj_->kind) {
+    if (path_nact_) {
+        switch (obj_->kind) {
+#define ROW(KIND, T) case KIND: r = launch_cg_path<T>(mode, path_nact_, P, grid, st); break;
+        CGO_OBJ_CURV_ROWS(ROW)
+#undef ROW
+        default: break;
+        }
+    } else switch (obj_->kind) {
 #define ROW(KIND, T) case KIND: r = big ? launch_cg<T, true>(mode, npts, P, grid, st) : launch_cg<T, false>(mode, npts, P, grid, st); break;
     CGO_OBJ_ROWS(ROW)
 #undef ROW
@@ -309,9 +351,10 @@
     return CGO_OK;
 }
 
-std::string HipBackend::r_symbol(int mode, int npts, bool big) const {
+std::string HipBackend::r_symbol(int mode, int npts, bool big, int nact) const {
     char buf[160];
     if (chain()) snprintf(buf, sizeof buf, "k_chain<%d, %d, %s>", mode, npts, big ? "true" : "false");
+    else if (nact) snprintf(buf, sizeof buf, "k_cg_path<%s, %d, %d, true>", obj_tname(), mode, nact);
     else snprintf(buf, sizeof buf, "k_cg<%s, %d, %d, %s>", obj_tname(), mode, npts, big ? "true" : "false");
     return buf;
 }
@@ -334,6 +377,10 @@
     }
     const RPlan plan = r_plan(mode, rk->pts == PTS_ONE ? 1 : npts_for(rk->pts == PTS_MAX ? max_points() : std::min(max_points(), 3)));
     if ((mode & R_REPLAY) && (mode & R_ACCEPT)) mode |= lean_for(mode);
+    if ((mode & R_REPLAY) && (mode & R_ACCEPT) && path_rows()) {
+        const int last = kk == KK_ACCEPT_TRIAL_NOSTORE ? path_last_n_ : path_last_s_;
+        return r_symbol(mode, plan.npts, plan.big, last ? last : MAXP);
+    }
     return r_symbol(mode, plan.npts, plan.big);
 }
 
@@ -676,6 +723,8 @@
                              const double *u, const double *aux, double *sums, int sums_cap, int *sums_len, double *x_out,
                              double *u_out, double *g_out, std::string &symbol) {
     *sums_len = 0;
+    const int want_nact = probe_nact_;
+    probe_nact_ = 0;
     const bool lse = obj_->two_phase();
     if (k < 0 || k > MAXP || (k > 0 && !a)) { set_error("probe: 0 ≤ k ≤ 7 trial steps"); return CGO_EINVAL; }
     if (!rmode_ && !lse) return probe_launch_stored(kk, variant, a_acc, beta, a, k, x, u, aux, sums, sums_cap, sums_len, x_out, u_out, g_out, symbol);
@@ -746,10 +795,15 @@
         symbol = buf;
     } else {
         double s[64];
+        if (want_nact) {
+            if (!path_row(mode, want_nact) || !path_objective(obj_->kind) || k > want_nact) { rep_n_ = 0; set_error("probe: not a path row of this solver, or more steps than it evaluates"); return CGO_EINVAL; }
+            path_nact_ = want_nact;
+        }
         rc = launch_r(kk, mode, a_acc, beta, a, k, true, s);
+        path_nact_ = 0;
         rep_n_ = 0;
         if (rc) return rc;
-        symbol = r_symbol(last_mode_, last_npts_, last_big_);
+        symbol = r_symbol(last_mode_, last_npts_, last_big_, last_nact_);
     }
     HIPCHK(hipStreamSynchronize(st));
     if (x_out) HIPCHK(hipMemcpyAsync(x_out, xc_, nb, hipMemcpyDeviceToHost, st));
diff --git a/conjugategradientoptim.jl_amd/csrc/cgo_capi.hip b/conjugategradientoptim.jl_amd/csrc/cgo_capi.hip
--- a/conjugategradientoptim.jl_amd/csrc/cgo_capi.hip
+++ b/conjugategradientoptim.jl_amd/csrc/cgo_capi.hip
@@ -370,8 +370,9 @@
     API_GUARD_END
 }
 
-static const int kReplayDepth = 6;
+static const int kReplayDepth = 8;
 static const bool kLeanSums = true;
+static const bool kPathPredict = true;
 static int env_tri(const char *name) { const char *e = getenv(name); return e ? (e[0] != '0' ? 1 : 0) : -1; }
 static int resolve_policy(cgo_ctx *ctx, const cgo_solver_policy *arg, cgo_solver_policy &r, std::string &why) {
     cgo_solver_policy lib; cgo_solver_policy_init(&lib);
@@ -444,6 +445,12 @@
     out->strict_tail = s->ctx->c.tail_strict ? 1 : 0;
     return CGO_OK;
     API_GUARD_END
+}
+
+static bool path_applies(const cgo_objective *obj, const cgo_cg_config *cfg, const cgo_ls_config *ls) {
+    if (!ls || obj->o.kind != CGO_OBJ_QUAD_DIAG || cfg->beta.kind != CGO_BETA_POLAK_RIBIERE) return false;
+    if (ls->kind == CGO_LS_STRONG_WOLFE_BISECTION) return true;
+    return ls->kind == CGO_LS_WOLFE_BISECTION && ls->cond_kind == CGO_COND_WOLFE;
 }
 
 static int make_solver(cgo_ctx *ctx, cgo_objective *obj, const cgo_cg_config *cfg, const cgo_ls_config *ls,
@@ -515,6 +522,12 @@
         s->be->set_beta_unread(beta_unread_sums(cfg->beta.kind));
         s->be->set_lean_sums(lean);
     }
+    {
+        bool predict = kPathPredict && kLeanSums && obj->o.kind == CGO_OBJ_QUAD_DIAG && 8.0 * (double)obj->o.n_local * 5.0 > 1.4e9;
+        const int forced = env_tri("CGO_PATH_PREDICT");
+        if (forced >= 0) predict = forced != 0;
+        s->be->set_path_prediction(predict && path_applies(obj, cfg, ls));
+    }
     if (int prc = s->be->place()) { delete s; obj_unref(obj); return prc; }
     if (pol.resident >= 0) s->be->set_resident(pol.resident != 0);
     if (int prc = s->be->prepare_controller()) { delete s; obj_unref(obj); return prc; }
@@ -740,6 +753,46 @@
     API_GUARD_BEGIN
     REQUIRE(s, "null argument");
     s->be->set_lean_sums(on != 0);
+    return CGO_OK;
+    API_GUARD_END
+}
+
+int cgo_solver_set_path_prediction(cgo_solver *s, int32_t on) {
+    API_GUARD_BEGIN
+    REQUIRE(s, "null argument");
+    const bool applies = s->sv && !s->sv->is_sys() && path_applies(s->obj, &s->sv->config(), &s->sv->linesearch());
+    s->be->set_path_prediction(on != 0 && applies);
+    return CGO_OK;
+    API_GUARD_END
+}
+
+int cgo_solver_path_stats(cgo_solver *s, int64_t *by_nact, int64_t *predicted, int64_t *tree, int64_t *misses) {
+    API_GUARD_BEGIN
+    REQUIRE(s && s->sv, "null argument");
+    if (by_nact) for (int j = 0; j < 8; ++j) by_nact[j] = s->be->path_launches(j);
+    int64_t p = 0, t = 0, m = 0;
+    s->sv->path_stats(p, t, m);
+    if (predicted) *predicted = p;
+    if (tree) *tree = t;
+    if (misses) *misses = m;
+    return CGO_OK;
+    API_GUARD_END
+}
+
+int cgo_solver_debug_set_path_skew(cgo_solver *s, double factor) {
+    API_GUARD_BEGIN
+    REQUIRE(s && s->sv, "null argument");
+    REQUIRE(factor > 0.0 && std::isfinite(factor), "path skew: a positive factor");
+    s->sv->set_path_skew(factor);
+    return CGO_OK;
+    API_GUARD_END
+}
+
+int cgo_solver_probe_set_path(cgo_solver *s, int32_t nact) {
+    API_GUARD_BEGIN
+    REQUIRE(s, "null argument");
+    REQUIRE(nact >= 0 && nact <= 7, "probe path row: 0 … 7 active points");
+    s->be->set_probe_path(nact);
     return CGO_OK;
     API_GUARD_END
 }
diff --git a/conjugategradientoptim.jl_amd/csrc/cgo_engine.cpp b/conjugategradientoptim.jl_amd/csrc/cgo_engine.cpp
--- a/conjugategradientoptim.jl_amd/csrc/cgo_engine.cpp
+++ b/conjugategradientoptim.jl_amd/csrc/cgo_engine.cpp
@@ -158,6 +158,8 @@
     qn_trial_done_ = false;
     res_fail_streak_ = 0; res_backoff_ = 0;
     tr_f_.clear(); tr_g_.clear(); tr_a_.clear(); tr_e_.clear(); log_.clear();
+    path_part_ = false; path_reset_ = false;
+    path_pred_ = 0; path_tree_ = 0; path_miss_ = 0;
     return CGO_OK;
 }
 
@@ -166,6 +168,7 @@
     status_ = status;
     finished_ = true;
     ncache_ = 0;
+    path_part_ = false;
     qn_trial_done_ = false;
     be_->discard_pending();
     if (cfg_.trace_enabled) {
@@ -187,8 +190,20 @@
     int hit = -1;
     for (int j = 0; j < ncache_; ++j)
         if (std::memcmp(&a, &cache_[j].a, sizeof(double)) == 0) { hit = j; break; }
+    int in_tree = -1;
+    if (hit < 0 && path_part_)
+        for (int j = 0; j < ntree_; ++j)
+            if (std::memcmp(&a, &tree_[j], sizeof(double)) == 0) { in_tree = j; break; }
     if (hit >= 0) {
         last_ = cache_[hit].s;
+    } else if (in_tree >= 0) {
+        Scal out[7];
+        if (int rc = be_->trial(tree_, ntree_, out)) return rc;
+        ncache_ = ntree_;
+        for (int j = 0; j < ntree_; ++j) cache_[j] = {tree_[j], out[j]};
+        last_ = out[in_tree];
+        path_part_ = false;
+        path_miss_++;
     } else {
         double pts[7] = {a, 0, 0, 0, 0, 0, 0};
         int k = 1;
@@ -250,6 +265,7 @@
             uu = sc.uu;
             s->dphi0_ = sc.gu;
             s->dir_is_neg_grad_ = true;
+            s->path_part_ = false; s->path_reset_ = true;
             return 0;
         }
     } bk{this};
@@ -407,12 +423,14 @@
             --res_backoff_;
         }
         host_next = false;
+        path_reset_ = false;
         LSOut o{};
         int rc = (ls_.kind == CGO_LS_STRONG_WOLFE_BISECTION) ? ls_strong_wolfe(a_initial_, o)
                  : (ls_.kind == CGO_LS_WOLFE_BISECTION)      ? ls_wolfe_bisection(a_initial_, o)
                                                              : ls_backtracking(a_initial_, o);
         if (rc) return rc;
         ncache_ = 0;
+        path_part_ = false;
         a_initial_ = o.a;
         if (o.status != CGO_SUCCESS) { finish(n - 1, o.status); break; }
         VecBackend::GramOut G;
@@ -525,6 +543,9 @@
                 for (int j = 0; j < CTL_MAXP; ++j) cs.a[j] = pts[j < k ? j : k - 1];
                 cs.npts = k; cs.go = 1; cs.it = it_;
                 rc = be_->accept_dir_trial_ctl(cc, cs, budget, out);
+            } else if (be_->path_rows() && k >= 6) {
+                k = path_points(a_xp, beta, pts, k);
+                rc = be_->accept_dir_trial_path(a_xp, beta, pts, k, out);
             } else {
                 rc = be_->accept_dir_trial(a_xp, beta, pts, k, out);
             }
@@ -537,6 +558,34 @@
     }
     finished = finished_;
     return CGO_OK;
+}
+
+int Solver::path_points(double a_xp, double beta, double (&pts)[7], int k) {
+    ntree_ = k;
+    for (int j = 0; j < 7; ++j) tree_[j] = pts[j];
+    path_part_ = false;
+    int kp = 0;
+    double pp[7] = {0, 0, 0, 0, 0, 0, 0};
+    if (cfg_.beta.kind == CGO_BETA_POLAK_RIBIERE && !path_reset_ && std::isfinite(last_.curv) && std::isfinite(beta) &&
+        std::isfinite(a_xp) && a_xp > 0.0 && std::isfinite(dphi0_) && std::isfinite(last_.gtu) && std::isfinite(last_.gtgt) &&
+        std::isfinite(last_.ygt) && std::isfinite(f_x_)) {
+        const double c_k = (last_.gtu - dphi0_) / a_xp;
+        const double d1 = -last_.gtgt + beta * last_.gtu;
+        const double c1 = (last_.curv - 2.0 * beta * last_.ygt / a_xp + beta * beta * c_k) * path_skew_;
+        kp = ls_predicted_path(ls_, f_x_, d1, c1, a_initial_, pp);
+    }
+    int ka = 0;
+    for (int j = 0; j < kp; ++j) {
+        bool held = false;
+        for (int q = 0; q < k; ++q) held = held || std::memcmp(&pp[j], &tree_[q], sizeof(double)) == 0;
+        if (!held) break;
+        pp[ka++] = pp[j];
+    }
+    if (ka == 0 || std::memcmp(&pp[0], &tree_[0], sizeof(double)) != 0) { path_tree_++; return k; }
+    for (int j = 0; j < 7; ++j) pts[j] = j < ka ? pp[j] : 0.0;
+    path_part_ = ka < k;
+    path_pred_++;
+    return ka;
 }
 
 int check_batch_config(const cgo_cg_config &cfg, const cgo_ls_config &ls, std::string &why) {
diff --git a/conjugategradientoptim.jl_amd/csrc/cgo_engine.hpp b/conjugategradientoptim.jl_amd/csrc/cgo_engine.hpp
--- a/conjugategradientoptim.jl_amd/csrc/cgo_engine.hpp
+++ b/conjugategradientoptim.jl_amd/csrc/cgo_engine.hpp
@@ -8,6 +8,7 @@
 
 #include "../../include/cgo.h"
 #include "cgo_ctl.hpp"
+#include "cgo_path.hpp"
 #include "cgo_resident.hpp"
 
 namespace cgo {
@@ -22,6 +23,7 @@
     double ygt = 0;
     double gu = 0;
     double uu = 0;
+    double curv = NAN;
 };
 
 enum KernelKind : int {
@@ -70,6 +72,8 @@
     virtual int max_points() const { return 1; }
     virtual int trial(const double *a, int k, Scal *out) = 0;
     virtual int accept_dir_trial(double a_acc, double beta, const double *a, int k, Scal *out) = 0;
+    virtual bool path_rows() const { return false; }
+    virtual int accept_dir_trial_path(double a_acc, double beta, const double *a, int k, Scal *out) { return accept_dir_trial(a_acc, beta, a, k, out); }
     virtual int ctl_depth() const { return 0; }
     virtual int accept_dir_trial_ctl(const CtlConfig &, const CtlState &s, int64_t , Scal *out) {
         return accept_dir_trial(s.a_acc, s.beta, s.a, s.npts, out);
@@ -151,6 +155,8 @@
     const cgo_cg_config &config() const { return cfg_; }
     const cgo_ls_config &linesearch() const { return ls_; }
     bool is_sys() const { return sys_; }
+    void path_stats(int64_t &predicted, int64_t &tree, int64_t &misses) const { predicted = path_pred_; tree = path_tree_; misses = path_miss_; }
+    void set_path_skew(double f) { path_skew_ = f; }
     void resume(double f_x0, int64_t evals, const ResState &s, const ResRecord *recs);
 
   private:
@@ -205,6 +211,12 @@
     std::vector<int64_t> tr_e_;
     std::vector<TrialRecord> log_;
     bool log_on_ = false;
+    double tree_[7] = {};
+    int ntree_ = 0;
+    bool path_part_ = false, path_reset_ = false;
+    double path_skew_ = 1.0;
+    int64_t path_pred_ = 0, path_tree_ = 0, path_miss_ = 0;
+    int path_points(double a_xp, double beta, double (&pts)[7], int k);
 };
 
 struct BatchRun {
diff --git a/conjugategradientoptim.jl_amd/csrc/cgo_hip_backend.hip b/conjugategradientoptim.jl_amd/csrc/cgo_hip_backend.hip
--- a/conjugategradientoptim.jl_amd/csrc/cgo_hip_backend.hip
+++ b/conjugategradientoptim.jl_amd/csrc/cgo_hip_backend.hip
@@ -793,6 +793,18 @@
     if (obj_->two_phase()) return lse_stats(LM_ACCEPT | LM_DIR, a_acc, beta, a[0], out[0], true);
     if (int rc = launch_k(KK_ACCEPT_DIR_TRIAL, a_acc, beta, a[0], true, s)) return rc;
     unpack(s, out[0], true, true);
+    return CGO_OK;
+}
+
+int HipBackend::accept_dir_trial_path(double a_acc, double beta, const double *a, int k, Scal *out) {
+    if (!path_rows()) return accept_dir_trial(a_acc, beta, a, k, out);
+    double s[NR7];
+    path_nact_ = k <= 5 ? std::max(k, 1) : MAXP;
+    const int rc = accept_dir_trial_r(a_acc, beta, a, k, s);
+    path_nact_ = 0;
+    if (rc) return rc;
+    unpack_r(s, k, out, true, MAXP);
+    for (int j = 0; j < k; ++j) { out[j].curv = out[j].yy; out[j].yy = 0.0; }
     return CGO_OK;
 }
 
diff --git a/conjugategradientoptim.jl_amd/csrc/cgo_hip_backend.hpp b/conjugategradientoptim.jl_amd/csrc/cgo_hip_backend.hpp
--- a/conjugategradientoptim.jl_amd/csrc/cgo_hip_backend.hpp
+++ b/conjugategradientoptim.jl_amd/csrc/cgo_hip_backend.hpp
@@ -223,6 +223,12 @@
     void set_beta_unread(int bits) { lean_mask_ = bits; if (lean_bits_) lean_bits_ = bits; }
     void set_lean_sums(bool on) { lean_bits_ = on ? lean_mask_ : 0; }
     bool lean_sums() const { return lean_bits_ != 0; }
+    void set_path_prediction(bool on) { path_on_ = on; }
+    bool path_prediction() const { return path_on_; }
+    bool path_rows() const override;
+    int accept_dir_trial_path(double a_acc, double beta, const double *a, int k, Scal *out) override;
+    int64_t path_launches(int nact) const { return (nact >= 1 && nact <= 7) ? path_count_[nact] : 0; }
+    void set_probe_path(int nact) { probe_nact_ = nact; }
     std::string kernel_symbol(int kernel_kind) const;
     int probe_launch(int kernel_kind, int variant, double a_acc, double beta, const double *a, int k, const double *x,
                      const double *u, const double *aux, double *sums, int sums_cap, int *sums_len, double *x_out,
@@ -272,7 +278,7 @@
     bool last_big_ = false;
     int probe_prepare();
     int probe_slack_intact();
-    std::string r_symbol(int mode, int npts, bool big) const;
+    std::string r_symbol(int mode, int npts, bool big, int nact = 0) const;
     std::string probe_syms_;
     void probe_note(const double *row, int len, const char *fmt, ...);
     int probe_ring_slack_intact();
@@ -316,6 +322,10 @@
     int materialize_lag();
     int lean_mask_ = 0, lean_bits_ = 0;
     int lean_for(int mode) const;
+    bool path_on_ = false;
+    int path_nact_ = 0, last_nact_ = 0, probe_nact_ = 0;
+    int path_last_n_ = 0, path_last_s_ = 0;
+    int64_t path_count_[8] = {};
     int accept_dir_trial_r(double a_acc, double beta, const double *a, int k, double *s);
     int trial_r(const double *a, int k, double *s);
     int launch_r_kernel(int kk, int mode, double a_acc, double beta, const double *a, int k, int npts,
diff --git a/conjugategradientoptim.jl_amd/csrc/cgo_kernels_cg_path.hip.hpp b/conjugategradientoptim.jl_amd/csrc/cgo_kernels_cg_path.hip.hpp
--- /dev/null
+++ b/conjugategradientoptim.jl_amd/csrc/cgo_kernels_cg_path.hip.hpp
@@ -0,0 +1,150 @@
+#pragma once
+
+#include "cgo_kernels_cg.hip.hpp"
+
+namespace cgo {
+namespace dev {
+
+template <class Obj> struct ObjCurv { static constexpr bool declared = false; };
+template <> struct ObjCurv<ObjQuadDiag> {
+    static constexpr bool declared = true;
+    __device__ static inline d2 apply2(d2 v, const PV<ObjQuadDiag> &p) { return d2{p.v[0].x * v.x, p.v[0].y * v.y}; }
+    __device__ static inline double apply1(double v, const PS<ObjQuadDiag> &p) { return p.v[0] * v; }
+};
+
+constexpr bool path_mode(int mode) {
+    return (r_base(mode) == (R_REPLAY | R_ACCEPT | R_DIR | R_TRIAL | R_NOWU | R_NOWX) || r_base(mode) == (R_REPLAY | R_ACCEPT | R_DIR | R_TRIAL)) &&
+           (mode & R_NOYY) != 0;
+}
+
+template <class Obj, int MODE, int NACT>
+__device__ inline void cg_path_pair(const RParams &P, d2 &x, d2 &u, const PV<Obj> &p, double (&acc)[RW<MAXP>::W], bool &wx, bool &wu) {
+    constexpr int R_GU = RW<MAXP>::GU, R_UU = RW<MAXP>::UU;
+#pragma unroll
+    for (int j = 0; j < RMAX; ++j) {
+        if (j < P.nrep) {
+            d2 gr;
+            double fr = 0.0;
+            x.x = x.x + P.ra[j] * u.x;
+            x.y = x.y + P.ra[j] * u.y;
+            obj_eval2<Obj>(x, p, P.s0, fr, gr);
+            u.x = -gr.x + P.rb[j] * u.x; u.y = -gr.y + P.rb[j] * u.y;
+        }
+    }
+    x.x = x.x + P.a_acc * u.x;
+    x.y = x.y + P.a_acc * u.y;
+    wx = r_writes_x(MODE);
+    d2 g;
+    double f0 = 0.0;
+    obj_eval2<Obj>(x, p, P.s0, f0, g);
+    {
+        d2 un;
+        un.x = -g.x + P.beta * u.x; un.y = -g.y + P.beta * u.y;
+        acc[R_GU] = dsum(acc[R_GU], g.x, un.x); acc[R_GU] = dsum(acc[R_GU], g.y, un.y);
+        acc[R_UU] = dsum(acc[R_UU], un.x, un.x); acc[R_UU] = dsum(acc[R_UU], un.y, un.y);
+        u = un;
+        wu = r_writes_u(MODE);
+    }
+#pragma unroll
+    for (int j = 0; j < NACT; ++j) {
+        const int b = RS_PER_POINT * j;
+        d2 xp, gt;
+        xp.x = x.x + P.a[j] * u.x;
+        xp.y = x.y + P.a[j] * u.y;
+        obj_term2<Obj, LateF<Obj, MODE>::on>(xp, p, P.s0, acc[b + RS_F], gt);
+        const double y0 = gt.x - g.x, y1 = gt.y - g.y;
+        acc[b + RS_GTU] = dsum(acc[b + RS_GTU], gt.x, u.x);   acc[b + RS_GTU] = dsum(acc[b + RS_GTU], gt.y, u.y);
+        acc[b + RS_GTGT] = dsum(acc[b + RS_GTGT], gt.x, gt.x); acc[b + RS_GTGT] = dsum(acc[b + RS_GTGT], gt.y, gt.y);
+        if (!(MODE & R_NOGTG)) { acc[b + RS_GTG] = dsum(acc[b + RS_GTG], gt.x, g.x);   acc[b + RS_GTG] = dsum(acc[b + RS_GTG], gt.y, g.y); }
+        if (!(MODE & R_NOUY)) { acc[b + RS_UY] = dsum(acc[b + RS_UY], u.x, y0);      acc[b + RS_UY] = dsum(acc[b + RS_UY], u.y, y1); }
+        if (!(MODE & R_NOYGT)) { acc[b + RS_YGT] = dsum(acc[b + RS_YGT], y0, gt.x);    acc[b + RS_YGT] = dsum(acc[b + RS_YGT], y1, gt.y); }
+        if constexpr (ObjCurv<Obj>::declared) {
+            const d2 hg = ObjCurv<Obj>::apply2(gt, p);
+            acc[b + RS_YY] = dsum(acc[b + RS_YY], gt.x, hg.x); acc[b + RS_YY] = dsum(acc[b + RS_YY], gt.y, hg.y);
+        }
+    }
+}
+
+template <class Obj, int MODE, int NACT>
+__device__ inline void cg_path_single(const RParams &P, long long i, double (&acc)[RW<MAXP>::W]) {
+    constexpr int R_GU = RW<MAXP>::GU, R_UU = RW<MAXP>::UU;
+    double x = P.x[i];
+    double u = P.u[i];
+    const PS<Obj> p = ps_load<Obj>(P, i);
+#pragma unroll
+    for (int j = 0; j < RMAX; ++j) {
+        if (j < P.nrep) {
+            double gr = 0.0, fr = 0.0;
+            x = x + P.ra[j] * u;
+            obj_eval1<Obj>(x, p, P.s0, fr, gr);
+            u = -gr + P.rb[j] * u;
+        }
+    }
+    x = x + P.a_acc * u;
+    if (r_writes_x(MODE)) P.xo[i] = x;
+    double g = 0.0, f0 = 0.0;
+    obj_eval1<Obj>(x, p, P.s0, f0, g);
+    const double un = -g + P.beta * u;
+    acc[R_GU] = dsum(acc[R_GU], g, un); acc[R_UU] = dsum(acc[R_UU], un, un);
+    if (r_writes_u(MODE)) P.uo[i] = un;
+    u = un;
+#pragma unroll
+    for (int j = 0; j < NACT; ++j) {
+        const int b = RS_PER_POINT * j;
+        const double xp = x + P.a[j] * u;
+        double gt;
+        obj_term1<Obj, LateF<Obj, MODE>::on>(xp, p, P.s0, acc[b + RS_F], gt);
+        const double y = gt - g;
+        acc[b + RS_GTU] = dsum(acc[b + RS_GTU], gt, u); acc[b + RS_GTGT] = dsum(acc[b + RS_GTGT], gt, gt);
+        if (!(MODE & R_NOGTG)) acc[b + RS_GTG] = dsum(acc[b + RS_GTG], gt, g);
+        if (!(MODE & R_NOUY)) acc[b + RS_UY] = dsum(acc[b + RS_UY], u, y);
+        if (!(MODE & R_NOYGT)) acc[b + RS_YGT] = dsum(acc[b + RS_YGT], y, gt);
+        if constexpr (ObjCurv<Obj>::declared) acc[b + RS_YY] = dsum(acc[b + RS_YY], gt, ObjCurv<Obj>::apply1(gt, p));
+    }
+}
+
+template <class Obj, int MODE, int NACT, bool BIG>
+__global__ __launch_bounds__(BLOCK) void k_cg_path(const RParams P) {
+    static_assert(BIG, "path launches exist as pure-HBM streams only");
+    static_assert(path_mode(MODE), "a path row is launch N or S of the replay cycle in a lean form that leaves the y·y slot free");
+    static_assert(NACT >= 1 && NACT <= MAXP, "1 … 7 of the row's seven points");
+    constexpr int W = RW<MAXP>::W;
+    double acc[W];
+#pragma unroll
+    for (int s = 0; s < W; ++s) acc[s] = 0.0;
+    const long long n2 = P.n >> 1;
+    const long long per = big_chunk_pairs(n2, gridDim.x);
+    long long i = per * blockIdx.x + threadIdx.x;
+    const long long hi = (per * blockIdx.x + per < n2) ? per * blockIdx.x + per : n2;
+    const long long step = BLOCK;
+    for (; i + step < hi; i += 2 * step) {
+        d2 xa = ldg2<true>(P.x, i), xb = ldg2<true>(P.x, i + step);
+        d2 ua = ldg2<true>(P.u, i), ub = ldg2<true>(P.u, i + step);
+        const PV<Obj> pa = pv_load<Obj, true>(P, i), pb = pv_load<Obj, true>(P, i + step);
+        bool wxa = false, wua = false, wxb = false, wub = false;
+        cg_path_pair<Obj, MODE, NACT>(P, xa, ua, pa, acc, wxa, wua);
+        cg_path_pair<Obj, MODE, NACT>(P, xb, ub, pb, acc, wxb, wub);
+        if (wxa) stg2<true>(P.xo, i, xa);
+        if (wua) stg2<true>(P.uo, i, ua);
+        if (wxb) stg2<true>(P.xo, i + step, xb);
+        if (wub) stg2<true>(P.uo, i + step, ub);
+    }
+    if (i < hi) {
+        d2 xa = ldg2<true>(P.x, i);
+        d2 ua = ldg2<true>(P.u, i);
+        const PV<Obj> pa = pv_load<Obj, true>(P, i);
+        bool wxa = false, wua = false;
+        cg_path_pair<Obj, MODE, NACT>(P, xa, ua, pa, acc, wxa, wua);
+        if (wxa) stg2<true>(P.xo, i, xa);
+        if (wua) stg2<true>(P.uo, i, ua);
+    }
+    if ((P.n & 1) && blockIdx.x == 0 && threadIdx.x == 0) cg_path_single<Obj, MODE, NACT>(P, P.n - 1, acc);
+    if constexpr (LateF<Obj, MODE>::on) {
+#pragma unroll
+        for (int j = 0; j < NACT; ++j) acc[RS_PER_POINT * j + RS_F] *= ObjFScale<Obj>::scale;
+    }
+    store_partials_n<W, false>(acc, P.partials, P.tail);
+}
+
+}
+}
diff --git a/conjugategradientoptim.jl_amd/csrc/cgo_path.hpp b/conjugategradientoptim.jl_amd/csrc/cgo_path.hpp
--- /dev/null
+++ b/conjugategradientoptim.jl_amd/csrc/cgo_path.hpp
@@ -0,0 +1,47 @@
+#pragma once
+
+#include "cgo_ctl.hpp"
+
+namespace cgo {
+
+struct PathModelEval {
+    double f, d0, c;
+    double a[CTL_MAXP];
+    int n; bool over;
+    CGO_HD int operator()(double step, double &phi, double &dphi, double, double, double, double) {
+        bool seen = false;
+        for (int j = 0; j < CTL_MAXP; ++j) if (j < n && a[j] == step) seen = true;
+        if (!seen) {
+            if (n >= CTL_MAXP) { over = true; return 1; }
+            for (int j = 0; j < CTL_MAXP; ++j) if (j == n) a[j] = step;
+            ++n;
+        }
+        phi = f + step * d0 + 0.5 * (step * step) * c;
+        dphi = d0 + step * c;
+        return 0;
+    }
+};
+
+CGO_HD inline int ls_predicted_path(const cgo_ls_config &ls, double f, double dphi0, double c, double a_initial, double (&pts)[7]) {
+    for (int j = 0; j < 7; ++j) pts[j] = 0.0;
+    if (!(hd_isfinite(f) && hd_isfinite(dphi0) && hd_isfinite(c))) return 0;
+    if (!(c > 0.0) || !(dphi0 < 0.0)) return 0;
+    if (ls.kind != CGO_LS_STRONG_WOLFE_BISECTION && ls.kind != CGO_LS_WOLFE_BISECTION) return 0;
+    if (ls.kind == CGO_LS_WOLFE_BISECTION && ls.cond_kind != CGO_COND_WOLFE) return 0;
+    PathModelEval ev;
+    ev.f = f; ev.d0 = dphi0; ev.c = c; ev.n = 0; ev.over = false;
+    for (int j = 0; j < CTL_MAXP; ++j) ev.a[j] = 0.0;
+    LSOut o = ls_out(0.0, 0.0, 0, CGO_INCOMPLETE);
+    if (ls.kind == CGO_LS_STRONG_WOLFE_BISECTION) {
+        (void)ls_strong_wolfe_t(ls, f, dphi0, a_initial, ev, o);
+    } else {
+        CtlNoBackend bk;
+        double uu = 0.0;
+        (void)ls_wolfe_bisection_t(ls, f, dphi0, uu, a_initial, ev, bk, o);
+    }
+    for (int j = 0; j < 7; ++j) pts[j] = ev.a[j];
+    for (int j = 0; j < 7; ++j) if (j < ev.n && !(hd_isfinite(pts[j]) && pts[j] > 0.0)) return 0;
+    return ev.n;
+}
+
+}
diff --git a/include/cgo.h b/include/cgo.h
--- a/include/cgo.h
+++ b/include/cgo.h
@@ -370,6 +370,10 @@
 } cgo_batch_probe_args;
 int cgo_batch_probe(cgo_ctx *ctx, cgo_batch_probe_args *p);
 int64_t cgo_batch_probe_qn_bytes(void);
+int cgo_solver_set_path_prediction(cgo_solver *s, int32_t on);
+int cgo_solver_path_stats(cgo_solver *s, int64_t *by_nact, int64_t *predicted, int64_t *tree, int64_t *misses);
+int cgo_solver_probe_set_path(cgo_solver *s, int32_t nact);
+int cgo_solver_debug_set_path_skew(cgo_solver *s, double factor);
 int32_t cgo_stop_status(int64_t it, int64_t max_iters, double f_x, double grad_norm, double eps, double f_x0, int64_t *iters_ran);
 
 int cgo_kernel_dir(cgo_ctx *ctx, double *u, const double *g, double beta, int64_t n,
```

After: 2324, median of 6. +7.3%, better.
